# nschejtman/deepLoopCloser

Measured on AMD Instinct MI355X. Metric: query-frames/sec vs N-keyframe DB + top-k recall@1, higher is better.
Workload: dtype bf16; 1 GPU; 1000000 x 4096 bf16 keyframe DB, Q=256, top-20 cosine match, 1 GPU(s); db_rows=1000000, dim=4096, k=20, rows_per_gpu=1000000, pipelined=False, crowded=False

## Files before the change

deeploopcloser_amd/_lib.py:

```python
import ctypes as C
import os

_HERE = os.path.dirname(os.path.abspath(__file__))
LIB_PATH = os.path.join(_HERE, "libdlc_hip.so")

DLC_OK = 0
DLC_ERR_BAD_ARG, DLC_ERR_BAD_SHAPE, DLC_ERR_UNSUPPORTED, DLC_ERR_HIP, DLC_ERR_WORKSPACE = -1, -2, -3, -4, -5
DLC_BF16, DLC_F16, DLC_F32, DLC_F64, DLC_I8, DLC_U8, DLC_I64 = 0, 1, 2, 3, 4, 5, 6
DLC_ACT_NONE, DLC_ACT_SIGMOID, DLC_ACT_RELU = 0, 1, 2
DLC_B_KN, DLC_B_NK = 0, 1
DLC_MAX_K = 128
DLC_ABI_VERSION = 17
DLC_SELECT_COOP = 1
DLC_SIM_FORCE_F64, DLC_SIM_NO_HOST_SYNC = 1, 2

_vp, _i64, _int, _sz, _dbl, _flt = C.c_void_p, C.c_int64, C.c_int, C.c_size_t, C.c_double, C.c_float

SIGNATURES = {
    "dlc_abi_version": (_int, []),
    "dlc_create": (_int, [_int, C.POINTER(_vp)]),
    "dlc_destroy": (_int, [_vp]),
    "dlc_last_error": (C.c_char_p, [_vp]),
    "dlc_status_string": (C.c_char_p, [_int]),
    "dlc_gemm_bias_act": (_int, [_vp, _int, _int, _int, _i64, _i64, _i64, _vp, _i64, _vp, _i64, _vp, _vp, _i64, _vp]),
    "dlc_bias_act": (_int, [_vp, _int, _int, _i64, _i64, _vp, _i64, _vp, _vp, _i64, _vp]),
    "dlc_sdav_encode_workspace_bytes": (_sz, [_i64, C.POINTER(_i64), _int, _int]),
    "dlc_sdav_encode": (_int, [_vp, _int, _i64, _int, C.POINTER(_i64), _vp, C.POINTER(_vp), C.POINTER(_vp), _vp, _vp,
                               _sz, _vp]),
    "dlc_sdav_split_panels_bytes": (_sz, [_int, C.POINTER(_i64)]),
    "dlc_sdav_split_prepare": (_int, [_vp, _int, C.POINTER(_i64), C.POINTER(_vp), _vp, _sz, _vp]),
    "dlc_sdav_encode_split_workspace_bytes": (_sz, [_i64, C.POINTER(_i64), _int]),
    "dlc_cnnvtl_split_panels_bytes": (_sz, [_int, C.POINTER(C.c_int32)]),
    "dlc_cnnvtl_split_prepare": (_int, [_vp, _int, C.POINTER(C.c_int32), C.POINTER(_vp), _vp, _sz, _vp]),
    "dlc_cnnvtl_encode_split_workspace_bytes": (_sz, [_i64, _int, _int, _int, _int, C.POINTER(C.c_int32)]),
    "dlc_cnnvtl_encode_split": (_int, [_vp, _int, _vp, _i64, _int, _int, _int, _int, _int, C.POINTER(C.c_int32), _vp, C.POINTER(_vp),
                                       _vp, _i64, _vp, C.POINTER(_vp), _vp, _vp, _sz, _vp]),
    "dlc_cnnvtl_layers_split": (_int, [_vp, _vp, _i64, _int, _int, _int, _int, C.POINTER(C.c_int32), _int, _int, _vp, C.POINTER(_vp),
                                       C.POINTER(_vp), _vp, _vp, _sz, _vp]),
    "dlc_sdav_encode_split": (_int, [_vp, _i64, _int, C.POINTER(_i64), _vp, _vp, C.POINTER(_vp), _vp, _vp, _sz, _vp]),
    "dlc_sdav_train_workspace_bytes": (_sz, [_i64, _i64, C.POINTER(_i64), _int, _int]),
    "dlc_sdav_train_step": (_int, [_vp, _int, _i64, _i64, _int, C.POINTER(_i64), _vp, C.POINTER(_vp), C.POINTER(_vp),
                                  C.POINTER(_vp), _vp, _dbl, _dbl, _dbl, _dbl, _vp, _vp, _sz, _vp]),
    "dlc_random_mask_f64": (_int, [_vp, _vp, _i64, _i64, C.c_uint64, C.c_uint64, _vp]),
    "dlc_salt_pepper_mask_f64": (_int, [_vp, _vp, _vp, _i64, _i64, C.c_uint64, C.c_uint64, _vp]),
    "dlc_da_corrupt_f64": (_int, [_vp, _vp, _vp, _vp, _i64, _i64, _vp, _i64, _vp]),
    "dlc_da_train_workspace_bytes": (_sz, [_i64, _i64, _i64, _i64]),
    "dlc_da_train_step": (_int, [_vp, _i64, _i64, _i64, _i64, _vp, _vp, _vp, _vp, _vp, _dbl, _dbl, _dbl, _dbl, _vp, _vp, _sz,
                                _vp]),
    "dlc_rgb_to_gray_u8": (_int, [_vp, _vp, _i64, _vp, _vp]),
    "dlc_harris_keypoints_workspace_bytes": (_sz, [_i64, _int, _int]),
    "dlc_harris_keypoints_u8": (_int, [_vp, _vp, _i64, _int, _int, _int, _vp, _vp, _vp, _vp, _sz, _vp]),
    "dlc_extract_patches": (_int, [_vp, _vp, _i64, _int, _int, _vp, _int, _int, _int, _vp, _vp]),
    "dlc_im2col_nhwc_f64": (_int, [_vp, _vp, _i64, _int, _int, _int, _int, _int, _int, _int, _int, _int, _int, _vp, _vp]),
    "dlc_conv2d_nhwc_f64": (_int, [_vp, _vp, _i64, _int, _int, _int, _vp, _vp, _int, _int, _int, _int, _int, _int, _int,
                                  _int, _int, _vp, _vp]),
    "dlc_space_to_depth_nhwc_f64": (_int, [_vp, _vp, _i64, _int, _int, _int, _int, _vp, _vp]),
    "dlc_maxpool3x3s2_nhwc_f64": (_int, [_vp, _vp, _i64, _int, _int, _int, _vp, _vp]),
    "dlc_minmax_quant_gather_i8": (_int, [_vp, C.POINTER(_vp), C.POINTER(_i64), _int, _i64, _vp, _i64, _vp, _vp, _vp]),
    "dlc_cnnvtl_frame_minmax_init": (_int, [_vp, _vp, _i64, _vp]),
    "dlc_conv2d_nhwc_f64_stats": (_int, [_vp, _vp, _i64, _int, _int, _int, _vp, _vp, _int, _int, _int, _int, _int, _int, _int,
                                         _int, _int, _vp, _vp, _vp]),
    "dlc_quant_gather_i8": (_int, [_vp, C.POINTER(_vp), C.POINTER(_i64), _int, _i64, _vp, _i64, _vp, _vp, _vp, _vp]),
    "dlc_sdav_range_words": (_sz, [_i64]),
    "dlc_sdav_distinctive_score": (_int, [_vp, _vp, _i64, _i64, _dbl, _dbl, _vp, _vp, _vp]),
    "dlc_sdav_similarity_workspace_bytes": (_sz, [_i64, _i64, _i64, _int, _i64]),
    "dlc_sdav_similarity_matrix": (_int, [_vp, _vp, _i64, _i64, _i64, _vp, _dbl, _dbl, _vp, _vp, _int, _i64, _vp, _vp, _vp,
                                         _vp, _sz, _vp]),
    "dlc_topk_rows_f64": (_int, [_vp, _vp, _i64, _i64, _i64, _i64, _int, _vp, _vp, _vp, _vp]),
    "dlc_sdav_stream_state_bytes": (_sz, [_i64, _i64, _i64]),
    "dlc_sdav_stream_init": (_int, [_vp, _vp, _sz, _i64, _i64, _i64, _dbl, _dbl, _vp, _vp]),
    "dlc_sdav_stream_append": (_int, [_vp, _vp, _sz, _i64, _i64, _i64, _vp, _i64, _i64, _vp, _vp]),
    "dlc_sdav_stream_query": (_int, [_vp, _vp, _sz, _i64, _i64, _i64, _vp, _i64, _vp, _dbl, _dbl, _vp, _vp, _vp]),
    "dlc_sdav_stream_query_batch_workspace_bytes": (_sz, [_i64, _i64, _i64]),
    "dlc_sdav_stream_query_batch": (_int, [_vp, _vp, _sz, _i64, _i64, _i64, _vp, _i64, _i64, _vp, _dbl, _dbl, _vp, _i64, _vp,
                                           _vp, _sz, _vp]),
    "dlc_sdav_stream_query_batch_staged": (_int, [_vp, _vp, _sz, _i64, _i64, _i64, _vp, _i64, _i64, _vp, _dbl, _dbl, _vp, _i64,
                                                  _vp, _vp, _sz, _int, _vp]),
    "dlc_cnnvtl_distance_matrix": (_int, [_vp, _vp, _i64, _i64, _i64, _vp, _vp]),
    "dlc_cnnvtl_distance_topk_workspace_bytes": (_sz, [_i64, _i64, _i64, _int]),
    "dlc_cnnvtl_distance_topk": (_int, [_vp, _vp, _i64, _i64, _vp, _i64, _i64, _i64, _i64, _i64, _int, _vp, _vp, _vp, _sz,
                                        _vp]),
    "dlc_cnnvtl_distance_rows": (_int, [_vp, _vp, _i64, _i64, _vp, _i64, _i64, _i64, _i64, _i64, _vp, _i64, _vp]),
    "dlc_sequence_topk_workspace_bytes": (_sz, [_i64, _i64, _int, _int, _int]),
    "dlc_sequence_topk": (_int, [_vp, _int, _vp, _i64, _i64, _i64, _i64, _i64, _i64, _int, _int, C.POINTER(C.c_int32), _int, _int,
                                 _vp, _vp, _vp, _vp, _i64, _vp, _vp, _sz, _vp]),
    "dlc_contrast_rows": (_int, [_vp, _int, _vp, _i64, _i64, _i64, _i64, _i64, _int, _vp, _i64, _vp]),
    "dlc_peak_topk_rows_workspace_bytes": (_sz, [_i64, _i64, _int]),
    "dlc_peak_topk_rows": (_int, [_vp, _int, _vp, _i64, _i64, _i64, _i64, _i64, _int, _i64, _int, _i64, _int, _vp, _vp, _vp,
                                  _vp, _sz, _vp]),
    "dlc_l2_normalize_rows": (_int, [_vp, _int, _vp, _i64, _i64, _i64, _int, _int, _vp, _i64, _vp]),
    "dlc_cosine_topk_workspace_bytes": (_sz, [_i64, _i64, _i64, _int]),
    "dlc_cosine_topk": (_int, [_vp, _int, _vp, _i64, _i64, _vp, _i64, _i64, _i64, _int, _i64, _vp, _vp, _vp, _vp, _vp, _vp, _sz,
                              _vp]),
    "dlc_max_row_norm": (_int, [_vp, _int, _vp, _i64, _i64, _i64, _vp, _vp]),
    "dlc_cosine_tau_scale": (_int, [_vp, _int, _vp, _i64, _i64, _i64, _vp, _vp, _vp]),
    "dlc_cosine_topk_older": (_int, [_vp, _int, _vp, _i64, _i64, _vp, _i64, _i64, _i64, _int, _i64, _i64, _vp, _vp, _vp, _vp, _vp,
                                    _vp, _sz, _vp]),
    "dlc_cosine_score_error_bound": (_dbl, [_i64, _i64, _i64, _int]),
    "dlc_cosine_score_error_bound_any_plan": (_dbl, [_i64]),
    "dlc_cosine_score_groups": (_int, [_vp, _int, _vp, _i64, _i64, _vp, _i64, _i64, _i64, _int, _vp, _sz, _vp]),
    "dlc_cosine_select_topk": (_int, [_vp, _int, _vp, _i64, _i64, _vp, _i64, _i64, _i64, _int, _i64, _vp, _vp, _vp, _vp, _vp, _vp,
                                     _sz, _int, _vp]),
    "dlc_cosine_groups_per_query": (_int, [_int]),
    "dlc_cosine_select_groups": (_int, [_vp, _int, _vp, _i64, _i64, _vp, _i64, _i64, _i64, _int, _vp, _sz, _vp, _vp, _int,
                                       _vp]),
    "dlc_cosine_rescore_topk": (_int, [_vp, _int, _vp, _i64, _i64, _vp, _i64, _i64, _i64, _int, _i64, _vp, _vp, _vp, _int,
                                      _vp, _vp, _vp, _vp, _int, _vp]),
    "dlc_cosine_exhaustive_topk": (_int, [_vp, _int, _vp, _i64, _i64, _vp, _i64, _i64, _i64, _int, _i64, _vp, _i64, _dbl,
                                         _vp, _vp, _vp, _vp, _vp, _vp, _sz, _vp]),
    "dlc_topk_merge_strided": (_int, [_vp, _vp, _i64, _vp, _i64, _int, _i64, _int, _vp, _dbl, _vp, _vp, _vp, _vp, _vp, _vp]),
    "dlc_topk_merge": (_int, [_vp, _vp, _vp, _int, _i64, _int, _vp, _vp, _vp, _vp]),
    "dlc_topk_keep_older": (_int, [_vp, _vp, _vp, _i64, _int, _i64, _int, _vp, _vp, _vp]),
    "dlc_cosine_scores_workspace_bytes": (_sz, [_i64, _i64, _i64]),
    "dlc_cosine_scores": (_int, [_vp, _int, _vp, _i64, _i64, _vp, _i64, _i64, _i64, _vp, _i64, _vp, _sz, _vp]),
    "dlc_cosine_score_rows": (_int, [_vp, _int, _vp, _i64, _i64, _vp, _i64, _i64, _i64, _i64, _i64, _vp, _vp, _i64, _vp]),
    "dlc_host_to_device": (_int, [_vp, _vp, _vp, _sz, _vp]),
    "dlc_device_to_host": (_int, [_vp, _vp, _vp, _sz, _vp]),
    "dlc_set_host_threads": (_int, [_vp, _int]),
    "dlc_set_scratch": (_int, [_vp, _vp, _sz]),
    "dlc_set_profiling": (_int, [_vp, _int]),
    "dlc_profile_gemm_ms": (_int, [_vp, C.POINTER(_flt), _int]),
}

_lib = None


class DlcError(RuntimeError):
    """A HIP-side failure (DLC_ERR_HIP / DLC_ERR_WORKSPACE) reported by the C ABI."""


def load():
    global _lib
    if _lib is not None:
        return _lib
    if not os.path.exists(LIB_PATH):
        raise ImportError(
            "deeploopcloser_amd: %s is missing -- build it with `python -c 'import __graft_entry__ as g; g.build()'` "
            "or `make -C deeploopcloser_amd/csrc`.  There is no CPU fallback." % LIB_PATH)
    lib = C.CDLL(LIB_PATH)
    for name, (res, args) in SIGNATURES.items():
        fn = getattr(lib, name)
        fn.restype = res
        fn.argtypes = args
    if lib.dlc_abi_version() != DLC_ABI_VERSION:
        raise ImportError("deeploopcloser_amd: %s has ABI %d, these bindings are for ABI %d -- rebuild it"
                          % (LIB_PATH, lib.dlc_abi_version(), DLC_ABI_VERSION))
    _lib = lib
    return lib


def raise_for_status(lib, ctx, rc):
    if rc == DLC_OK:
        return
    msg = lib.dlc_last_error(ctx).decode() if ctx else ""
    text = "%s: %s" % (lib.dlc_status_string(rc).decode(), msg)
    if rc in (DLC_ERR_BAD_ARG, DLC_ERR_BAD_SHAPE, DLC_ERR_UNSUPPORTED):
        raise ValueError(text)
    raise DlcError(text)
```

deeploopcloser_amd/csrc/cosine_topk.hip:

```cpp
#include "dlc_internal.h"
#include "lds_dma.h"

#include <algorithm>

namespace {

constexpr int BM = 256;
constexpr int BNQ = 256;
constexpr int BK = 64;
constexpr int NTHREADS = 512;
constexpr int TILE_BYTES = 256 * BK * 2;
constexpr int A_TILE = TILE_BYTES;
constexpr int B_TILE = TILE_BYTES;
#ifndef DLC_A_STAGES
#define DLC_A_STAGES 2
#endif
constexpr int A_STAGES = DLC_A_STAGES;
constexpr int B_RING = A_STAGES * A_TILE;
constexpr int LDS_BYTES = A_STAGES * A_TILE + 2 * B_TILE;
#ifndef DLC_STAGGER_SLEEP
#define DLC_STAGGER_SLEEP 15
#endif
#ifndef DLC_STAGGER_PHASES
#define DLC_STAGGER_PHASES 32
// ... 241 lines not shown
#pragma unroll
                for (int r = 0; r < 4; ++r)
                    if (row0 + r < p.n) p.S[(long long)qidx * p.lds + row0 + r] = acc[t][c][r];
            }
        }
    } else {
#pragma unroll
        for (int c = 0; c < 4; ++c) {
            const int qidx = qblk * BNQ + wc * 64 + c * 16 + i;
            float hm[2];
#pragma unroll
            for (int th = 0; th < 2; ++th) {
                float m0 = acc[th * 4][c][0], m1 = acc[th * 4 + 2][c][0];
#pragma unroll
                for (int tt = 0; tt < 2; ++tt)
#pragma unroll
                    for (int r = 0; r < 4; ++r) {
                        m0 = fmaxf(m0, acc[th * 4 + tt][c][r]);
                        m1 = fmaxf(m1, acc[th * 4 + 2 + tt][c][r]);
                    }
                hm[th] = fmaxf(m0, m1);
                const long long g = tile * (BM / GROUP) + wr * 16 + th * 8 + lg * 2;
                if (qidx < p.q) {
                    float* dst = p.gmax + (long long)qidx * p.ldg + g;
                    if (g + 1 < p.ng) *(float2*)dst = make_float2(m0, m1);
                    else if (g < p.ng) dst[0] = m0;
                }
            }
            float h = fmaxf(hm[0], hm[1]);
            h = fmaxf(h, __shfl_xor(h, 16));
            h = fmaxf(h, __shfl_xor(h, 32));
            const long long ht = tile * 2 + wr;
            if (lg == 0 && qidx < p.q && ht < p.nh) p.tmax[(long long)qidx * p.ldt + ht] = h;
        }
    }
}

template <typename Tag> struct Dot2;
template <> struct Dot2<dlc_bf16_tag> {
    typedef __attribute__((ext_vector_type(2))) __bf16 v2_t;
    static __device__ __forceinline__ float run(unsigned a, unsigned b, float c) {
        return __builtin_amdgcn_fdot2_f32_bf16(__builtin_bit_cast(v2_t, a), __builtin_bit_cast(v2_t, b), c, false);
    }
};
template <> struct Dot2<dlc_f16_tag> {
    typedef __attribute__((ext_vector_type(2))) _Float16 v2_t;
    static __device__ __forceinline__ float run(unsigned a, unsigned b, float c) {
        return __builtin_amdgcn_fdot2(__builtin_bit_cast(v2_t, a), __builtin_bit_cast(v2_t, b), c, false);
    }
};

constexpr int GEMV_MAX_Q = 4;
constexpr int GEMV_MAX_LDS = 64 * 1024;

template <typename Tag, int QB>
__global__ __launch_bounds__(256) void score_gemv_kernel(GemmArgs p) {
    extern __shared__ __attribute__((aligned(16))) char smem[];
    __shared__ float wmax[4][QB];
    const int tid = threadIdx.x, lane = tid & 63, w = tid >> 6;
    const long long half = blockIdx.x;
    const int d_bytes = p.nk * 128;
    for (int off = tid * 16; off < QB * d_bytes; off += 256 * 16) {
        const int qi = off / d_bytes, within = off - qi * d_bytes;
        uint4 v = make_uint4(0, 0, 0, 0);
        if (qi < p.q) v = *(const uint4*)(p.Q + (long long)qi * p.ldq_b + within);
        *(uint4*)(smem + off) = v;
    }
    __syncthreads();
    float hmax[QB];
#pragma unroll
    for (int qq = 0; qq < QB; ++qq) hmax[qq] = -INFINITY;
    for (int gi = 0; gi < 4; ++gi) {
        const long long g = half * GROUPS_PER_HALF + w * 4 + gi;
        const char* rows[GROUP];
#pragma unroll
        for (int r = 0; r < GROUP; ++r) {
            long long rr = g * GROUP + r;
            if (rr > p.n - 1) rr = p.n - 1;
            rows[r] = p.DB + rr * p.lddb_b;
        }
        float acc[QB][GROUP];
#pragma unroll
        for (int qq = 0; qq < QB; ++qq)
#pragma unroll
            for (int r = 0; r < GROUP; ++r) acc[qq][r] = 0.f;
        for (int c = lane * 16; c < d_bytes; c += 1024) {
            uint4 rv[GROUP];
#pragma unroll
            for (int r = 0; r < GROUP; ++r) rv[r] = *(const uint4*)(rows[r] + c);
#pragma unroll
            for (int qq = 0; qq < QB; ++qq) {
                const uint4 qv = *(const uint4*)(smem + qq * d_bytes + c);
#pragma unroll
                for (int r = 0; r < GROUP; ++r) {
                    float a = acc[qq][r];
                    a = Dot2<Tag>::run(rv[r].x, qv.x, a);
                    a = Dot2<Tag>::run(rv[r].y, qv.y, a);
                    a = Dot2<Tag>::run(rv[r].z, qv.z, a);
                    a = Dot2<Tag>::run(rv[r].w, qv.w, a);
                    acc[qq][r] = a;
                }
            }
        }
#pragma unroll
        for (int qq = 0; qq < QB; ++qq) {
            float m = -INFINITY;
#pragma unroll
            for (int r = 0; r < GROUP; ++r) {
                float v = acc[qq][r];
#pragma unroll
                for (int o = 32; o > 0; o >>= 1) v += __shfl_xor(v, o);
                m = fmaxf(m, v);
            }
            hmax[qq] = fmaxf(hmax[qq], m);
            if (lane == 0 && qq < p.q && g < p.ng) p.gmax[(long long)qq * p.ldg + g] = m;
        }
    }
    if (lane == 0) {
#pragma unroll
        for (int qq = 0; qq < QB; ++qq) wmax[w][qq] = hmax[qq];
    }
    __syncthreads();
    if (tid < QB && tid < p.q && half < p.nh)
        p.tmax[(long long)tid * p.ldt + half] = fmaxf(fmaxf(wmax[0][tid], wmax[1][tid]), fmaxf(wmax[2][tid], wmax[3][tid]));
}

__device__ __forceinline__ unsigned f32_key(float x) {
    unsigned u = __float_as_uint(x);
    return (u & 0x80000000u) ? ~u : (u | 0x80000000u);
}
__device__ __forceinline__ float key_f32(unsigned k) {
    return __uint_as_float((k & 0x80000000u) ? (k ^ 0x80000000u) : ~k);
}
__device__ __forceinline__ unsigned long long pack_key(float score, unsigned id) {
    return ((unsigned long long)f32_key(score) << 32) | (unsigned long long)(~id);
}
__device__ __forceinline__ unsigned key_id(unsigned long long key) { return ~(unsigned)key; }


__device__ __forceinline__ unsigned wave_max_u32(unsigned v) {
#define DLC_DPP_MAX(ctrl, rmask) \
    v = max(v, (unsigned)__builtin_amdgcn_update_dpp((int)v, (int)v, ctrl, rmask, 0xf, false))
    DLC_DPP_MAX(0x111, 0xf);
    DLC_DPP_MAX(0x112, 0xf);
    DLC_DPP_MAX(0x114, 0xf);
    DLC_DPP_MAX(0x118, 0xf);
    DLC_DPP_MAX(0x142, 0xa);
    DLC_DPP_MAX(0x143, 0xc);
#undef DLC_DPP_MAX
    return (unsigned)__builtin_amdgcn_readlane((int)v, 63);
}

constexpr int FIN_THREADS = 512;
__host__ __device__ inline size_t fin_lds_fixed(int kg) {
    return (size_t)kg * (GROUPS_PER_HALF * 8 + GROUP * (8 + 8 + 4)) + (size_t)(kg + 1) * 8 + 64;
}

__device__ __forceinline__ void rank_select(const unsigned long long* keys, int m, int k, int* out, bool plus_one = false) {
    const int lim = plus_one ? k + 1 : k;
    for (int e = threadIdx.x; e < m; e += blockDim.x) {
        const unsigned long long ke = keys[e];
        if (ke == 0ull) continue;
        int rank = 0;
#pragma unroll 8
        for (int j = 0; j < m; ++j) rank += keys[j] > ke ? 1 : 0;
        if (rank < lim) out[rank] = e;
    }
}
template <typename Id>
__device__ __forceinline__ void rank_select64(const long long* keys, const Id* ids, int m, int k, int* out) {
    for (int e = threadIdx.x; e < m; e += blockDim.x) {
        const long long ke = keys[e];
        if (ke == KEY64_EMPTY) continue;
        const Id ie = ids[e];
        int rank = 0;
#pragma unroll 4
        for (int j = 0; j < m; ++j) {
            const long long kj = keys[j];
            rank += (kj > ke || (kj == ke && kj != KEY64_EMPTY && ids[j] < ie)) ? 1 : 0;
        }
        if (rank < k) out[rank] = e;
    }
}

template <typename Tag, int RS_UNROLL>
__device__ __forceinline__ void rescore8_f64(const char* qrow, const char* const (&rows)[GROUP], int d, int lane,
                                             double (&acc)[GROUP]) {
#pragma unroll
    for (int r = 0; r < GROUP; ++r) acc[r] = 0.0;
    for (int d0 = lane * 8; d0 < d; d0 += 512 * RS_UNROLL) {
        uint4 qv[RS_UNROLL], rv[RS_UNROLL][GROUP];
#pragma unroll
        for (int u = 0; u < RS_UNROLL; ++u) {
            const int dd = d0 + u * 512;
            const bool ok = dd < d;
            qv[u] = ok ? *(const uint4*)(qrow + (long long)dd * 2) : make_uint4(0, 0, 0, 0);
#pragma unroll
            for (int r = 0; r < GROUP; ++r)
                rv[u][r] = ok ? *(const uint4*)(rows[r] + (long long)dd * 2) : make_uint4(0, 0, 0, 0);
        }
#pragma unroll
        for (int u = 0; u < RS_UNROLL; ++u) {
            const unsigned qw[4] = {qv[u].x, qv[u].y, qv[u].z, qv[u].w};
            double qd[8];
#pragma unroll
            for (int e = 0; e < 4; ++e) {
                qd[2 * e] = (double)Mfma16<Tag>::to_f32((unsigned short)(qw[e] & 0xffffu));
                qd[2 * e + 1] = (double)Mfma16<Tag>::to_f32((unsigned short)(qw[e] >> 16));
            }
#pragma unroll
            for (int r = 0; r < GROUP; ++r) {
                const unsigned w4[4] = {rv[u][r].x, rv[u][r].y, rv[u][r].z, rv[u][r].w};
#pragma unroll
                for (int e = 0; e < 4; ++e) {
                    acc[r] = fma(qd[2 * e], (double)Mfma16<Tag>::to_f32((unsigned short)(w4[e] & 0xffffu)), acc[r]);
                    acc[r] = fma(qd[2 * e + 1], (double)Mfma16<Tag>::to_f32((unsigned short)(w4[e] >> 16)), acc[r]);
                }
            }
        }
    }
#pragma unroll
    for (int r = 0; r < GROUP; ++r) {
        double v = acc[r];
#pragma unroll
        for (int o = 32; o > 0; o >>= 1) v += __shfl_xor(v, o);
        acc[r] = v;
    }
}

template <typename Tag, int R, int U>
__device__ __forceinline__ void rescore_rows_f64(const char* qrow, const char* const (&rows)[R], int d, int lane,
                                                 double (&acc)[R]) {
#pragma unroll
    for (int r = 0; r < R; ++r) acc[r] = 0.0;
    for (int d0 = lane * 8; d0 < d; d0 += 512 * U) {
        uint4 qv[U], rv[U][R];
#pragma unroll
        for (int u = 0; u < U; ++u) {
            const int dd = d0 + u * 512;
            const bool ok = dd < d;
            qv[u] = ok ? *(const uint4*)(qrow + (long long)dd * 2) : make_uint4(0, 0, 0, 0);
#pragma unroll
            for (int r = 0; r < R; ++r) rv[u][r] = ok ? *(const uint4*)(rows[r] + (long long)dd * 2) : make_uint4(0, 0, 0, 0);
        }
#pragma unroll
        for (int u = 0; u < U; ++u) {
            const unsigned qw[4] = {qv[u].x, qv[u].y, qv[u].z, qv[u].w};
            double qd[8];
#pragma unroll
            for (int e = 0; e < 4; ++e) {
                qd[2 * e] = (double)Mfma16<Tag>::to_f32((unsigned short)(qw[e] & 0xffffu));
                qd[2 * e + 1] = (double)Mfma16<Tag>::to_f32((unsigned short)(qw[e] >> 16));
            }
#pragma unroll
            for (int r = 0; r < R; ++r) {
                const unsigned w4[4] = {rv[u][r].x, rv[u][r].y, rv[u][r].z, rv[u][r].w};
#pragma unroll
                for (int e = 0; e < 4; ++e) {
                    acc[r] = fma(qd[2 * e], (double)Mfma16<Tag>::to_f32((unsigned short)(w4[e] & 0xffffu)), acc[r]);
                    acc[r] = fma(qd[2 * e + 1], (double)Mfma16<Tag>::to_f32((unsigned short)(w4[e] >> 16)), acc[r]);
                }
            }
        }
    }
#pragma unroll
    for (int r = 0; r < R; ++r) {
        double v = acc[r];
#pragma unroll
        for (int o = 32; o > 0; o >>= 1) v += __shfl_xor(v, o);
        acc[r] = v;
    }
}
template <typename Tag>
__device__ __forceinline__ double rescore1_f64(const char* qrow, const char* row, int d, int lane) {
    const char* const rows[1] = {row};
    double acc[1];
    rescore_rows_f64<Tag, 1, 4>(qrow, rows, d, lane, acc);
    return acc[0];
}

__device__ __forceinline__ double scaled_tau(double tau, const float* __restrict__ tau_scale, int qi) {
    return tau_scale ? tau * (double)tau_scale[qi] : tau;
}

enum { FIN_FUSED = 0, FIN_GROUPS = 1, FIN_RESCORE = 2 };
struct FinishArgs {
    float* tmax; long long ldt; int nh; int tv_in_lds;
    const float* gmax; long long ldg; long long ng;
    int kg;
    const char* Q; long long ldq_b; const char* DB; long long lddb_b;
    long long n; int d; int k; long long row_offset;
    float* out_s;
    double* out_s64;
    long long* out_i;
    int* status;
    double tau;
    const float* tau_scale;
    int* grp_ids;
    float* grp_max;
    const float* all_max;
    int parts;
    long long nq;
    int gparts;
    float* bound_out;
    const float* dense_S;
    long long ld_s;
    int rslack;
    int limited;
    long long limit0;
};
__device__ __forceinline__ long long visible_rows(long long n, int limited, long long limit0, int qi) {
    if (!limited) return n;
    const long long lim = limit0 + qi;
    return lim < 0 ? 0 : (lim < n ? lim : n);
}

template <typename Tag, int THREADS, int RS_UNROLL, int MODE>
__device__ __forceinline__ void finish_topk_body(const FinishArgs& a) {
    extern __shared__ __attribute__((aligned(16))) char dsm[];
    constexpr int FIN_WAVES = THREADS / 64;
    constexpr int FIN_THREADS = THREADS;
    constexpr int GPH = GROUPS_PER_HALF;
    const int kg = a.kg, k = a.k;
    const double tau = scaled_tau(a.tau, a.tau_scale, (int)blockIdx.x);
    const long long n = visible_rows(a.n, a.limited, a.limit0, (int)blockIdx.x);
    const long long ng = a.limited ? (n + GROUP - 1) / GROUP : a.ng;
    if (n <= 0) {
        if constexpr (MODE == FIN_GROUPS) {
            for (int e = threadIdx.x; e <= kg; e += THREADS) {
                if (e < kg) a.grp_ids[(long long)blockIdx.x * kg + e] = -1;
                a.grp_max[(long long)blockIdx.x * (kg + 1) + e] = -INFINITY;
            }
        } else {
            const long long oq = (long long)blockIdx.y * a.nq + blockIdx.x;
            for (int e = threadIdx.x; e < k; e += THREADS) {
                if (a.out_s) a.out_s[oq * k + e] = -INFINITY;
                a.out_s64[oq * k + e] = -INFINITY;
                a.out_i[oq * k + e] = -1;
            }
            if (MODE == FIN_FUSED && threadIdx.x == 0) a.status[blockIdx.x] = 0;
            if (MODE == FIN_RESCORE && a.bound_out && blockIdx.y == 0 && threadIdx.x == 0) a.bound_out[blockIdx.x] = -INFINITY;
        }
        return;
    }
    unsigned long long* ckey = (unsigned long long*)dsm;
    long long* ck64 = (long long*)(dsm + (size_t)kg * GPH * 8);
    double* cs64 = (double*)(dsm + (size_t)kg * (GPH * 8 + GROUP * 8));
    int* crow = (int*)(dsm + (size_t)kg * (GPH * 8 + GROUP * 16));
    int* sel = (int*)(dsm + (size_t)kg * (GPH * 8 + GROUP * 20));
    int* sel2 = sel + kg + 1;
    unsigned* misc = (unsigned*)(sel2 + kg + 1);
    const int qi = blockIdx.x, tid = threadIdx.x, lane = tid & 63, w = tid >> 6;
    float* tv = a.tv_in_lds ? (float*)(dsm + fin_lds_fixed(kg)) : a.tmax + (long long)qi * a.ldt;
    if (a.tv_in_lds)
        for (int e = tid; e < a.nh; e += FIN_THREADS) tv[e] = a.tmax[(long long)qi * a.ldt + e];
    for (int e = tid; e <= kg; e += FIN_THREADS) { sel[e] = -1; sel2[e] = -1; }
    if (tid < 16) misc[tid] = 0u;
    __syncthreads();
    int kg2;
    unsigned bkey = 0u;
    if constexpr (MODE != FIN_RESCORE) {
    const int nh = a.limited ? (int)((n + HALF - 1) / HALF) : a.nh;
    const int kt = min(kg, nh);
    {
        const int chunk = (nh + FIN_WAVES - 1) / FIN_WAVES;
        const int lo_e = w * chunk, hi_e = min(nh, lo_e + chunk);
        unsigned bh = 0, bl = 0;
        constexpr int LV = 16;
        if ((THREADS == 512 || MODE == FIN_GROUPS) && chunk <= 64 * LV) {
            unsigned vk[LV];
#pragma unroll
            for (int j = 0; j < LV; ++j) {
                const int e = lo_e + lane + 64 * j;
                const float v = e < hi_e ? tv[e] : -INFINITY;
                vk[j] = v == -INFINITY ? 0u : f32_key(v);
            }
            auto rescan_regs = [&]() {
                bh = 0; bl = 0;
#pragma unroll
                for (int j = 0; j < LV; ++j) {
                    const unsigned l = ~(unsigned)(lo_e + lane + 64 * j);
                    if (vk[j] > bh) { bh = vk[j]; bl = l; }
                }
            };
            rescan_regs();
            for (int it = 0; it < kt; ++it) {
                const unsigned mh = wave_max_u32(bh);
                const unsigned ml = wave_max_u32(bh == mh ? bl : 0u);
                if (lane == 0) ckey[w * kt + it] = mh == 0u ? 0ull : (((unsigned long long)mh << 32) | ml);
                if (mh != 0u && bh == mh && bl == ml) {
                    const int jr = (int)((~ml) - (unsigned)(lo_e + lane)) >> 6;
#pragma unroll
                    for (int j = 0; j < LV; ++j)
                        if (j == jr) vk[j] = 0u;
                    rescan_regs();
                }
            }
        } else {
        auto rescan = [&]() {
            bh = 0; bl = 0;
            for (int e = lo_e + lane; e < hi_e; e += 64) {
                const float v = tv[e];
                if (v == -INFINITY) continue;
                const unsigned h = f32_key(v), l = ~(unsigned)e;
                if (h > bh || (h == bh && l > bl)) { bh = h; bl = l; }
            }
        };
        rescan();
        for (int it = 0; it < kt; ++it) {
            const unsigned mh = wave_max_u32(bh);
            const unsigned ml = wave_max_u32(bh == mh ? bl : 0u);
            if (lane == 0) ckey[w * kt + it] = mh == 0u ? 0ull : (((unsigned long long)mh << 32) | ml);
            if (mh != 0u && bh == mh && bl == ml) {
                tv[~ml] = -INFINITY;
                rescan();
            }
        }
        }
        const unsigned rest = wave_max_u32(bh);
        if (lane == 0) misc[w] = rest;
    }
    __syncthreads();
    rank_select(ckey, FIN_WAVES * kt, kt, sel, true);
    __syncthreads();
#pragma unroll
    for (int ww = 0; ww < FIN_WAVES; ++ww) bkey = max(bkey, misc[ww]);
    if (sel[kt] >= 0) bkey = max(bkey, (unsigned)(ckey[sel[kt]] >> 32));
    if (tid < kt) { const int c = sel[tid]; sel[tid] = c < 0 ? -1 : (int)key_id(ckey[c]); }
    __syncthreads();

    const int m2 = kt * GPH;
    for (int e = tid; e < m2; e += FIN_THREADS) {
        const int ht = sel[e / GPH];
        const long long g = (long long)ht * GPH + (e % GPH);
        float gm = (ht >= 0 && g < ng) ? a.gmax[(long long)qi * a.ldg + g] : 0.0f;
        if (a.limited && a.dense_S && ht >= 0 && g == ng - 1 && (n & (GROUP - 1))) {
            gm = -INFINITY;
            for (long long row = g * GROUP; row < n; ++row) gm = fmaxf(gm, a.dense_S[(long long)qi * a.ld_s + row]);
        }
        ckey[e] = (ht >= 0 && g < ng) ? pack_key(gm, (unsigned)g) : 0ull;
    }
    __syncthreads();
    kg2 = min(kg, m2);
    rank_select(ckey, m2, kg2, sel2, true);
    __syncthreads();
    if (sel2[kg2] >= 0) bkey = max(bkey, (unsigned)(ckey[sel2[kg2]] >> 32));
    if constexpr (MODE == FIN_GROUPS) {
        const long long W = kg + 1;
        for (int e = tid; e < kg; e += FIN_THREADS) {
            const int c = e < kg2 ? sel2[e] : -1;
            a.grp_ids[(long long)qi * kg + e] = c < 0 ? -1 : (int)key_id(ckey[c]);
            a.grp_max[(long long)qi * W + e] = c < 0 ? -INFINITY : a.gmax[(long long)qi * a.ldg + key_id(ckey[c])];
        }
        if (tid == 0) a.grp_max[(long long)qi * W + kg] = bkey ? key_f32(bkey) : -INFINITY;
        return;
    }
    if (tid < kg2) {
        const int c = sel2[tid];
        int g = c < 0 ? -1 : (int)key_id(ckey[c]);
        if (tid >= k && g >= 0 && sel2[k - 1] >= 0 && !(a.limited && !a.dense_S)) {
            const double uk = (double)key_f32((unsigned)(ckey[sel2[k - 1]] >> 32));
            if ((double)key_f32((unsigned)(ckey[c] >> 32)) < uk - 2.0 * tau) g = -2;
        }
        misc[9] = 0u;
        crow[tid] = g;
    }
    __syncthreads();
    if (tid < kg2) {
        const int g = crow[tid];
        if (g == -2) atomicMax(&misc[9], (unsigned)(ckey[sel2[tid]] >> 32));
    }
    __syncthreads();
    if (tid < kg2) sel2[tid] = crow[tid] < 0 ? -1 : crow[tid];
    bkey = max(bkey, misc[9]);
    __syncthreads();
    } else {
        kg2 = kg;
        const long long W = kg + 1;
        if (a.parts > 0) {
            unsigned bk = 0u;
            for (int e = tid; e < a.parts * (int)W; e += FIN_THREADS) {
                const int pp = e / (int)W, j = e % (int)W;
                const float v = a.all_max[((long long)pp * a.nq + qi) * W + j];
                if (v == -INFINITY) continue;
                if (j == kg) { bk = max(bk, f32_key(v)); continue; }
                int greater = 0;
                for (int p2 = 0; p2 < a.parts; ++p2) {
                    const float* av = a.all_max + ((long long)p2 * a.nq + qi) * W;
                    for (int j2 = 0; j2 < kg; ++j2) greater += av[j2] > v ? 1 : 0;
                }
                if (greater >= kg) bk = max(bk, f32_key(v));
            }
            if (bk) atomicMax(&misc[8], bk);
        }
        for (int e = tid; e < kg; e += FIN_THREADS) {
            int g = a.grp_ids[(long long)qi * kg + e];
            if (g >= 0 && a.parts > 0) {
                const float v = a.grp_max[(long long)qi * W + e];
                int greater = 0;
                for (int pp = 0; pp < a.parts; ++pp) {
                    const float* av = a.all_max + ((long long)pp * a.nq + qi) * W;
                    for (int j = 0; j < kg; ++j) greater += av[j] > v ? 1 : 0;
                }
                if (greater >= kg) g = -1;
            }
            if (a.gparts > 1 && e % a.gparts != (int)blockIdx.y) g = -1;
            sel2[e] = g;
        }
        __syncthreads();
        if (a.parts > 0) bkey = misc[8];
        else {
            const float v = a.grp_max[(long long)qi * W + kg];
            bkey = v == -INFINITY ? 0u : f32_key(v);
        }
        if (a.bound_out && blockIdx.y == 0 && tid == 0) a.bound_out[qi] = bkey ? key_f32(bkey) : -INFINITY;
    }

    int m3;
    if (a.dense_S) {
        const int m = kg2 * GROUP;
        for (int e = tid; e < m; e += FIN_THREADS) {
            const int g = sel2[e / GROUP];
            const long long row = (long long)g * GROUP + (e % GROUP);
            ckey[e] = (g >= 0 && row < n) ? pack_key(a.dense_S[(long long)qi * a.ld_s + row], (unsigned)row) : 0ull;
        }
        m3 = min(k + a.rslack, m);
        for (int e = tid; e <= m3 && e < kg * GROUP; e += FIN_THREADS) crow[e] = -1;
        __syncthreads();
        if (m3 < m) rank_select(ckey, m, m3, crow, true);
        else rank_select(ckey, m, m3, crow, false);
        __syncthreads();
        if (m3 < m && crow[m3] >= 0) bkey = max(bkey, (unsigned)(ckey[crow[m3]] >> 32));
        __syncthreads();
        for (int e = tid; e < m3; e += FIN_THREADS) { const int c = crow[e]; crow[e] = c < 0 ? -1 : (int)key_id(ckey[c]); }
    } else {
        m3 = kg2 * GROUP;
        for (int e = tid; e < m3; e += FIN_THREADS) {
            const int g = sel2[e / GROUP];
            const long long row = (long long)g * GROUP + (e % GROUP);
            crow[e] = (g >= 0 && row < n) ? (int)row : -1;
        }
    }
    __syncthreads();

    const char* qrow = a.Q + (long long)qi * a.ldq_b;
    if (MODE == FIN_FUSED && a.dense_S != nullptr) {
        for (int ci = w; ci < m3; ci += FIN_WAVES) {
            const int id = __builtin_amdgcn_readfirstlane(crow[ci]);
            const double sc = id < 0 ? 0.0 : rescore1_f64<Tag>(qrow, a.DB + (long long)id * a.lddb_b, a.d, lane);
            if (lane == 0) {
                cs64[ci] = id < 0 ? -INFINITY : sc;
                ck64[ci] = id < 0 ? KEY64_EMPTY : f64_key(sc);
            }
        }
    } else
    for (int s = w; s * GROUP < m3; s += FIN_WAVES) {
        int ids[GROUP];
        bool any = false;
        const char* rows[GROUP];
#pragma unroll
        for (int r = 0; r < GROUP; ++r) {
            ids[r] = __builtin_amdgcn_readfirstlane(s * GROUP + r < m3 ? crow[s * GROUP + r] : -1);
            any |= ids[r] >= 0;
            rows[r] = a.DB + (long long)(ids[r] < 0 ? 0 : ids[r]) * a.lddb_b;
        }
        double acc[GROUP] = {0.0, 0.0, 0.0, 0.0, 0.0, 0.0, 0.0, 0.0};
        if (any) rescore8_f64<Tag, RS_UNROLL>(qrow, rows, a.d, lane, acc);
#pragma unroll
        for (int r = 0; r < GROUP; ++r)
            if (lane == r && s * GROUP + r < m3) {
                cs64[s * GROUP + r] = ids[r] < 0 ? -INFINITY : acc[r];
                ck64[s * GROUP + r] = ids[r] < 0 ? KEY64_EMPTY : f64_key(acc[r]);
            }
    }
    const long long oq = (long long)blockIdx.y * a.nq + qi;
    for (int e = tid; e < k; e += FIN_THREADS) {
        if (a.out_s) a.out_s[oq * k + e] = -INFINITY;
        a.out_s64[oq * k + e] = -INFINITY;
        a.out_i[oq * k + e] = -1;
    }
    for (int e = tid; e <= kg; e += FIN_THREADS) sel[e] = -1;
    __syncthreads();

    rank_select64(ck64, crow, m3, k, sel);
    __syncthreads();
    for (int e = tid; e < k; e += FIN_THREADS) {
        const int c = sel[e];
        if (c >= 0) {
            if (a.out_s) a.out_s[oq * k + e] = (float)cs64[c];
            a.out_s64[oq * k + e] = cs64[c];
            a.out_i[oq * k + e] = (long long)crow[c] + a.row_offset;
        }
    }
    if constexpr (MODE == FIN_FUSED) {
        if (tid == 0) {
            const int c = sel[k - 1];
            const bool cert = bkey == 0u || (c >= 0 && cs64[c] > (double)key_f32(bkey) + tau);
            a.status[qi] = cert ? 0 : 1;
        }
    }
}

template <typename Tag, int THREADS, int RS_UNROLL, int MODE>
__global__ __launch_bounds__(THREADS) void finish_topk_kernel(FinishArgs a) {
    finish_topk_body<Tag, THREADS, RS_UNROLL, MODE>(a);
}
template <typename Tag, int RS_UNROLL, int MODE>
__global__ __launch_bounds__(256) __attribute__((amdgpu_waves_per_eu(5))) void finish_topk_coop_kernel(FinishArgs a) {
    finish_topk_body<Tag, 256, RS_UNROLL, MODE>(a);
}

struct ExhaustiveArgs {
    const float* gmax; long long ldg; long long ng;
    const char* Q; long long ldq_b; const char* DB; long long lddb_b;
    long long n; int d; int k; long long row_offset;
    const double* lower; long long lower_stride;
    float* out_s; double* out_s64; long long* out_i;
    int* status;
    double tau;
    const float* tau_scale;
    int limited; long long limit0;
};
constexpr int EXH_BATCH = 64;
constexpr int EXH_POOL = EXH_BATCH * GROUP + DLC_MAX_K;

template <typename Tag, int RS_UNROLL = 4>
__device__ __forceinline__ void exhaustive_topk_body(const ExhaustiveArgs& a, double lower) {
    const int qi = blockIdx.x;
    __shared__ long long pk[EXH_POOL];
    __shared__ double ps[EXH_POOL];
    __shared__ int pid[EXH_POOL];
    __shared__ int qlist[FIN_THREADS];
    __shared__ int wcnt[FIN_THREADS / 64];
    __shared__ int sel[DLC_MAX_K];
    const int tid = threadIdx.x, lane = tid & 63, w = tid >> 6, k = a.k;
    const long long n_vis = visible_rows(a.n, a.limited, a.limit0, qi);
    const long long ng_vis = a.limited ? (n_vis + GROUP - 1) / GROUP : a.ng;
    const double tau = scaled_tau(a.tau, a.tau_scale, qi);
    double theta = lower - tau;
    int cnt = 0;
    const char* qrow = a.Q + (long long)qi * a.ldq_b;
    for (long long c0 = 0; c0 < ng_vis; c0 += FIN_THREADS) {
        const long long g = c0 + tid;
        const bool qual = g < ng_vis && (double)a.gmax[(long long)qi * a.ldg + g] >= theta;
        const unsigned long long bal = __ballot(qual);
        if (lane == 0) wcnt[w] = __popcll(bal);
        __syncthreads();
        int base = 0, nqual = 0;
#pragma unroll
        for (int ww = 0; ww < FIN_THREADS / 64; ++ww) {
            base += ww < w ? wcnt[ww] : 0;
            nqual += wcnt[ww];
        }
        if (qual) qlist[base + __popcll(bal & ((1ull << lane) - 1ull))] = (int)g;
        __syncthreads();
        for (int b0 = 0; b0 < nqual; b0 += EXH_BATCH) {
            const int nb = min(EXH_BATCH, nqual - b0);
            for (int s = w; s < nb; s += FIN_THREADS / 64) {
                const long long row0 = (long long)qlist[b0 + s] * GROUP;
                const char* rows[GROUP];
#pragma unroll
                for (int r = 0; r < GROUP; ++r) rows[r] = a.DB + (row0 + r < a.n ? row0 + r : a.n - 1) * a.lddb_b;
                double acc[GROUP];
                rescore8_f64<Tag, RS_UNROLL>(qrow, rows, a.d, lane, acc);
#pragma unroll
                for (int r = 0; r < GROUP; ++r)
                    if (lane == r) {
                        const bool ok = row0 + r < n_vis;
                        ps[cnt + s * GROUP + r] = ok ? acc[r] : -INFINITY;
                        pk[cnt + s * GROUP + r] = ok ? f64_key(acc[r]) : KEY64_EMPTY;
                        pid[cnt + s * GROUP + r] = (int)(row0 + r);
                    }
            }
            for (int e = tid; e < k; e += FIN_THREADS) sel[e] = -1;
            __syncthreads();
            const int m = cnt + nb * GROUP;
            rank_select64(pk, pid, m, k, sel);
            __syncthreads();
            long long tk = KEY64_EMPTY; double ts = -INFINITY; int ti = -1;
            if (tid < k && sel[tid] >= 0) { const int c = sel[tid]; tk = pk[c]; ts = ps[c]; ti = pid[c]; }
            const unsigned long long have = __ballot(tid < k && sel[tid] >= 0);
            if (lane == 0) wcnt[w] = __popcll(have);
            __syncthreads();
            if (tid < k) { pk[tid] = tk; ps[tid] = ts; pid[tid] = ti; }
            cnt = 0;
#pragma unroll
            for (int ww = 0; ww < FIN_THREADS / 64; ++ww) cnt += wcnt[ww];
            __syncthreads();
            if (cnt == k && ps[k - 1] - tau > theta) theta = ps[k - 1] - tau;
        }
        __syncthreads();
    }
    for (int e = tid; e < k; e += FIN_THREADS) {
        const bool ok = e < cnt;
        if (a.out_s) a.out_s[(long long)qi * k + e] = ok ? (float)ps[e] : -INFINITY;
        if (a.out_s64) a.out_s64[(long long)qi * k + e] = ok ? ps[e] : -INFINITY;
        a.out_i[(long long)qi * k + e] = ok ? (long long)pid[e] + a.row_offset : -1;
    }
    if (tid == 0) a.status[qi] = 2;
}

template <typename Tag>
__global__ __launch_bounds__(FIN_THREADS) void exhaustive_topk_kernel(ExhaustiveArgs a) {
    const int qi = blockIdx.x;
    if (a.status[qi] != 1) return;
    exhaustive_topk_body<Tag>(a, a.lower[(long long)qi * a.lower_stride]);
}

struct SmallArgs {
    const float* P; long long ldp; long long qstride; int nsplit;
    float* gmax; long long ldg;
    const char* Q; long long ldq_b; const char* DB; long long lddb_b;
    long long n; int d; int k; int m3max; long long row_offset;
    float* out_s; double* out_s64; long long* out_i; int* status; double tau;
    const float* tau_scale;
    int limited; long long limit0;
};
constexpr int SMALL_KT_MAX = 40;
constexpr int SMALL_GPT = 4;

template <typename Tag, bool LONG>
__device__ __forceinline__ void small_topk_body(const SmallArgs& a) {
    __shared__ unsigned long long ckey[(FIN_THREADS / 64) * SMALL_KT_MAX];
    __shared__ long long ck64[SMALL_KT_MAX];
    __shared__ double cs64[SMALL_KT_MAX];
    __shared__ int crow[SMALL_KT_MAX];
    __shared__ int sel[SMALL_KT_MAX + 1];
    const int qi = blockIdx.x, tid = threadIdx.x, lane = tid & 63, w = tid >> 6, k = a.k;
    const long long n = visible_rows(a.n, a.limited, a.limit0, qi);
    for (int e = tid; e < k; e += FIN_THREADS) {
        if (a.out_s) a.out_s[(long long)qi * k + e] = -INFINITY;
        a.out_s64[(long long)qi * k + e] = -INFINITY;
        a.out_i[(long long)qi * k + e] = -1;
    }
    for (int e = tid; e <= SMALL_KT_MAX; e += FIN_THREADS) sel[e] = -1;
    if (n <= 0) {
        if (tid == 0) a.status[qi] = 0;
        return;
    }
    const long long ng_all = (a.n + GROUP - 1) / GROUP;
    unsigned vk[SMALL_GPT][GROUP];
#pragma unroll
    for (int j = 0; j < SMALL_GPT; ++j) {
        const long long g = tid + (long long)FIN_THREADS * j;
#pragma unroll
        for (int r = 0; r < GROUP; ++r) vk[j][r] = 0u;
        if (g < ng_all) {
            f64x4_t a64 = {0., 0., 0., 0.}, b64 = {0., 0., 0., 0.};
            const float* src = a.P + (long long)qi * a.ldp + g * GROUP;
            constexpr int PU = LONG ? 4 : 16;
            for (int c0 = 0; c0 < a.nsplit; c0 += PU) {
                f32x4_t pa[PU], pb[PU];
#pragma unroll
                for (int u = 0; u < PU; ++u) {
                    const float* sp = src + (long long)(c0 + u < a.nsplit ? c0 + u : c0) * a.qstride;
                    pa[u] = *(const f32x4_t*)(sp);
                    pb[u] = *(const f32x4_t*)(sp + 4);
                }
#pragma unroll
                for (int u = 0; u < PU; ++u)
                    if (c0 + u < a.nsplit) {
                        a64 += __builtin_convertvector(pa[u], f64x4_t);
                        b64 += __builtin_convertvector(pb[u], f64x4_t);
                    }
            }
            const f32x4_t lo = __builtin_convertvector(a64, f32x4_t), hi = __builtin_convertvector(b64, f32x4_t);
            a.gmax[(long long)qi * a.ldg + g] =
                fmaxf(fmaxf(fmaxf(lo[0], lo[1]), fmaxf(lo[2], lo[3])), fmaxf(fmaxf(hi[0], hi[1]), fmaxf(hi[2], hi[3])));
#pragma unroll
            for (int r = 0; r < 4; ++r) {
                vk[j][r] = g * GROUP + r < n ? f32_key(lo[r]) : 0u;
                vk[j][r + 4] = g * GROUP + r + 4 < n ? f32_key(hi[r]) : 0u;
            }
        }
    }
    const int m3 = (int)(n < (long long)a.m3max ? n : (long long)a.m3max);
    const int kt = (int)(n < (long long)(m3 + 1) ? n : (long long)(m3 + 1));
    unsigned bh = 0u, bl = 0u;
    unsigned gh[SMALL_GPT], gl[SMALL_GPT];
    auto rescan_group = [&](int j) {
        gh[j] = 0u; gl[j] = 0u;
#pragma unroll
        for (int r = 0; r < GROUP; ++r)
            if (vk[j][r] > gh[j]) { gh[j] = vk[j][r]; gl[j] = ~(unsigned)((tid + FIN_THREADS * j) * GROUP + r); }
    };
    auto combine = [&]() {
        bh = 0u; bl = 0u;
#pragma unroll
        for (int j = 0; j < SMALL_GPT; ++j)
            if (gh[j] > bh) { bh = gh[j]; bl = gl[j]; }
    };
#pragma unroll
    for (int j = 0; j < SMALL_GPT; ++j) rescan_group(j);
    combine();
    for (int it = 0; it < kt; ++it) {
        const unsigned mh = wave_max_u32(bh);
        const unsigned ml = wave_max_u32(bh == mh ? bl : 0u);
        if (lane == 0) ckey[w * kt + it] = mh == 0u ? 0ull : (((unsigned long long)mh << 32) | ml);
        if (mh != 0u && bh == mh && bl == ml) {
            const unsigned row = ~ml;
#pragma unroll
            for (int j = 0; j < SMALL_GPT; ++j)
                if ((row >> 3) == (unsigned)(tid + FIN_THREADS * j)) {
#pragma unroll
                    for (int r = 0; r < GROUP; ++r)
                        if ((row & 7u) == (unsigned)r) vk[j][r] = 0u;
                    rescan_group(j);
                }
            combine();
        }
    }
    __syncthreads();
    rank_select(ckey, (FIN_THREADS / 64) * kt, kt, sel);
    __syncthreads();
    const unsigned bkey = (kt > m3 && sel[m3] >= 0) ? (unsigned)(ckey[sel[m3]] >> 32) : 0u;
    if (tid < m3) crow[tid] = sel[tid] < 0 ? -1 : (int)key_id(ckey[sel[tid]]);
    __syncthreads();
    const char* qrow = a.Q + (long long)qi * a.ldq_b;
    constexpr int NW = FIN_THREADS / 64;
    if constexpr (LONG) {
        for (int s3 = w; s3 * 3 < m3; s3 += NW) {
            int ids[3];
            const char* rows[3];
#pragma unroll
            for (int r = 0; r < 3; ++r) {
                ids[r] = __builtin_amdgcn_readfirstlane(s3 * 3 + r < m3 ? crow[s3 * 3 + r] : -1);
                rows[r] = a.DB + (long long)(ids[r] < 0 ? 0 : ids[r]) * a.lddb_b;
            }
            double acc[3];
            rescore_rows_f64<Tag, 3, 4>(qrow, rows, a.d, lane, acc);
#pragma unroll
            for (int r = 0; r < 3; ++r)
                if (lane == r && s3 * 3 + r < m3) {
                    cs64[s3 * 3 + r] = ids[r] < 0 ? -INFINITY : acc[r];
                    ck64[s3 * 3 + r] = ids[r] < 0 ? KEY64_EMPTY : f64_key(acc[r]);
                }
        }
    } else {
    int ci = w;
    for (; ci + NW < m3; ci += 2 * NW) {
        const int id0 = __builtin_amdgcn_readfirstlane(crow[ci]), id1 = __builtin_amdgcn_readfirstlane(crow[ci + NW]);
        const char* const rows[2] = {a.DB + (long long)(id0 < 0 ? 0 : id0) * a.lddb_b,
                                     a.DB + (long long)(id1 < 0 ? 0 : id1) * a.lddb_b};
        double sc[2];
        rescore_rows_f64<Tag, 2, 8>(qrow, rows, a.d, lane, sc);
        if (lane == 0) {
            cs64[ci] = id0 < 0 ? -INFINITY : sc[0];
            ck64[ci] = id0 < 0 ? KEY64_EMPTY : f64_key(sc[0]);
            cs64[ci + NW] = id1 < 0 ? -INFINITY : sc[1];
            ck64[ci + NW] = id1 < 0 ? KEY64_EMPTY : f64_key(sc[1]);
        }
    }
// ... 172 lines not shown
    }
}

template <typename Src, typename Tag, int TPR, int NVEC>
__global__ __launch_bounds__(256) void l2_normalize_regs_kernel(const Src* __restrict__ src, long long lds, long long n,
                                                                int d, int center, unsigned short* __restrict__ dst,
                                                                long long ldd) {
    constexpr int VW = 16 / (int)sizeof(Src);
    typedef Src vec_t __attribute__((ext_vector_type(VW)));
    __shared__ double red[2][4];
    const int tid = threadIdx.x, lane = tid & 63;
    const int t = TPR == 64 ? lane : tid;
    const long long row = TPR == 64 ? (long long)blockIdx.x * 4 + (tid >> 6) : (long long)blockIdx.x;
    if (row >= n) return;
    const Src* x = src + row * lds;
    vec_t v[NVEC];
#pragma unroll
    for (int j = 0; j < NVEC; ++j) {
        const int e0 = (j * TPR + t) * VW;
        if (e0 + VW <= d) {
            v[j] = *(const vec_t*)(x + e0);
        } else {
#pragma unroll
            for (int i = 0; i < VW; ++i) v[j][i] = e0 + i < d ? x[e0 + i] : (Src)0;
        }
    }
    auto row_sum = [&](double s, int slot) -> double {
        for (int o = 32; o > 0; o >>= 1) s += __shfl_xor(s, o);
        if constexpr (TPR == 64) return s;
        if (lane == 0) red[slot][tid >> 6] = s;
        __syncthreads();
        return red[slot][0] + red[slot][1] + red[slot][2] + red[slot][3];
    };
    double mean = 0.0;
    if (center) {
        double s = 0.0;
#pragma unroll
        for (int j = 0; j < NVEC; ++j)
#pragma unroll
            for (int i = 0; i < VW; ++i) s += (double)v[j][i];
        mean = row_sum(s, 0) / (double)d;
    }
    double ss = 0.0;
#pragma unroll
    for (int j = 0; j < NVEC; ++j)
#pragma unroll
        for (int i = 0; i < VW; ++i) {
            const double c = (double)v[j][i] - mean;
            ss += ((j * TPR + t) * VW + i < d) ? c * c : 0.0;
        }
    const double nrm = sqrt(row_sum(ss, 1));
    const double inv = nrm > 0.0 ? 1.0 / nrm : 1.0;
    unsigned short* o = dst + row * ldd;
#pragma unroll
    for (int j = 0; j < NVEC; ++j) {
        const int e0 = (j * TPR + t) * VW;
        if (e0 >= ldd) continue;
        unsigned short bits[VW];
#pragma unroll
        for (int i = 0; i < VW; ++i) {
            bits[i] = 0;
            if (e0 + i < d) {
                const float f = f64_to_f32_once(((double)v[j][i] - mean) * inv);
                if constexpr (__is_same(Tag, dlc_bf16_tag)) bits[i] = __builtin_bit_cast(unsigned short, (__bf16)f);
                else bits[i] = __builtin_bit_cast(unsigned short, (_Float16)f);
            }
        }
        if constexpr (VW == 4) {
            *(uint2*)(o + e0) = make_uint2((unsigned)bits[0] | ((unsigned)bits[1] << 16),
                                           (unsigned)bits[2] | ((unsigned)bits[3] << 16));
        } else {
            *(unsigned*)(o + e0) = (unsigned)bits[0] | ((unsigned)bits[1] << 16);
        }
    }
}

__global__ __launch_bounds__(256) void splitk_groups_kernel(float* __restrict__ P, long long ldp, int q, int nsplit,
                                                            float* __restrict__ gmax, long long ldg, long long ng,
                                                            float* __restrict__ tmax, long long ldt, long long nh,
                                                            int keep_sum) {
    const int qi = blockIdx.x;
    const long long g = (long long)blockIdx.y * 256 + threadIdx.x;
    float m = -INFINITY;
    if (g < ng) {
        f64x4_t a64 = {0., 0., 0., 0.}, b64 = {0., 0., 0., 0.};
        float* dst0 = P + (long long)qi * ldp + g * GROUP;
        const float* src = dst0;
        for (int c = 0; c < nsplit; ++c) {
            a64 += __builtin_convertvector(*(const f32x4_t*)(src), f64x4_t);
            b64 += __builtin_convertvector(*(const f32x4_t*)(src + 4), f64x4_t);
            src += (long long)q * ldp;
        }
        const f32x4_t a = __builtin_convertvector(a64, f32x4_t), b = __builtin_convertvector(b64, f32x4_t);
        if (keep_sum && nsplit > 1) {
            *(f32x4_t*)dst0 = a;
            *(f32x4_t*)(dst0 + 4) = b;
        }
        m = fmaxf(fmaxf(fmaxf(a[0], a[1]), fmaxf(a[2], a[3])), fmaxf(fmaxf(b[0], b[1]), fmaxf(b[2], b[3])));
        gmax[(long long)qi * ldg + g] = m;
    }
    m = fmaxf(m, __shfl_xor(m, 1));
    m = fmaxf(m, __shfl_xor(m, 2));
    m = fmaxf(m, __shfl_xor(m, 4));
    m = fmaxf(m, __shfl_xor(m, 8));
    const long long ht = g / GROUPS_PER_HALF;
    if ((threadIdx.x & 15) == 0 && ht < nh) tmax[(long long)qi * ldt + ht] = m;
}

__global__ __launch_bounds__(256) void splitk_dense_kernel(const float* __restrict__ P, long long ldp, int q, int nsplit,
                                                           float* __restrict__ S, long long lds, long long n) {
    const int qi = blockIdx.x;
    const long long r0 = ((long long)blockIdx.y * 256 + threadIdx.x) * 4;
    if (r0 >= n) return;
    f64x4_t a64 = {0., 0., 0., 0.};
    const float* src = P + (long long)qi * ldp + r0;
    for (int c = 0; c < nsplit; ++c) {
        a64 += __builtin_convertvector(*(const f32x4_t*)src, f64x4_t);
        src += (long long)q * ldp;
    }
    const f32x4_t a = __builtin_convertvector(a64, f32x4_t);
#pragma unroll
    for (int r = 0; r < 4; ++r)
        if (r0 + r < n) S[(long long)qi * lds + r0 + r] = a[r];
}

struct SplitPlan {
    int nsplit, kchunk;
};
SplitPlan split_plan(int64_t q, int64_t n, int64_t d) {
    const int64_t ntiles = dlc::cdiv(n, BM);
    const int64_t base = dlc::cdiv(ntiles, (int64_t)8) * 8 * dlc::cdiv(q, BNQ);
    const int64_t nk = d / BK;
    SplitPlan best{1, (int)nk};
    if (base >= 256 || nk < 8) return best;
    const double t_k = 1.6, t_fix = 8.0, t_launch = 5.0, bytes_per_us = 3.0e6;
    const double part_bytes = (double)q * (double)ntiles * BM * 4.0;
    const int64_t work = ntiles * dlc::cdiv(q, BNQ);
    double best_t = (double)dlc::cdiv(work, (int64_t)256) * ((double)nk * t_k + t_fix);
    for (int64_t ns = 2; ns <= nk / 4 && ns <= 256; ++ns) {
        const int64_t kc = dlc::cdiv(nk, ns), ns_eff = dlc::cdiv(nk, kc);
        if (ns_eff != ns) continue;
        if ((double)ns_eff * part_bytes > (double)(1ll << 30)) break;
        const double t = (double)dlc::cdiv(work * ns_eff, (int64_t)256) * ((double)kc * t_k + t_fix) +
                         2.0 * (double)ns_eff * part_bytes / bytes_per_us + t_launch;
        if (t < best_t * 0.9) {
            best_t = t;
            best = SplitPlan{(int)ns_eff, (int)kc};
        }
    }
    return best;
}

struct WsLayout {
    size_t gmax, tmax, part, status, s64, rs_ids, rs_max, rs_scores, rs_idx, rs_bound, total;
    long long ldg, ldt, ldp;
    int kg;
    SplitPlan sp;
    int rparts;
    bool dense;
    double tau;
};

inline bool gemv_shape(int64_t q, int64_t nk) {
    const int qb = q <= 1 ? 1 : (q <= 2 ? 2 : 4);
    return q <= GEMV_MAX_Q && (long long)qb * nk * 128 <= GEMV_MAX_LDS;
}

constexpr int64_t DENSE_MAX_ROWS = 16384;
constexpr int DENSE_ROW_SLACK = 4;
constexpr int64_t DENSE_GEMV_BYTES = 32ll << 20;
inline bool dense_plan(int64_t q, int64_t n, int64_t d) {
    return n <= DENSE_MAX_ROWS && (!gemv_shape(q, d / BK) || n * d * 2 <= DENSE_GEMV_BYTES);
}

int rescore_parts(int64_t q, int64_t d, int kg, int k) {
    if (q > 32 || (int64_t)kg * GROUP * d * 2 < (2 << 20)) return 1;
    return std::min(kg, 2048 / k);
}

constexpr double SCORE_STEP_EPS = 1.1920928955078125e-07;
double score_error_bound(int64_t q, int64_t nk, const SplitPlan& sp, bool dense) {
    double steps;
    if (!dense && gemv_shape(q, nk)) steps = (double)nk * 0.5 + 8.0;
    else steps = 2.0 * (double)sp.kchunk + 2.0;
    return SCORE_STEP_EPS * 1.01 * steps + 3.7e-12;
}

WsLayout ws_layout(int64_t q, int64_t n, int64_t d, int k) {
    WsLayout w;
    const int64_t ntiles = dlc::cdiv(n, BM);
    w.ldg = ntiles * (BM / GROUP);
    w.ldt = ntiles * 2;
    w.kg = k + SLACK;
    size_t o = 0;
    w.gmax = o; o += dlc::align_up((size_t)q * w.ldg * 4, 256);
    w.tmax = o; o += dlc::align_up((size_t)q * w.ldt * 4, 256);
    w.sp = split_plan(q, n, d);
    w.dense = dense_plan(q, n, d);
    w.tau = score_error_bound(q, d / BK, w.sp, w.dense);
    w.ldp = ntiles * BM;
    w.part = o;
    if (w.sp.nsplit > 1 || w.dense) o += dlc::align_up((size_t)w.sp.nsplit * q * w.ldp * 4, 256);
    w.status = o; o += dlc::align_up((size_t)q * 4, 256);
    w.s64 = o; o += dlc::align_up((size_t)q * k * 8, 256);
    w.rparts = w.dense ? 1 : rescore_parts(q, d, w.kg, k);
    w.rs_ids = w.rs_max = w.rs_scores = w.rs_idx = w.rs_bound = o;
    if (w.rparts > 1) {
        w.rs_ids = o; o += dlc::align_up((size_t)q * w.kg * 4, 256);
        w.rs_max = o; o += dlc::align_up((size_t)q * (w.kg + 1) * 4, 256);
        w.rs_scores = o; o += dlc::align_up((size_t)w.rparts * q * k * 8, 256);
        w.rs_idx = o; o += dlc::align_up((size_t)w.rparts * q * k * 8, 256);
        w.rs_bound = o; o += dlc::align_up((size_t)q * 4, 256);
    }
    w.total = o;
    return w;
}

int check_operands(dlc_ctx* ctx, int dtype, const void* Q, int64_t q, int64_t ldq, const void* DB, int64_t n,
                   int64_t lddb, int64_t d) {
    if (!ctx) return DLC_ERR_BAD_ARG;
    if (dtype != DLC_BF16 && dtype != DLC_F16)
        return dlc::fail(ctx, DLC_ERR_UNSUPPORTED, "cosine match: dtype %d (need DLC_BF16 or DLC_F16)", dtype);
    if (!Q || !DB || q < 1 || n < 1 || d < 1) return dlc::fail(ctx, DLC_ERR_BAD_ARG, "cosine match: null/empty operand");
    if (d % BK != 0) return dlc::fail(ctx, DLC_ERR_BAD_SHAPE, "cosine match: d=%lld must be a multiple of %d", (long long)d, BK);
    if (ldq < d || lddb < d || (ldq % 8) || (lddb % 8))
        return dlc::fail(ctx, DLC_ERR_BAD_SHAPE, "cosine match: row strides must be >= d and multiples of 8 elements");
    if (((uintptr_t)Q & 15) || ((uintptr_t)DB & 15))
        return dlc::fail(ctx, DLC_ERR_BAD_ARG, "cosine match: operands must be 16-byte aligned");
    if (ldq * 2 * 255 + 128 > 0xffffffffll || lddb * 2 * 255 + 128 > 0xffffffffll)
        return dlc::fail(ctx, DLC_ERR_BAD_SHAPE, "cosine match: row stride %lld elements too large (255 rows must span < 4 GiB)",
                         (long long)(ldq > lddb ? ldq : lddb));
    if (q > 0x7fffff00ll) return dlc::fail(ctx, DLC_ERR_BAD_SHAPE, "cosine match: q too large");
    if (n > 0x7ffffff0ll) return dlc::fail(ctx, DLC_ERR_BAD_SHAPE, "cosine match: more than 2^31 rows in one shard");
    return DLC_OK;
}

template <typename Tag, int MODE, bool MASKQ>
int launch_gemm_masked(dlc_ctx* ctx, const GemmArgs& a, hipStream_t st);

template <typename Tag, int MODE>
int launch_gemm(dlc_ctx* ctx, const GemmArgs& a, hipStream_t st) {
    const int tail = a.q % BNQ;
    return (tail > 0 && tail <= 192) ? launch_gemm_masked<Tag, MODE, true>(ctx, a, st)
                                     : launch_gemm_masked<Tag, MODE, false>(ctx, a, st);
}

template <typename Tag> constexpr int tag_id() { return __is_same(Tag, dlc_bf16_tag) ? 0 : 1; }

template <typename K>
int raise_lds_limit(dlc_ctx* ctx, K kern, int bit, int bytes) {
    const unsigned long long m = 1ull << bit;
    if (!(ctx->func_attr_set & m)) {
        DLC_HIP_CHECK(ctx, hipFuncSetAttribute((const void*)kern, hipFuncAttributeMaxDynamicSharedMemorySize, bytes));
        ctx->func_attr_set |= m;
    }
    return DLC_OK;
}

template <typename Tag, int MODE, bool MASKQ>
int launch_gemm_masked(dlc_ctx* ctx, const GemmArgs& a, hipStream_t st) {
    auto kern = score_gemm_kernel<Tag, MODE, MASKQ>;
    int rc_attr = raise_lds_limit(ctx, kern, DLC_ATTR_GEMM_BASE + tag_id<Tag>() * 8 + MODE * 2 + (MASKQ ? 1 : 0), LDS_BYTES);
    if (rc_attr != DLC_OK) return rc_attr;
    GemmArgs b = a;
    b.ntiles = dlc::cdiv(a.n, BM);
    b.nqb = (int)dlc::cdiv(a.q, BNQ);
    if (MODE != GEMM_PARTIAL) { b.nsplit = 1; b.kchunk = a.nk; }
    const long long nwg = dlc::cdiv(b.ntiles, 8) * 8 * b.nqb * b.nsplit;
    if (nwg > 0x7fffffffll) return dlc::fail(ctx, DLC_ERR_BAD_SHAPE, "cosine match: %lld workgroups exceed the grid limit", nwg);
    dim3 grid((unsigned)nwg);
    b.stagger_mult = (nwg >= 3 * 256) ? 4 : 2;
    b.stagger_phases = (nwg >= 3 * 256) ? DLC_STAGGER_PHASES : 16;
    hipLaunchKernelGGL(kern, grid, dim3(NTHREADS), LDS_BYTES, st, b);
    DLC_LAUNCH_CHECK(ctx, "score_gemm_kernel");
    return DLC_OK;
}

inline bool use_gemv(const GemmArgs& a) { return gemv_shape(a.q, a.nk); }

template <typename Tag, int QB>
int launch_gemv_qb(dlc_ctx* ctx, const GemmArgs& a, hipStream_t st) {
    auto kern = score_gemv_kernel<Tag, QB>;
    const int lds = QB * a.nk * 128;
    int rc_attr = raise_lds_limit(ctx, kern, DLC_ATTR_GEMV_BASE + tag_id<Tag>() * 3 + (QB == 1 ? 0 : (QB == 2 ? 1 : 2)), GEMV_MAX_LDS);
    if (rc_attr != DLC_OK) return rc_attr;
    hipLaunchKernelGGL(kern, dim3((unsigned)a.nh), dim3(256), lds, st, a);
    DLC_LAUNCH_CHECK(ctx, "score_gemv_kernel");
    return DLC_OK;
}

template <typename Tag>
int launch_gemv(dlc_ctx* ctx, const GemmArgs& a, hipStream_t st) {
    if (a.q <= 1) return launch_gemv_qb<Tag, 1>(ctx, a, st);
    if (a.q <= 2) return launch_gemv_qb<Tag, 2>(ctx, a, st);
    return launch_gemv_qb<Tag, 4>(ctx, a, st);
}

template <typename Tag>
int launch_scores(dlc_ctx* ctx, const GemmArgs& a, bool dense, hipStream_t st, bool keep = false, bool partials_only = false) {
    if (!dense && !keep && use_gemv(a)) return launch_gemv<Tag>(ctx, a, st);
    if (a.nsplit <= 1 && !keep)
        return dense ? launch_gemm<Tag, GEMM_DENSE>(ctx, a, st) : launch_gemm<Tag, GEMM_GROUPS>(ctx, a, st);
    int rc = launch_gemm<Tag, GEMM_PARTIAL>(ctx, a, st);
    if (rc != DLC_OK) return rc;
    if (partials_only) return DLC_OK;
    if (dense) {
        dim3 grid((unsigned)a.q, (unsigned)dlc::cdiv(a.n, (int64_t)1024));
        hipLaunchKernelGGL(splitk_dense_kernel, grid, dim3(256), 0, st, a.P, a.ldp, a.q, a.nsplit, a.S, a.lds, a.n);
        DLC_LAUNCH_CHECK(ctx, "splitk_dense_kernel");
    } else {
        const long long groups = dlc::cdiv(a.n, BM) * (BM / GROUP);
        dim3 grid((unsigned)a.q, (unsigned)dlc::cdiv(groups, (long long)256));
        hipLaunchKernelGGL(splitk_groups_kernel, grid, dim3(256), 0, st, a.P, a.ldp, a.q, a.nsplit, a.gmax, a.ldg, a.ng,
                           a.tmax, a.ldt, a.nh, keep ? 1 : 0);
        DLC_LAUNCH_CHECK(ctx, "splitk_groups_kernel");
    }
    return DLC_OK;
}

}

extern "C" size_t dlc_cosine_topk_workspace_bytes(int64_t q, int64_t n, int64_t d, int k) {
    if (q < 1 || n < 1 || d < BK || k < 1 || k > DLC_MAX_K) return 0;
    return ws_layout(q, n, d, k).total;
}

namespace {

struct MatchCall {
    GemmArgs a;
    WsLayout w;
};

int prepare_match(dlc_ctx* ctx, const char* what, int dtype, const void* Q, int64_t q, int64_t ldq, const void* DB,
                  int64_t n, int64_t lddb, int64_t d, int k, void* workspace, size_t workspace_bytes, MatchCall* mc) {
    int rc = check_operands(ctx, dtype, Q, q, ldq, DB, n, lddb, d);
    if (rc != DLC_OK) return rc;
    if (k < 1 || k > DLC_MAX_K) return dlc::fail(ctx, DLC_ERR_BAD_ARG, "%s: k=%d outside 1..%d", what, k, DLC_MAX_K);
    mc->w = ws_layout(q, n, d, k);
    if (!workspace || workspace_bytes < mc->w.total)
        return dlc::fail(ctx, DLC_ERR_WORKSPACE, "%s: workspace %zu < %zu bytes", what, workspace_bytes, mc->w.total);
    if (((uintptr_t)workspace & 255)) return dlc::fail(ctx, DLC_ERR_BAD_ARG, "%s: workspace must be 256-byte aligned", what);
    char* ws = (char*)workspace;
    GemmArgs& a = mc->a;
    a.Q = (const char*)Q; a.DB = (const char*)DB;
    a.ldq_b = ldq * 2; a.lddb_b = lddb * 2;
    a.q = (int)q; a.n = n; a.nk = (int)(d / BK);
    a.gmax = (float*)(ws + mc->w.gmax); a.ldg = mc->w.ldg;
    a.tmax = (float*)(ws + mc->w.tmax); a.ldt = mc->w.ldt;
    a.ng = dlc::cdiv(n, GROUP); a.nh = dlc::cdiv(n, HALF);
    a.S = nullptr; a.lds = 0;
    a.nsplit = mc->w.sp.nsplit; a.kchunk = mc->w.sp.kchunk;
    a.P = (float*)(ws + mc->w.part); a.ldp = mc->w.ldp;
    return DLC_OK;
}

inline bool small_direct(const MatchCall& mc, int k) {
    return mc.w.dense && mc.a.n <= (int64_t)FIN_THREADS * SMALL_GPT * GROUP && k + DENSE_ROW_SLACK + 1 <= SMALL_KT_MAX;
}

int run_score(dlc_ctx* ctx, int dtype, MatchCall& mc, hipStream_t st, bool partials_only = false) {
    return dlc::profiled(ctx, st, [&]() -> int {
        return (dtype == DLC_BF16) ? launch_scores<dlc_bf16_tag>(ctx, mc.a, false, st, mc.w.dense, partials_only)
                                   : launch_scores<dlc_f16_tag>(ctx, mc.a, false, st, mc.w.dense, partials_only);
    });
}

FinishArgs finish_args(const MatchCall& mc, int k, int64_t n, int64_t d, int64_t q, int64_t row_offset) {
    const GemmArgs& g = mc.a;
    FinishArgs f{};
    f.tmax = g.tmax; f.ldt = g.ldt; f.nh = (int)g.nh;
    f.gmax = g.gmax; f.ldg = g.ldg; f.ng = g.ng;
    f.kg = mc.w.kg;
    f.Q = g.Q; f.ldq_b = g.ldq_b; f.DB = g.DB; f.lddb_b = g.lddb_b;
    f.n = n; f.d = (int)d; f.k = k; f.row_offset = row_offset;
    f.tau = mc.w.tau;
    f.nq = q;
    return f;
}

template <typename Tag, int THREADS, int RS_UNROLL, int MODE>
int launch_finish(dlc_ctx* ctx, FinishArgs f, int64_t q, bool small_lds, hipStream_t st) {
    size_t dsm = fin_lds_fixed(f.kg);
    f.tv_in_lds = MODE != FIN_RESCORE && !small_lds && (size_t)f.nh * 4 <= 96 * 1024;
    if (f.tv_in_lds) dsm += (size_t)f.nh * 4;
    dsm = dlc::align_up(dsm, 16);
    void (*fk)(FinishArgs);
    if constexpr (THREADS == 256) fk = finish_topk_coop_kernel<Tag, RS_UNROLL, MODE>;
    else fk = finish_topk_kernel<Tag, THREADS, RS_UNROLL, MODE>;
    if (dsm > 48 * 1024)
        DLC_HIP_CHECK(ctx, hipFuncSetAttribute((const void*)fk, hipFuncAttributeMaxDynamicSharedMemorySize, (int)dsm));
    hipLaunchKernelGGL(fk, dim3((unsigned)q, (unsigned)(MODE == FIN_RESCORE && f.gparts > 1 ? f.gparts : 1)), dim3(THREADS),
                       dsm, st, f);
    DLC_LAUNCH_CHECK(ctx, "finish_topk_kernel");
    return DLC_OK;
}

template <int MODE>
int run_select(dlc_ctx* ctx, int dtype, const FinishArgs& f, int64_t q, int flags, hipStream_t st) {
    const bool coop = (flags & DLC_SELECT_COOP) != 0;
    if (dtype == DLC_BF16)
        return coop ? launch_finish<dlc_bf16_tag, 256, 1, MODE>(ctx, f, q, true, st)
                    : launch_finish<dlc_bf16_tag, 512, 4, MODE>(ctx, f, q, false, st);
    return coop ? launch_finish<dlc_f16_tag, 256, 1, MODE>(ctx, f, q, true, st)
                : launch_finish<dlc_f16_tag, 512, 4, MODE>(ctx, f, q, false, st);
}

int run_exhaustive(dlc_ctx* ctx, int dtype, const FinishArgs& f, int64_t q, const double* lower, int64_t lower_stride,
                   float* out_s, double* out_s64, int64_t* out_i, int* status, hipStream_t st) {
    ExhaustiveArgs e{};
    e.gmax = f.gmax; e.ldg = f.ldg; e.ng = f.ng;
    e.Q = f.Q; e.ldq_b = f.ldq_b; e.DB = f.DB; e.lddb_b = f.lddb_b;
    e.n = f.n; e.d = f.d; e.k = f.k; e.row_offset = f.row_offset;
    e.lower = lower; e.lower_stride = lower_stride;
    e.out_s = out_s; e.out_s64 = out_s64; e.out_i = (long long*)out_i;
    e.status = status; e.tau = f.tau; e.tau_scale = f.tau_scale;
    e.limited = f.limited; e.limit0 = f.limit0;
    if (dtype == DLC_BF16)
        hipLaunchKernelGGL(exhaustive_topk_kernel<dlc_bf16_tag>, dim3((unsigned)q), dim3(FIN_THREADS), 0, st, e);
    else
        hipLaunchKernelGGL(exhaustive_topk_kernel<dlc_f16_tag>, dim3((unsigned)q), dim3(FIN_THREADS), 0, st, e);
    DLC_LAUNCH_CHECK(ctx, "exhaustive_topk_kernel");
    return DLC_OK;
}

int launch_merge(dlc_ctx* ctx, const double* scores, int64_t score_part_stride, const int64_t* idx, int64_t idx_part_stride,
                 int parts, int64_t q, int k, const float* bound, double tau, const float* tau_scale, float* out_scores,
                 double* out_scores_f64, int64_t* out_idx, int* status, hipStream_t st) {
    const size_t m = (size_t)parts * k;
    const size_t dsm = m * 24;
    if (dsm > 48 * 1024) return dlc::fail(ctx, DLC_ERR_BAD_SHAPE, "topk_merge: parts*k=%zu too large (max 2048)", m);
    hipLaunchKernelGGL(merge_topk_kernel, dim3((unsigned)q), dim3(FIN_THREADS), dsm, st, scores, (long long)score_part_stride,
                       (const long long*)idx, (long long)idx_part_stride, parts, (long long)q, k, bound, tau, tau_scale,
                       out_scores, out_scores_f64, (long long*)out_idx, status);
    DLC_LAUNCH_CHECK(ctx, "merge_topk_kernel");
    return DLC_OK;
}

int run_finish(dlc_ctx* ctx, int dtype, const MatchCall& mc, int k, int64_t n, int64_t d, int64_t q, int64_t row_offset,
               float* out_scores, double* out_scores_f64, int64_t* out_idx, int32_t* out_status, void* workspace, int flags,
               const float* tau_scale, hipStream_t st, int limited = 0, int64_t limit0 = 0, bool direct = false) {
    char* ws = (char*)workspace;
    FinishArgs f = finish_args(mc, k, n, d, q, row_offset);
    f.limited = limited; f.limit0 = limit0; f.tau_scale = tau_scale;
    int* status = out_status ? out_status : (int*)(ws + mc.w.status);
    double* s64 = out_scores_f64 ? out_scores_f64 : (double*)(ws + mc.w.s64);
    int rc;
    if (direct) {
        SmallArgs sa{};
        sa.P = mc.a.P; sa.ldp = mc.a.ldp; sa.qstride = (long long)q * mc.a.ldp; sa.nsplit = mc.a.nsplit;
        sa.gmax = mc.a.gmax; sa.ldg = mc.a.ldg;
        sa.Q = f.Q; sa.ldq_b = f.ldq_b; sa.DB = f.DB; sa.lddb_b = f.lddb_b;
        sa.n = n; sa.d = (int)d; sa.k = k; sa.m3max = k + DENSE_ROW_SLACK; sa.row_offset = row_offset;
        sa.out_s = out_scores; sa.out_s64 = s64; sa.out_i = (long long*)out_idx; sa.status = status; sa.tau = mc.w.tau;
        sa.tau_scale = tau_scale; sa.limited = limited; sa.limit0 = limit0;
        const bool long_rows = d >= 16384;
        if (dtype == DLC_BF16) {
            if (long_rows) hipLaunchKernelGGL(small_topk_long_kernel<dlc_bf16_tag>, dim3((unsigned)q), dim3(FIN_THREADS), 0, st, sa);
            else hipLaunchKernelGGL(small_topk_kernel<dlc_bf16_tag>, dim3((unsigned)q), dim3(FIN_THREADS), 0, st, sa);
        } else {
            if (long_rows) hipLaunchKernelGGL(small_topk_long_kernel<dlc_f16_tag>, dim3((unsigned)q), dim3(FIN_THREADS), 0, st, sa);
            else hipLaunchKernelGGL(small_topk_kernel<dlc_f16_tag>, dim3((unsigned)q), dim3(FIN_THREADS), 0, st, sa);
        }
        DLC_LAUNCH_CHECK(ctx, "small_topk_kernel");
    } else if (mc.w.rparts <= 1) {
        f.out_s = out_scores; f.out_s64 = s64; f.out_i = (long long*)out_idx; f.status = status;
        if (mc.w.dense) { f.dense_S = mc.a.P; f.ld_s = mc.a.ldp; f.rslack = DENSE_ROW_SLACK; }
        rc = run_select<FIN_FUSED>(ctx, dtype, f, q, flags, st);
        if (rc != DLC_OK) return rc;
    } else {
        f.grp_ids = (int*)(ws + mc.w.rs_ids); f.grp_max = (float*)(ws + mc.w.rs_max);
        rc = run_select<FIN_GROUPS>(ctx, dtype, f, q, 0, st);
        if (rc != DLC_OK) return rc;
        double* ps = (double*)(ws + mc.w.rs_scores);
        int64_t* pi = (int64_t*)(ws + mc.w.rs_idx);
        float* pb = (float*)(ws + mc.w.rs_bound);
        f.gparts = mc.w.rparts; f.out_s = nullptr; f.out_s64 = ps; f.out_i = (long long*)pi; f.bound_out = pb;
        rc = run_select<FIN_RESCORE>(ctx, dtype, f, q, DLC_SELECT_COOP, st);
        if (rc != DLC_OK) return rc;
        rc = launch_merge(ctx, ps, q * k, pi, q * k, mc.w.rparts, q, k, pb, mc.w.tau, tau_scale, out_scores, s64, out_idx, status, st);
        if (rc != DLC_OK) return rc;
    }
    if (direct) return DLC_OK;
    return run_exhaustive(ctx, dtype, f, q, s64 + (k - 1), k, out_scores, s64, out_idx, status, st);
}

}

extern "C" double dlc_cosine_score_error_bound(int64_t q, int64_t n, int64_t d, int k) {
    if (q < 1 || n < 1 || d < BK || k < 1 || k > DLC_MAX_K) return 0.0;
    return ws_layout(q, n, d, k).tau;
}

extern "C" int dlc_cosine_topk(dlc_ctx* ctx, int dtype, const void* Q, int64_t q, int64_t ldq, const void* DB,
                               int64_t n, int64_t lddb, int64_t d, int k, int64_t row_offset, float* out_scores,
                               double* out_scores_f64, int64_t* out_idx, int32_t* out_status, const float* tau_scale,
                               void* workspace, size_t workspace_bytes, void* stream) {
    if (!ctx) return DLC_ERR_BAD_ARG;
    if (!out_scores || !out_idx) return dlc::fail(ctx, DLC_ERR_BAD_ARG, "cosine_topk: null output");
    MatchCall mc;
    int rc = prepare_match(ctx, "cosine_topk", dtype, Q, q, ldq, DB, n, lddb, d, k, workspace, workspace_bytes, &mc);
    if (rc != DLC_OK) return rc;
    dlc::DeviceGuard guard(ctx->device);
    if (!guard.ok) return dlc::fail(ctx, DLC_ERR_HIP, "hipSetDevice(%d) failed", ctx->device);
    const bool direct = small_direct(mc, k);
    rc = run_score(ctx, dtype, mc, (hipStream_t)stream, direct);
    if (rc != DLC_OK) return rc;
    return run_finish(ctx, dtype, mc, k, n, d, q, row_offset, out_scores, out_scores_f64, out_idx, out_status, workspace, 0,
                      tau_scale, (hipStream_t)stream, 0, 0, direct);
}

extern "C" int dlc_cosine_topk_older(dlc_ctx* ctx, int dtype, const void* Q, int64_t q, int64_t ldq, const void* DB,
                                     int64_t n, int64_t lddb, int64_t d, int k, int64_t row_offset, int64_t limit0,
                                     float* out_scores, double* out_scores_f64, int64_t* out_idx, int32_t* out_status,
                                     const float* tau_scale, void* workspace, size_t workspace_bytes, void* stream) {
    if (!ctx) return DLC_ERR_BAD_ARG;
    if (!out_scores || !out_idx) return dlc::fail(ctx, DLC_ERR_BAD_ARG, "cosine_topk_older: null output");
    MatchCall mc;
    int rc = prepare_match(ctx, "cosine_topk_older", dtype, Q, q, ldq, DB, n, lddb, d, k, workspace, workspace_bytes, &mc);
    if (rc != DLC_OK) return rc;
    dlc::DeviceGuard guard(ctx->device);
    if (!guard.ok) return dlc::fail(ctx, DLC_ERR_HIP, "hipSetDevice(%d) failed", ctx->device);
    const bool direct = small_direct(mc, k);
    rc = run_score(ctx, dtype, mc, (hipStream_t)stream, direct);
    if (rc != DLC_OK) return rc;
    return run_finish(ctx, dtype, mc, k, n, d, q, row_offset, out_scores, out_scores_f64, out_idx, out_status, workspace, 0,
                      tau_scale, (hipStream_t)stream, 1, limit0, direct);
}

extern "C" int dlc_cosine_score_groups(dlc_ctx* ctx, int dtype, const void* Q, int64_t q, int64_t ldq, const void* DB,
                                       int64_t n, int64_t lddb, int64_t d, int k, void* workspace,
                                       size_t workspace_bytes, void* stream) {
    if (!ctx) return DLC_ERR_BAD_ARG;
    MatchCall mc;
    int rc = prepare_match(ctx, "cosine_score_groups", dtype, Q, q, ldq, DB, n, lddb, d, k, workspace, workspace_bytes, &mc);
    if (rc != DLC_OK) return rc;
    dlc::DeviceGuard guard(ctx->device);
    if (!guard.ok) return dlc::fail(ctx, DLC_ERR_HIP, "hipSetDevice(%d) failed", ctx->device);
    return run_score(ctx, dtype, mc, (hipStream_t)stream);
}

extern "C" int dlc_cosine_select_topk(dlc_ctx* ctx, int dtype, const void* Q, int64_t q, int64_t ldq, const void* DB,
                                      int64_t n, int64_t lddb, int64_t d, int k, int64_t row_offset, float* out_scores,
                                      double* out_scores_f64, int64_t* out_idx, int32_t* out_status,
                                      const float* tau_scale, void* workspace, size_t workspace_bytes, int flags,
                                      void* stream) {
    if (!ctx) return DLC_ERR_BAD_ARG;
    if (!out_scores || !out_idx) return dlc::fail(ctx, DLC_ERR_BAD_ARG, "cosine_select_topk: null output");
    MatchCall mc;
    int rc = prepare_match(ctx, "cosine_select_topk", dtype, Q, q, ldq, DB, n, lddb, d, k, workspace, workspace_bytes, &mc);
    if (rc != DLC_OK) return rc;
    dlc::DeviceGuard guard(ctx->device);
    if (!guard.ok) return dlc::fail(ctx, DLC_ERR_HIP, "hipSetDevice(%d) failed", ctx->device);
    return run_finish(ctx, dtype, mc, k, n, d, q, row_offset, out_scores, out_scores_f64, out_idx, out_status, workspace, flags,
                      tau_scale, (hipStream_t)stream);
}

extern "C" int dlc_cosine_groups_per_query(int k) { return (k < 1 || k > DLC_MAX_K) ? 0 : k + SLACK; }

extern "C" int dlc_cosine_select_groups(dlc_ctx* ctx, int dtype, const void* Q, int64_t q, int64_t ldq, const void* DB,
                                        int64_t n, int64_t lddb, int64_t d, int k, void* workspace,
                                        size_t workspace_bytes, int32_t* group_ids, float* group_max, int flags,
                                        void* stream) {
    if (!ctx) return DLC_ERR_BAD_ARG;
    if (!group_ids || !group_max) return dlc::fail(ctx, DLC_ERR_BAD_ARG, "cosine_select_groups: null output");
    MatchCall mc;
    int rc = prepare_match(ctx, "cosine_select_groups", dtype, Q, q, ldq, DB, n, lddb, d, k, workspace, workspace_bytes, &mc);
    if (rc != DLC_OK) return rc;
    dlc::DeviceGuard guard(ctx->device);
    if (!guard.ok) return dlc::fail(ctx, DLC_ERR_HIP, "hipSetDevice(%d) failed", ctx->device);
    FinishArgs f = finish_args(mc, k, n, d, q, 0);
    f.grp_ids = group_ids; f.grp_max = group_max;
    return run_select<FIN_GROUPS>(ctx, dtype, f, q, flags, (hipStream_t)stream);
}

namespace {
int operands_only(dlc_ctx* ctx, const char* what, int dtype, const void* Q, int64_t q, int64_t ldq, const void* DB, int64_t n,
                  int64_t lddb, int64_t d, int k, MatchCall* mc) {
    int rc = check_operands(ctx, dtype, Q, q, ldq, DB, n, lddb, d);
    if (rc != DLC_OK) return rc;
    if (k < 1 || k > DLC_MAX_K) return dlc::fail(ctx, DLC_ERR_BAD_ARG, "%s: k=%d outside 1..%d", what, k, DLC_MAX_K);
    mc->w = ws_layout(q, n, d, k);
    mc->a = GemmArgs{};
    mc->a.Q = (const char*)Q; mc->a.DB = (const char*)DB;
    mc->a.ldq_b = ldq * 2; mc->a.lddb_b = lddb * 2;
    mc->a.q = (int)q; mc->a.n = n; mc->a.nk = (int)(d / BK);
    mc->a.ng = dlc::cdiv(n, GROUP); mc->a.nh = dlc::cdiv(n, HALF);
    return DLC_OK;
}
}

extern "C" int dlc_cosine_rescore_topk(dlc_ctx* ctx, int dtype, const void* Q, int64_t q, int64_t ldq, const void* DB,
                                       int64_t n, int64_t lddb, int64_t d, int k, int64_t row_offset,
                                       const int32_t* group_ids, const float* group_max, const float* all_group_max,
                                       int parts, double* out_scores_f64, int64_t* out_idx, float* out_bound,
                                       const float* tau_scale, int flags, void* stream) {
    if (!ctx) return DLC_ERR_BAD_ARG;
    if (!out_scores_f64 || !out_idx || !group_ids || !group_max || parts < 0 || (parts > 0 && !all_group_max))
        return dlc::fail(ctx, DLC_ERR_BAD_ARG, "cosine_rescore_topk: bad argument");
    MatchCall mc;
    int rc = operands_only(ctx, "cosine_rescore_topk", dtype, Q, q, ldq, DB, n, lddb, d, k, &mc);
    if (rc != DLC_OK) return rc;
    dlc::DeviceGuard guard(ctx->device);
    if (!guard.ok) return dlc::fail(ctx, DLC_ERR_HIP, "hipSetDevice(%d) failed", ctx->device);
    FinishArgs f = finish_args(mc, k, n, d, q, row_offset);
    f.grp_ids = const_cast<int32_t*>(group_ids); f.grp_max = const_cast<float*>(group_max);
    f.all_max = all_group_max; f.parts = parts;
    f.out_s = nullptr; f.out_s64 = out_scores_f64; f.out_i = (long long*)out_idx; f.bound_out = out_bound;
    f.tau_scale = tau_scale;
    return run_select<FIN_RESCORE>(ctx, dtype, f, q, flags, (hipStream_t)stream);
}

extern "C" int dlc_cosine_exhaustive_topk(dlc_ctx* ctx, int dtype, const void* Q, int64_t q, int64_t ldq, const void* DB,
                                          int64_t n, int64_t lddb, int64_t d, int k, int64_t row_offset,
                                          const double* lower, int64_t lower_stride, double tau,
                                          const float* tau_scale, int32_t* status, float* out_scores, double* out_scores_f64, int64_t* out_idx, void* workspace,
                                          size_t workspace_bytes, void* stream) {
    if (!ctx) return DLC_ERR_BAD_ARG;
    if (!lower || lower_stride < 0 || !status || !out_idx || !(tau >= 0.0))
        return dlc::fail(ctx, DLC_ERR_BAD_ARG, "cosine_exhaustive_topk: bad argument");
    MatchCall mc;
    int rc = prepare_match(ctx, "cosine_exhaustive_topk", dtype, Q, q, ldq, DB, n, lddb, d, k, workspace, workspace_bytes, &mc);
    if (rc != DLC_OK) return rc;
    dlc::DeviceGuard guard(ctx->device);
    if (!guard.ok) return dlc::fail(ctx, DLC_ERR_HIP, "hipSetDevice(%d) failed", ctx->device);
    FinishArgs f = finish_args(mc, k, n, d, q, row_offset);
    f.tau = tau; f.tau_scale = tau_scale;
    return run_exhaustive(ctx, dtype, f, q, lower, lower_stride, out_scores, out_scores_f64, out_idx, status, (hipStream_t)stream);
}

namespace {
__global__ __launch_bounds__(256) void keep_older_kernel(const float* __restrict__ scores, const long long* __restrict__ idx,
                                                         long long rows, int kk, long long limit0, int k,
                                                         float* __restrict__ out_s, long long* __restrict__ out_i) {
    const int lane = threadIdx.x & 63;
    const long long b = (long long)blockIdx.x * 4 + (threadIdx.x >> 6);
    if (b >= rows) return;
    int kept = 0;
    for (int c0 = 0; c0 < kk && kept < k; c0 += 64) {
        const int c = c0 + lane;
        const long long id = c < kk ? idx[b * kk + c] : -1;
        const bool ok = id >= 0 && id < limit0 + b;
        const unsigned long long m = __ballot(ok);
        const int pos = kept + __popcll(m & ((1ull << lane) - 1ull));
        if (ok && pos < k) {
            out_s[b * k + pos] = scores[b * kk + c];
            out_i[b * k + pos] = id;
        }
        kept += __popcll(m);
    }
    for (int e = (kept < k ? kept : k) + lane; e < k; e += 64) {
        out_s[b * k + e] = -INFINITY;
        out_i[b * k + e] = -1;
    }
}
}

extern "C" int dlc_topk_keep_older(dlc_ctx* ctx, const float* scores, const int64_t* idx, int64_t rows, int kk,
                                   int64_t limit0, int k, float* out_scores, int64_t* out_idx, void* stream) {
    if (!ctx) return DLC_ERR_BAD_ARG;
    if (!scores || !idx || !out_scores || !out_idx || rows < 1 || kk < 1 || kk > DLC_MAX_K || k < 1 || k > DLC_MAX_K)
        return dlc::fail(ctx, DLC_ERR_BAD_ARG, "topk_keep_older: bad argument (1 <= kk, k <= %d)", DLC_MAX_K);
    dlc::DeviceGuard guard(ctx->device);
    if (!guard.ok) return dlc::fail(ctx, DLC_ERR_HIP, "hipSetDevice(%d) failed", ctx->device);
    hipLaunchKernelGGL(keep_older_kernel, dim3((unsigned)dlc::cdiv(rows, (int64_t)4)), dim3(256), 0, (hipStream_t)stream, scores,
                       (const long long*)idx, (long long)rows, kk, (long long)limit0, k, out_scores, (long long*)out_idx);
    DLC_LAUNCH_CHECK(ctx, "keep_older_kernel");
    return DLC_OK;
}

extern "C" int dlc_topk_merge_strided(dlc_ctx* ctx, const double* scores_f64, int64_t score_part_stride, const int64_t* idx,
                                      int64_t idx_part_stride, int parts, int64_t q, int k, const float* bound, double tau,
                                      const float* tau_scale, float* out_scores, double* out_scores_f64, int64_t* out_idx,
                                      int32_t* out_status, void* stream) {
    if (!ctx) return DLC_ERR_BAD_ARG;
    if (!scores_f64 || !idx || !out_idx || parts < 1 || q < 1 || k < 1 || k > DLC_MAX_K ||
        score_part_stride < q * k || idx_part_stride < q * k || !(tau >= 0.0))
        return dlc::fail(ctx, DLC_ERR_BAD_ARG, "topk_merge: bad argument");
    dlc::DeviceGuard guard(ctx->device);
    if (!guard.ok) return dlc::fail(ctx, DLC_ERR_HIP, "hipSetDevice(%d) failed", ctx->device);
    return launch_merge(ctx, scores_f64, score_part_stride, idx, idx_part_stride, parts, q, k, bound, tau, tau_scale,
                        out_scores, out_scores_f64, out_idx, out_status, (hipStream_t)stream);
}

extern "C" int dlc_topk_merge(dlc_ctx* ctx, const double* scores_f64, const int64_t* idx, int parts, int64_t q, int k,
                              float* out_scores, double* out_scores_f64, int64_t* out_idx, void* stream) {
    return dlc_topk_merge_strided(ctx, scores_f64, q * k, idx, q * k, parts, q, k, nullptr, 0.0, nullptr, out_scores,
                                  out_scores_f64, out_idx, nullptr, stream);
}

extern "C" size_t dlc_cosine_scores_workspace_bytes(int64_t q, int64_t n, int64_t d) {
    if (q < 1 || n < 1 || d < BK) return 0;
    const SplitPlan sp = split_plan(q, n, d);
    return sp.nsplit > 1 ? dlc::align_up((size_t)sp.nsplit * q * dlc::cdiv(n, BM) * BM * 4, 256) : 0;
}

extern "C" int dlc_cosine_scores(dlc_ctx* ctx, int dtype, const void* Q, int64_t q, int64_t ldq, const void* DB,
                                 int64_t n, int64_t lddb, int64_t d, float* S, int64_t lds, void* workspace,
                                 size_t workspace_bytes, void* stream) {
    int rc = check_operands(ctx, dtype, Q, q, ldq, DB, n, lddb, d);
    if (rc != DLC_OK) return rc;
    if (!S || lds < n) return dlc::fail(ctx, DLC_ERR_BAD_ARG, "cosine_scores: bad output");
    const SplitPlan sp = split_plan(q, n, d);
    const size_t need = dlc_cosine_scores_workspace_bytes(q, n, d);
    if (need && (!workspace || workspace_bytes < need))
        return dlc::fail(ctx, DLC_ERR_WORKSPACE, "cosine_scores: workspace %zu < %zu bytes", workspace_bytes, need);
    if (need && ((uintptr_t)workspace & 255)) return dlc::fail(ctx, DLC_ERR_BAD_ARG, "cosine_scores: workspace must be 256-byte aligned");
    dlc::DeviceGuard guard(ctx->device);
    if (!guard.ok) return dlc::fail(ctx, DLC_ERR_HIP, "hipSetDevice(%d) failed", ctx->device);
    GemmArgs a{};
    a.Q = (const char*)Q; a.DB = (const char*)DB;
    a.ldq_b = ldq * 2; a.lddb_b = lddb * 2;
    a.q = (int)q; a.n = n; a.nk = (int)(d / BK);
    a.S = S; a.lds = lds;
    a.nsplit = sp.nsplit; a.kchunk = sp.kchunk;
    a.P = (float*)workspace; a.ldp = dlc::cdiv(n, BM) * BM;
    return (dtype == DLC_BF16) ? launch_scores<dlc_bf16_tag>(ctx, a, true, (hipStream_t)stream)
                               : launch_scores<dlc_f16_tag>(ctx, a, true, (hipStream_t)stream);
}

extern "C" int dlc_l2_normalize_rows(dlc_ctx* ctx, int src_dtype, const void* src, int64_t n, int64_t d, int64_t lds,
                                     int center, int dst_dtype, void* dst, int64_t ldd, void* stream) {
    if (!ctx) return DLC_ERR_BAD_ARG;
    if (!src || !dst || n < 1 || d < 1 || lds < d || ldd < d)
        return dlc::fail(ctx, DLC_ERR_BAD_ARG, "l2_normalize_rows: bad argument");
    if (ldd % BK) return dlc::fail(ctx, DLC_ERR_BAD_SHAPE, "l2_normalize_rows: ldd=%lld must be a multiple of %d", (long long)ldd, BK);
    if (ldd > 0x7fffffff) return dlc::fail(ctx, DLC_ERR_BAD_SHAPE, "l2_normalize_rows: ldd too large");
    if ((uintptr_t)dst & 3) return dlc::fail(ctx, DLC_ERR_BAD_SHAPE, "l2_normalize_rows: dst must be 4-byte aligned");
    dlc::DeviceGuard guard(ctx->device);
    if (!guard.ok) return dlc::fail(ctx, DLC_ERR_HIP, "hipSetDevice(%d) failed", ctx->device);
    hipStream_t st = (hipStream_t)stream;
    if (src_dtype != DLC_F32 && src_dtype != DLC_F64)
        return dlc::fail(ctx, DLC_ERR_UNSUPPORTED, "l2_normalize_rows: dtype pair %d -> %d", src_dtype, dst_dtype);
    if (dst_dtype != DLC_BF16 && dst_dtype != DLC_F16)
        return dlc::fail(ctx, DLC_ERR_UNSUPPORTED, "l2_normalize_rows: dtype pair %d -> %d", src_dtype, dst_dtype);
    unsigned short* o = (unsigned short*)dst;
    const int vw = src_dtype == DLC_F32 ? 4 : 2;
    const bool aligned = ((uintptr_t)src & 15) == 0 && (lds % vw) == 0 && ((uintptr_t)dst & 7) == 0;
    const int64_t cap_wave = 64 * 4 * vw, cap_block = 256 * 16 * vw;
#define DLC_NORM_REGS(SRC, TAG, TPR)                                                                              \
    hipLaunchKernelGGL((l2_normalize_regs_kernel<SRC, TAG, TPR, 16>), dim3((unsigned)(TPR == 64 ? dlc::cdiv(n, 4) : n)), \
                       dim3(256), 0, st, (const SRC*)src, (long long)lds, (long long)n, (int)d, center, o, (long long)ldd)
#define DLC_NORM(SRC, TAG) \
    hipLaunchKernelGGL((l2_normalize_kernel<SRC, TAG>), dim3((unsigned)n), dim3(256), 0, st, (const SRC*)src, (long long)lds, (int)d, center, o, (long long)ldd)
#define DLC_NORM_PICK(SRC, TAG)                                                   \
    do {                                                                          \
        if (aligned && ldd <= cap_wave) DLC_NORM_REGS(SRC, TAG, 64);              \
        else if (aligned && ldd <= cap_block) DLC_NORM_REGS(SRC, TAG, 256);       \
        else DLC_NORM(SRC, TAG);                                                  \
    } while (0)
    if (src_dtype == DLC_F32 && dst_dtype == DLC_BF16) DLC_NORM_PICK(float, dlc_bf16_tag);
    else if (src_dtype == DLC_F32 && dst_dtype == DLC_F16) DLC_NORM_PICK(float, dlc_f16_tag);
    else if (src_dtype == DLC_F64 && dst_dtype == DLC_BF16) DLC_NORM_PICK(double, dlc_bf16_tag);
    else DLC_NORM_PICK(double, dlc_f16_tag);
#undef DLC_NORM_PICK
#undef DLC_NORM_REGS
#undef DLC_NORM
    DLC_LAUNCH_CHECK(ctx, "l2_normalize_kernel");
    return DLC_OK;
}

namespace {
template <typename Tag>
__device__ __forceinline__ float row_norm_up(const char* __restrict__ row, int d, int lane) {
    float acc = 0.f;
    for (int c = lane * 8; c < d; c += 512) {
        const u32x4_t v = *(const u32x4_t*)(row + (long long)c * 2);
#pragma unroll
        for (int j = 0; j < 4; ++j) {
            float lo, hi;
            if constexpr (__is_same(Tag, dlc_bf16_tag)) {
                lo = __uint_as_float(v[j] << 16);
                hi = __uint_as_float(v[j] & 0xffff0000u);
            } else {
                lo = dlc_f16_bits_to_f32((unsigned short)(v[j] & 0xffffu));
                hi = dlc_f16_bits_to_f32((unsigned short)(v[j] >> 16));
            }
            acc = fmaf(lo, lo, acc);
            acc = fmaf(hi, hi, acc);
        }
    }
#pragma unroll
    for (int m = 32; m >= 1; m >>= 1) acc += __shfl_xor(acc, m, 64);
    const float nrm = sqrtf(acc) * 1.001f;
    return (nrm <= 3.0e38f) ? nrm : INFINITY;
}

template <typename Tag>
__global__ __launch_bounds__(256) void max_row_norm_kernel(const char* __restrict__ rows, long long ld_b, long long n, int d,
                                                           float* __restrict__ out) {
    const int lane = threadIdx.x & 63;
    float best = 0.f;
    for (long long r = (long long)blockIdx.x * 4 + (threadIdx.x >> 6); r < n; r += (long long)gridDim.x * 4)
        best = fmaxf(best, row_norm_up<Tag>(rows + r * ld_b, d, lane));
    if (lane == 0) atomicMax((unsigned*)out, __float_as_uint(best));
}

template <typename Tag>
__global__ __launch_bounds__(256) void tau_scale_kernel(const char* __restrict__ Q, long long ldq_b, long long q, int d,
                                                        const float* __restrict__ db_max_norm, float* __restrict__ out) {
    const int lane = threadIdx.x & 63;
    const long long qi = (long long)blockIdx.x * 4 + (threadIdx.x >> 6);
    if (qi >= q) return;
    const float nq = row_norm_up<Tag>(Q + qi * ldq_b, d, lane);
    const float R = db_max_norm ? *db_max_norm : 1.005f;
    const float prod = nq * R * (1.0f / 1.01f) * 1.000001f;
    const float s = (prod <= 3.0e38f) ? fmaxf(prod, 1.0f) : INFINITY;
    if (lane == 0) out[qi] = s;
}

int check_rows(dlc_ctx* ctx, const char* what, int dtype, const void* rows, int64_t n, int64_t ld, int64_t d) {
    if (!ctx) return DLC_ERR_BAD_ARG;
    if (dtype != DLC_BF16 && dtype != DLC_F16)
        return dlc::fail(ctx, DLC_ERR_UNSUPPORTED, "%s: dtype %d (need DLC_BF16 or DLC_F16)", what, dtype);
    if (!rows || n < 1 || d < 1) return dlc::fail(ctx, DLC_ERR_BAD_ARG, "%s: null/empty operand", what);
    if (d % 8 != 0 || ld < d || (ld % 8) || ((uintptr_t)rows & 15))
        return dlc::fail(ctx, DLC_ERR_BAD_SHAPE, "%s: rows must be 16-byte aligned, d and the stride multiples of 8 elements", what);
    if (d > 0x7ffffff0ll) return dlc::fail(ctx, DLC_ERR_BAD_SHAPE, "%s: d too large", what);
    return DLC_OK;
}
}

extern "C" int dlc_max_row_norm(dlc_ctx* ctx, int dtype, const void* rows, int64_t n, int64_t ld, int64_t d,
                                float* max_norm, void* stream) {
    int rc = check_rows(ctx, "max_row_norm", dtype, rows, n, ld, d);
    if (rc != DLC_OK) return rc;
    if (!max_norm) return dlc::fail(ctx, DLC_ERR_BAD_ARG, "max_row_norm: null output");
    dlc::DeviceGuard guard(ctx->device);
    if (!guard.ok) return dlc::fail(ctx, DLC_ERR_HIP, "hipSetDevice(%d) failed", ctx->device);
    const unsigned grid = (unsigned)std::min<int64_t>(dlc::cdiv(n, 4), 256 * 16);
    if (dtype == DLC_BF16)
        hipLaunchKernelGGL(max_row_norm_kernel<dlc_bf16_tag>, dim3(grid), dim3(256), 0, (hipStream_t)stream, (const char*)rows,
                           (long long)ld * 2, (long long)n, (int)d, max_norm);
    else
        hipLaunchKernelGGL(max_row_norm_kernel<dlc_f16_tag>, dim3(grid), dim3(256), 0, (hipStream_t)stream, (const char*)rows,
                           (long long)ld * 2, (long long)n, (int)d, max_norm);
    DLC_LAUNCH_CHECK(ctx, "max_row_norm_kernel");
    return DLC_OK;
}

extern "C" int dlc_cosine_tau_scale(dlc_ctx* ctx, int dtype, const void* Q, int64_t q, int64_t ldq, int64_t d,
                                    const float* db_max_norm, float* tau_scale, void* stream) {
    int rc = check_rows(ctx, "cosine_tau_scale", dtype, Q, q, ldq, d);
    if (rc != DLC_OK) return rc;
    if (!tau_scale) return dlc::fail(ctx, DLC_ERR_BAD_ARG, "cosine_tau_scale: null output");
    dlc::DeviceGuard guard(ctx->device);
    if (!guard.ok) return dlc::fail(ctx, DLC_ERR_HIP, "hipSetDevice(%d) failed", ctx->device);
    const unsigned grid = (unsigned)dlc::cdiv(q, 4);
    if (dtype == DLC_BF16)
        hipLaunchKernelGGL(tau_scale_kernel<dlc_bf16_tag>, dim3(grid), dim3(256), 0, (hipStream_t)stream, (const char*)Q,
                           (long long)ldq * 2, (long long)q, (int)d, db_max_norm, tau_scale);
    else
        hipLaunchKernelGGL(tau_scale_kernel<dlc_f16_tag>, dim3(grid), dim3(256), 0, (hipStream_t)stream, (const char*)Q,
                           (long long)ldq * 2, (long long)q, (int)d, db_max_norm, tau_scale);
    DLC_LAUNCH_CHECK(ctx, "tau_scale_kernel");
    return DLC_OK;
}

extern "C" double dlc_cosine_score_error_bound_any_plan(int64_t d) {
    if (d < BK) return 0.0;
    const double nk = (double)(d / BK);
    const double steps = std::max(2.0 * nk + 2.0, nk * 0.5 + 8.0);
    return SCORE_STEP_EPS * 1.01 * steps + 3.7e-12;
}
```

deeploopcloser_amd/engine.py:

```python
import collections
import contextlib
import ctypes as C
import weakref

import numpy as np
import torch

from . import _lib as L

_TORCH_TO_DLC = {torch.bfloat16: L.DLC_BF16, torch.float16: L.DLC_F16, torch.float32: L.DLC_F32,
                 torch.float64: L.DLC_F64, torch.int8: L.DLC_I8}
_NAME_TO_TORCH = {"bf16": torch.bfloat16, "bfloat16": torch.bfloat16, "f16": torch.float16, "fp16": torch.float16,
                  "float16": torch.float16, "f32": torch.float32, "float32": torch.float32, "f64": torch.float64,
                  "float64": torch.float64}

SCRATCH_BYTES = 256 << 20
K_STEP = 64


TopK = collections.namedtuple("TopK", "scores idx scores_f64 status")


_RAW_STREAM = getattr(torch._C, "_cuda_getCurrentRawStream", None)

# ... 804 lines not shown
    _SEQ_DTYPES = {torch.float64: L.DLC_F64, torch.float32: L.DLC_F32, torch.int64: L.DLC_I64}

    def _score_matrix(self, who, scores, n, nothing):
        if not isinstance(scores, torch.Tensor) or scores.dim() != 2 or scores.dtype not in self._SEQ_DTYPES:
            raise ValueError("%s: scores must be a 2-D float64, float32 or int64 tensor" % who)
        if scores.device != self.device:
            raise ValueError("%s: scores must be on %s" % (who, self.device))
        rows = scores.shape[0]
        n = scores.shape[1] if n is None else int(n)
        if rows < 1 or n < 1 or n > scores.shape[1]:
            raise ValueError("%s: scores [%d, %d] with n=%d: nothing to %s" % (who, rows, scores.shape[1], n, nothing))
        if scores.stride(1) != 1 or (rows > 1 and scores.stride(0) < n):
            scores = scores.contiguous()
        return scores, rows, n, scores.stride(0) if rows > 1 else max(n, scores.stride(0))

    def sequence_topk(self, scores, length, offsets, k=None, row0=0, n=None, limit0=None, limit_step=0, lower_is_better=False,
                      dense=False, poison=None):
        scores, rows, n, ld = self._score_matrix("sequence_topk", scores, n, "search")
        off = np.ascontiguousarray(np.asarray(offsets), dtype=np.int32)
        if off.ndim != 2 or off.shape[1] != int(length) or not np.array_equal(off, np.asarray(offsets)):
            raise ValueError("sequence_topk: offsets must be an integer table [n_slopes, L=%d]" % int(length))
        if not 0 <= int(row0) < rows:
            raise ValueError("sequence_topk: row0=%d outside 0..%d" % (row0, rows - 1))
        if k is None and not dense:
            raise ValueError("sequence_topk: neither lists (k) nor the dense scores were asked for")
        if k is not None and not 1 <= k <= L.DLC_MAX_K:
            raise ValueError("sequence_topk: k=%d outside 1..%d" % (k, L.DLC_MAX_K))
        if poison is not None:
            self._check_out("poison", poison, (1,), torch.int64)
        out_dtype = torch.int64 if scores.dtype == torch.int64 else torch.float64
        ro = rows - int(row0)
        o_s = o_i = o_v = seq = ws = None
        if k is not None:
            o_s = torch.empty((ro, k), dtype=out_dtype, device=self.device)
            o_i = torch.empty((ro, k), dtype=torch.int64, device=self.device)
            o_v = torch.empty((ro, k), dtype=torch.int32, device=self.device)
            need = self.lib.dlc_sequence_topk_workspace_bytes(rows, n, int(length), off.shape[0], int(k))
            if need == 0:
                raise ValueError("sequence_topk: L=%d, %d slopes, k=%d, n=%d outside the supported sizes" % (length, off.shape[0], k, n))
            ws = self.workspace("sequence_topk", need)
        if dense:
            seq = torch.empty((ro, n), dtype=out_dtype, device=self.device)
        self._check(self.lib.dlc_sequence_topk(
            self.ctx, self._SEQ_DTYPES[scores.dtype], _ptr(scores), rows, int(row0), n, ld, n if limit0 is None else int(limit0),
            int(limit_step), int(length), off.shape[0], off.ctypes.data_as(C.POINTER(C.c_int32)), int(bool(lower_is_better)),
            1 if k is None else int(k), _ptr(o_s), _ptr(o_i), _ptr(o_v), _ptr(seq), n, _ptr(poison), _ptr(ws),
            ws.numel() if ws is not None else 0, self._stream()))
        return o_s, o_i, o_v, seq

    def contrast_rows(self, scores, radius, n=None, limit0=None, limit_step=0, out=None):
        scores, rows, n, ld = self._score_matrix("contrast_rows", scores, n, "normalise")
        if not 1 <= int(radius) <= 32:
            raise ValueError("contrast_rows: radius=%d outside 1..32" % int(radius))
        out = self._rows_out("contrast_rows: out", out, rows, n, torch.float64, "a float64",
                             float("nan") if limit0 is not None or limit_step != 0 else None, wider=True)
        ld_out = out.stride(0) if rows > 1 else n
        self._check(self.lib.dlc_contrast_rows(self.ctx, self._SEQ_DTYPES[scores.dtype], _ptr(scores), rows, n, ld,
                                                n if limit0 is None else int(limit0), int(limit_step), int(radius), _ptr(out),
                                                ld_out, self._stream()))
        self._wrote(out)
        return out[:, :n]

    def peak_topk_rows(self, scores, k, suppress, n=None, limit0=None, limit_step=0, lower_is_better=False, absent=None,
                       poison=None):
        scores, rows, n, ld = self._score_matrix("peak_topk_rows", scores, n, "pick from")
        k, suppress = int(k), int(suppress)
        if not 1 <= k <= L.DLC_MAX_K:
            raise ValueError("peak_topk_rows: k=%d outside 1..%d" % (k, L.DLC_MAX_K))
        if not 0 <= suppress < 1 << 63:
            raise ValueError("peak_topk_rows: suppress=%d outside 0..2^63-1" % suppress)
        is_int = scores.dtype == torch.int64
        if absent is not None and not is_int:
            raise ValueError("peak_topk_rows: absent is for int64 rows (a float row marks absence with NaN)")
        if poison is not None:
            if is_int:
                raise ValueError("peak_topk_rows: the poison word marks fp64 outputs; int64 rows have none")
            self._check_out("poison", poison, (1,), torch.int64)
        o_s = torch.empty((rows, k), dtype=torch.int64 if is_int else torch.float64, device=self.device)
        o_i = torch.empty((rows, k), dtype=torch.int64, device=self.device)
        need = self.lib.dlc_peak_topk_rows_workspace_bytes(rows, n, k)
        if need == 0:
            raise ValueError("peak_topk_rows: rows=%d, n=%d outside the supported sizes" % (rows, n))
        ws = self.workspace("peak_topk_rows", need)
        self._check(self.lib.dlc_peak_topk_rows(
            self.ctx, self._SEQ_DTYPES[scores.dtype], _ptr(scores), rows, n, ld, n if limit0 is None else int(limit0),
            int(limit_step), int(bool(lower_is_better)), suppress, int(absent is not None), 0 if absent is None else int(absent),
            k, _ptr(o_s), _ptr(o_i), _ptr(poison), _ptr(ws), ws.numel(), self._stream()))
        return o_s, o_i

    @staticmethod
    def stored_width(d):
        return (d + K_STEP - 1) // K_STEP * K_STEP

    def normalize(self, x, dtype="bf16", center=False, out=None):
        dt = torch_dtype(dtype)
        if dt not in (torch.bfloat16, torch.float16):
            raise ValueError("stored descriptor dtype must be bf16 or fp16")
        if x.dtype not in (torch.float32, torch.float64):
            raise ValueError("normalize: float32 or float64 input")
        x = x.contiguous()
        n, d = x.shape
        ldd = self.stored_width(d)
        if out is None:
            out = torch.empty((n, ldd), dtype=dt, device=self.device)
        elif out.shape != (n, ldd) or out.dtype != dt or not out.is_contiguous() or out.device != self.device:
            raise ValueError("normalize: out must be a contiguous [%d, %d] %s tensor on %s" % (n, ldd, dt, self.device))
        if n > 0:
            self._check(self.lib.dlc_l2_normalize_rows(self.ctx, _TORCH_TO_DLC[x.dtype], _ptr(x), n, d, x.stride(0),
                                                        1 if center else 0, _TORCH_TO_DLC[dt], _ptr(out), ldd,
                                                        self._stream()))
        self._wrote(out)
        out._dlc_unit_rows = out._version
        return out

    @staticmethod
    def unit_rows(t):
        return getattr(t, "_dlc_unit_rows", None) == t._version

    def max_row_norm(self, rows, out=None):
        if rows.dim() != 2 or rows.dtype not in (torch.bfloat16, torch.float16) or rows.stride(1) != 1:
            raise ValueError("max_row_norm: stored rows [n, d] (bf16 / fp16, contiguous rows)")
        if out is None:
            out = torch.zeros((1,), dtype=torch.float32, device=self.device)
        else:
            self._check_out("out", out, (1,), torch.float32)
        if rows.shape[0] > 0:
            self._check(self.lib.dlc_max_row_norm(self.ctx, _TORCH_TO_DLC[rows.dtype], _ptr(rows), rows.shape[0],
                                                   rows.stride(0), rows.shape[1], _ptr(out), self._stream()))
        return out

    def cosine_tau_scale(self, q, db_max_norm=None, out=None, stream=None):
        if q.dim() != 2 or q.dtype not in (torch.bfloat16, torch.float16) or q.stride(1) != 1:
            raise ValueError("cosine_tau_scale: stored queries [Q, d] (bf16 / fp16, contiguous rows)")
        if out is None:
            out = torch.empty((q.shape[0],), dtype=torch.float32, device=self.device)
        else:
            self._check_out("out", out, (q.shape[0],), torch.float32)
        if db_max_norm is not None:
            self._check_out("db_max_norm", db_max_norm, (1,), torch.float32)
        st = C.c_void_p(stream.cuda_stream) if stream is not None else self._stream()
        if q.shape[0] > 0:
            self._check(self.lib.dlc_cosine_tau_scale(self.ctx, _TORCH_TO_DLC[q.dtype], _ptr(q), q.shape[0], q.stride(0),
                                                       q.shape[1], _ptr(db_max_norm), _ptr(out), st))
        return out

    def _check_stored(self, q, db):
        if q.dim() != 2 or db.dim() != 2 or q.shape[1] != db.shape[1]:
            raise ValueError("stored descriptors must be 2-D with one width")
        if q.dtype != db.dtype or q.dtype not in (torch.bfloat16, torch.float16):
            raise ValueError("stored descriptors must both be bf16 or both fp16")
        if q.stride(1) != 1 or db.stride(1) != 1:
            raise ValueError("stored descriptor rows must be contiguous")

    def match_topk(self, q, db, k, row_offset=0, out=None, details=False, older_than=None, tau_scale=None):
        self._check_stored(q, db)
        nq, d = q.shape
        if tau_scale is not None:
            self._check_out("tau_scale", tau_scale, (nq,), torch.float32)
        n = db.shape[0]
        need = self.lib.dlc_cosine_topk_workspace_bytes(nq, n, d, k)
        if need == 0:
            raise ValueError("match_topk: k=%d outside 1..%d (or empty operand)" % (k, L.DLC_MAX_K))
        ws = self.workspace("topk", need)
        if out is None:
            scores = torch.empty((nq, k), dtype=torch.float32, device=self.device)
            idx = torch.empty((nq, k), dtype=torch.int64, device=self.device)
        else:
            scores = self._check_out("out[0] (scores)", out[0], (nq, k), torch.float32)
            idx = self._check_out("out[1] (idx)", out[1], (nq, k), torch.int64)
        s64 = torch.empty((nq, k), dtype=torch.float64, device=self.device) if details else None
        status = torch.empty((nq,), dtype=torch.int32, device=self.device) if details else None
        if older_than is None:
            self._check(self.lib.dlc_cosine_topk(self.ctx, _TORCH_TO_DLC[q.dtype], _ptr(q), nq, q.stride(0), _ptr(db), n,
                                                  db.stride(0), d, k, row_offset, _ptr(scores), _ptr(s64), _ptr(idx),
                                                  _ptr(status), _ptr(tau_scale), _ptr(ws), ws.numel(), self._stream()))
        else:
            self._check(self.lib.dlc_cosine_topk_older(self.ctx, _TORCH_TO_DLC[q.dtype], _ptr(q), nq, q.stride(0), _ptr(db), n,
                                                        db.stride(0), d, k, row_offset, int(older_than), _ptr(scores),
                                                        _ptr(s64), _ptr(idx), _ptr(status), _ptr(tau_scale), _ptr(ws),
                                                        ws.numel(), self._stream()))
        return TopK(scores, idx, s64, status) if details else (scores, idx)

    def topk_workspace_bytes(self, nq, n, d, k):
        need = self.lib.dlc_cosine_topk_workspace_bytes(nq, n, d, k)
        if need == 0:
            raise ValueError("k=%d outside 1..%d (or empty operand)" % (k, L.DLC_MAX_K))
        return need

    def score_error_bound(self, nq, n, d, k):
        return float(self.lib.dlc_cosine_score_error_bound(nq, n, d, k))

    def score_error_bound_any_plan(self, d):
        return float(self.lib.dlc_cosine_score_error_bound_any_plan(d))

    def score_groups(self, q, db, k, ws, stream=None):
        self._check_stored(q, db)
        self._check_ws(ws)
        st = C.c_void_p(stream.cuda_stream) if stream is not None else self._stream()
        self._check(self.lib.dlc_cosine_score_groups(self.ctx, _TORCH_TO_DLC[q.dtype], _ptr(q), q.shape[0], q.stride(0),
                                                      _ptr(db), db.shape[0], db.stride(0), q.shape[1], k, _ptr(ws),
                                                      ws.numel(), st))

    def select_topk(self, q, db, k, ws, scores, idx, row_offset=0, coop=False, stream=None, scores_f64=None, status=None,
                    tau_scale=None):
        self._check_stored(q, db)
        self._check_ws(ws)
        self._check_out("scores", scores, (q.shape[0], k), torch.float32)
        self._check_out("idx", idx, (q.shape[0], k), torch.int64)
        if scores_f64 is not None:
            self._check_out("scores_f64", scores_f64, (q.shape[0], k), torch.float64)
        if status is not None:
            self._check_out("status", status, (q.shape[0],), torch.int32)
        st = C.c_void_p(stream.cuda_stream) if stream is not None else self._stream()
        self._check(self.lib.dlc_cosine_select_topk(self.ctx, _TORCH_TO_DLC[q.dtype], _ptr(q), q.shape[0], q.stride(0),
                                                     _ptr(db), db.shape[0], db.stride(0), q.shape[1], k, row_offset,
                                                     _ptr(scores), _ptr(scores_f64), _ptr(idx), _ptr(status),
                                                     _ptr(tau_scale), _ptr(ws), ws.numel(),
                                                     L.DLC_SELECT_COOP if coop else 0, st))

    def _check_ws(self, ws):
        if not isinstance(ws, torch.Tensor) or ws.dtype != torch.uint8 or not ws.is_contiguous() or ws.device != self.device:
            raise ValueError("workspace must be a contiguous uint8 tensor on %s" % (self.device,))

    def groups_per_query(self, k):
        kg = self.lib.dlc_cosine_groups_per_query(k)
        if kg == 0:
            raise ValueError("k=%d outside 1..%d" % (k, L.DLC_MAX_K))
        return kg

    def select_groups(self, q, db, k, ws, grp_ids, grp_max, coop=False, stream=None):
        self._check_stored(q, db)
        self._check_ws(ws)
        kg = self.groups_per_query(k)
        self._check_out("grp_ids", grp_ids, (q.shape[0], kg), torch.int32)
        self._check_out("grp_max", grp_max, (q.shape[0], kg + 1), torch.float32)
        st = C.c_void_p(stream.cuda_stream) if stream is not None else self._stream()
        self._check(self.lib.dlc_cosine_select_groups(self.ctx, _TORCH_TO_DLC[q.dtype], _ptr(q), q.shape[0], q.stride(0),
                                                       _ptr(db), db.shape[0], db.stride(0), q.shape[1], k, _ptr(ws),
                                                       ws.numel(), _ptr(grp_ids), _ptr(grp_max),
                                                       L.DLC_SELECT_COOP if coop else 0, st))

    def rescore_topk(self, q, db, k, grp_ids, grp_max, scores_f64, idx, bound=None, all_max=None, row_offset=0, coop=False,
                     stream=None, tau_scale=None):
        self._check_stored(q, db)
        kg = self.groups_per_query(k)
        self._check_out("grp_ids", grp_ids, (q.shape[0], kg), torch.int32)
        self._check_out("grp_max", grp_max, (q.shape[0], kg + 1), torch.float32)
        self._check_out("scores_f64", scores_f64, (q.shape[0], k), torch.float64)
        self._check_out("idx", idx, (q.shape[0], k), torch.int64)
        if bound is not None:
            self._check_out("bound", bound, (q.shape[0],), torch.float32)
        if all_max is not None:
            self._check_out("all_max", all_max, (all_max.shape[0], q.shape[0], kg + 1), torch.float32)
        st = C.c_void_p(stream.cuda_stream) if stream is not None else self._stream()
        parts = 0 if all_max is None else all_max.shape[0]
        self._check(self.lib.dlc_cosine_rescore_topk(self.ctx, _TORCH_TO_DLC[q.dtype], _ptr(q), q.shape[0], q.stride(0),
                                                      _ptr(db), db.shape[0], db.stride(0), q.shape[1], k, row_offset,
                                                      _ptr(grp_ids), _ptr(grp_max), _ptr(all_max), parts, _ptr(scores_f64),
                                                      _ptr(idx), _ptr(bound), _ptr(tau_scale),
                                                      L.DLC_SELECT_COOP if coop else 0, st))

    def exhaustive_topk(self, q, db, k, ws, lower, tau, status, scores_f64, idx, scores=None, row_offset=0, stream=None,
                        tau_scale=None):
        self._check_stored(q, db)
        self._check_ws(ws)
        nq = q.shape[0]
        self._check_out("lower", lower, (nq,), torch.float64)
        self._check_out("status", status, (nq,), torch.int32)
        self._check_out("scores_f64", scores_f64, (nq, k), torch.float64)
        self._check_out("idx", idx, (nq, k), torch.int64)
        if scores is not None:
            self._check_out("scores", scores, (nq, k), torch.float32)
        st = C.c_void_p(stream.cuda_stream) if stream is not None else self._stream()
        self._check(self.lib.dlc_cosine_exhaustive_topk(self.ctx, _TORCH_TO_DLC[q.dtype], _ptr(q), nq, q.stride(0), _ptr(db),
                                                         db.shape[0], db.stride(0), q.shape[1], k, row_offset, _ptr(lower), 1,
                                                         float(tau), _ptr(tau_scale), _ptr(status), _ptr(scores),
                                                         _ptr(scores_f64), _ptr(idx), _ptr(ws), ws.numel(), st))

    def topk_merge_packed(self, gathered, nq, k, out, bound=None, tau=0.0, scores_f64=None, status=None, tau_scale=None):
        parts = gathered.shape[0]
        self._check_out("gathered", gathered, (parts, nq * k * 16), torch.uint8)
        base = gathered.data_ptr()
        o_s = self._check_out("out[0] (scores)", out[0], (nq, k), torch.float32)
        o_i = self._check_out("out[1] (idx)", out[1], (nq, k), torch.int64)
        if bound is not None:
            self._check_out("bound", bound, (nq,), torch.float32)
        if scores_f64 is not None:
            self._check_out("scores_f64", scores_f64, (nq, k), torch.float64)
        if status is not None:
            self._check_out("status", status, (nq,), torch.int32)
        self._check(self.lib.dlc_topk_merge_strided(self.ctx, C.c_void_p(base + nq * k * 8), nq * k * 2,
                                                     C.c_void_p(base), nq * k * 2, parts, nq, k, _ptr(bound), float(tau),
                                                     _ptr(tau_scale), _ptr(o_s), _ptr(scores_f64), _ptr(o_i), _ptr(status),
                                                     self._stream()))
        return o_s, o_i

    def topk_keep_older(self, scores, idx, limit0, k):
        scores, idx = scores.contiguous(), idx.contiguous()
        if scores.dim() != 2 or idx.shape != scores.shape or scores.dtype != torch.float32 or idx.dtype != torch.int64:
            raise ValueError("topk_keep_older: scores float32 / idx int64 of one shape [B, kk]")
        b, kk = scores.shape
        o_s = torch.empty((b, k), dtype=torch.float32, device=self.device)
        o_i = torch.empty((b, k), dtype=torch.int64, device=self.device)
        self._check(self.lib.dlc_topk_keep_older(self.ctx, _ptr(scores), _ptr(idx), b, kk, int(limit0), int(k), _ptr(o_s),
                                                  _ptr(o_i), self._stream()))
        return o_s, o_i

    def topk_merge(self, scores_f64, idx, out=None, details=False):
        scores_f64, idx = scores_f64.contiguous(), idx.contiguous()
        if scores_f64.dim() != 3 or idx.shape != scores_f64.shape or scores_f64.dtype != torch.float64 or \
                idx.dtype != torch.int64:
            raise ValueError("topk_merge: scores float64 / idx int64 of one shape [parts, Q, k]")
        parts, nq, k = scores_f64.shape
        if out is None:
            o_s = torch.empty((nq, k), dtype=torch.float32, device=self.device)
            o_i = torch.empty((nq, k), dtype=torch.int64, device=self.device)
        else:
            o_s = self._check_out("out[0] (scores)", out[0], (nq, k), torch.float32)
            o_i = self._check_out("out[1] (idx)", out[1], (nq, k), torch.int64)
        o_64 = torch.empty((nq, k), dtype=torch.float64, device=self.device) if details else None
        self._check(self.lib.dlc_topk_merge(self.ctx, _ptr(scores_f64), _ptr(idx), parts, nq, k, _ptr(o_s), _ptr(o_64),
                                             _ptr(o_i), self._stream()))
        return TopK(o_s, o_i, o_64, None) if details else (o_s, o_i)

    def cosine_scores(self, q, db):
        self._check_stored(q, db)
        nq, d = q.shape
        n = db.shape[0]
        s = torch.empty((nq, n), dtype=torch.float32, device=self.device)
        need = self.lib.dlc_cosine_scores_workspace_bytes(nq, n, d)
        ws = self.workspace("scores", need) if need else None
        self._check(self.lib.dlc_cosine_scores(self.ctx, _TORCH_TO_DLC[q.dtype], _ptr(q), nq, q.stride(0), _ptr(db), n,
                                                db.stride(0), d, _ptr(s), s.stride(0), _ptr(ws) if need else None,
# ... 66 lines not shown
```

deeploopcloser_amd/matching.py:

```python
import numpy as np
import torch

from .engine import default_engine, torch_dtype


def encode(frames, network):
    return network.transform(frames)


def flatten_frame_descriptors(h, patches=30):
    h = h if isinstance(h, torch.Tensor) else torch.from_numpy(np.asarray(h))
    return h.reshape(h.shape[0] // patches, patches * h.shape[1])


class KeyframeDatabase:

    def __init__(self, descriptors, dtype="bf16", center=False, row_offset=0, device=None, stored=False,
                 capacity=None, _norm_bound=None):
        self.engine = default_engine(device)
        self.dtype = torch_dtype(dtype)
        self.center = center
        self.row_offset = int(row_offset)
        self.norm_bound = None
        if stored:
            d = descriptors.to(self.engine.device)
            if d.dtype != self.dtype:
                raise ValueError("stored descriptors have dtype %s, expected %s" % (d.dtype, self.dtype))
            rows = d
            if _norm_bound is not None:
                self.norm_bound = _norm_bound[0]
            elif d.shape[0] > 0 and not self.engine.unit_rows(d):
                self.norm_bound = self.engine.max_row_norm(
                    d, out=torch.full((1,), 1.005, dtype=torch.float32, device=self.engine.device))
        else:
            rows = self.engine.normalize(self._as_float(descriptors), self.dtype, center)
        self._n = rows.shape[0]
        if capacity is not None and capacity > self._n:
            self._store = torch.empty((int(capacity), rows.shape[1]), dtype=self.dtype, device=self.engine.device)
            self._store[:self._n] = rows
        else:
            self._store = rows

    @classmethod
    def empty(cls, dim, capacity=4096, dtype="bf16", center=False, row_offset=0, device=None):
        if dim < 1 or capacity < 1:
            raise ValueError("KeyframeDatabase.empty: dim and capacity must be positive")
        eng = default_engine(device)
        dt = torch_dtype(dtype)
        if dt not in (torch.bfloat16, torch.float16):
            raise ValueError("stored descriptor dtype must be bf16 or fp16")
        none = torch.empty((0, eng.stored_width(dim)), dtype=dt, device=eng.device)
        return cls(none, dtype=dt, center=center, row_offset=row_offset, device=device, stored=True, capacity=capacity)

    def _as_float(self, descriptors):
        x = self.engine.to_device(descriptors)
        if x.dtype not in (torch.float32, torch.float64):
            x = x.to(torch.float32)
        return x

    @property
    def rows(self):
        return self._store[:self._n]

    @property
    def capacity(self):
        return self._store.shape[0]

    def __len__(self):
        return self._n

    def reserve(self, capacity):
        if capacity > self.capacity:
            grown = torch.empty((int(capacity), self._store.shape[1]), dtype=self.dtype, device=self.engine.device)
            grown[:self._n] = self._store[:self._n]
            self._store = grown

    def append(self, descriptors):
        x = self._as_float(descriptors)
        if x.dim() != 2 or self.engine.stored_width(x.shape[1]) != self._store.shape[1]:
            raise ValueError("append: descriptors must be [B, dim] with the database's width")
        b = x.shape[0]
        if self._n + b > self.capacity:
            self.reserve(max(2 * self.capacity, self._n + b))
        self.engine.normalize(x, self.dtype, self.center, out=self._store[self._n:self._n + b])
        first = self.row_offset + self._n
        self._n += b
        return first, first + b

    def prefix(self, n):
        if not 0 <= n <= self._n:
            raise ValueError("prefix: n=%d outside 0..%d" % (n, self._n))
        return KeyframeDatabase(self._store[:n], dtype=self.dtype, center=self.center, row_offset=self.row_offset,
                                device=self.engine.device, stored=True, _norm_bound=(self.norm_bound,))

    def save(self, path):
        np.savez(path, rows_u16=self.rows.view(torch.int16).cpu().numpy().view(np.uint16),
                 dtype=np.array(str(self.dtype).replace("torch.", "")), center=np.array(bool(self.center)),
                 row_offset=np.array(self.row_offset, dtype=np.int64), format=np.array("dlc-keyframes-v1"))

    @classmethod
    def load(cls, path, device=None, row_offset=None):
        z = np.load(path)
        if str(z["format"]) != "dlc-keyframes-v1":
            raise ValueError("%s is not a dlc-keyframes-v1 file" % path)
        dt = torch_dtype(str(z["dtype"]))
        rows = torch.from_numpy(z["rows_u16"].view(np.int16).copy()).view(dt)
        return cls(rows, dtype=dt, center=bool(z["center"]), device=device, stored=True,
                   row_offset=int(z["row_offset"]) if row_offset is None else row_offset)

    def prepare_queries(self, queries):
        x = self.engine.to_device(queries)
        if x.dtype in (torch.bfloat16, torch.float16):
            return x
        return self.engine.normalize(self._as_float(x), self.dtype, self.center)

    def tau_scale(self, q, out=None, stream=None):
        if self.norm_bound is None and self.engine.unit_rows(q):
            return None
        return self.engine.cosine_tau_scale(q, self.norm_bound, out=out, stream=stream)

    def match_topk(self, queries, k, out=None, details=False):
        q = self.prepare_queries(queries)
        return self.engine.match_topk(q, self.rows, k, self.row_offset, out=out, details=details, tau_scale=self.tau_scale(q))

    def match(self, queries):
        return self.engine.cosine_scores(self.prepare_queries(queries), self.rows)

    def scores_f64(self, queries, limit0=None, limit_step=0, out=None):
        return self.engine.cosine_score_rows(self.prepare_queries(queries), self.rows, limit0=limit0, limit_step=limit_step,
                                             out=out)

    def score_keys(self, queries, limit0=None, limit_step=0, out=None):
        return self.engine.cosine_score_rows(self.prepare_queries(queries), self.rows, limit0=limit0, limit_step=limit_step,
                                             keys=True, out_keys=out)


class MatchPipeline:

    def __init__(self, db, k, depth=2, group=None, queries_per_batch=None, force_collectives=False):
        import torch.distributed as dist
        self.db, self.k, self.depth = db, int(k), int(depth)
        self.engine = db.engine
        dev = self.engine.device
        self.s_select = self.engine.side_stream
        self.group = group
        self.world = dist.get_world_size(group) if dist.is_initialized() else 1
        if force_collectives and not dist.is_initialized():
            raise ValueError("MatchPipeline(force_collectives=True) needs an initialised torch.distributed process group")
        self._force_collectives = bool(force_collectives)
        self._slots = []
        self._count = 0
        self._nq = queries_per_batch
        self.all_gather = dist.all_gather_into_tensor
        self._norm_bound = db.norm_bound
        if self.sharded:
            r = db.norm_bound.clone() if db.norm_bound is not None else \
                torch.full((1,), 1.005, dtype=torch.float32, device=dev)
            dist.all_reduce(r, op=dist.ReduceOp.MAX, group=group)
            self._norm_bound = r
        self.resolved_batches = 0
        self.dropped_batches = 0
        self.time_collectives = False
        self._coll_events = []

    @property
    def sharded(self):
        return self.world > 1 or self._force_collectives

    def _slot(self, i, nq, d):
        while len(self._slots) <= i:
            self._slots.append(None)
        s = self._slots[i]
        if s is None or s["nq"] != nq or s["n"] != len(self.db):
            if s is not None and s["busy"]:
                s["done"].synchronize()
            dev = self.engine.device
            eng, k = self.engine, self.k
            need = eng.topk_workspace_bytes(nq, len(self.db), d, k)
            s = {"nq": nq, "n": len(self.db), "ws": torch.empty(need, dtype=torch.uint8, device=dev),
                 "scores": torch.empty((nq, k), dtype=torch.float32, device=dev),
                 "idx": torch.empty((nq, k), dtype=torch.int64, device=dev),
                 "scored": torch.cuda.Event(), "done": torch.cuda.Event(), "busy": False, "fetched": True, "q": None,
                 "rows": None, "ts_buf": torch.empty((nq,), dtype=torch.float32, device=dev), "ts": None}
            if self.sharded:
                kg = eng.groups_per_query(k)
                nb = nq * k * 16
                s["pack"] = torch.empty(nb, dtype=torch.uint8, device=dev)
                s["p_idx"] = s["pack"][:nq * k * 8].view(torch.int64).view(nq, k)
                s["p_s64"] = s["pack"][nq * k * 8:].view(torch.float64).view(nq, k)
                s["g_pack"] = torch.empty((self.world, nb), dtype=torch.uint8, device=dev)
                s["grp_ids"] = torch.empty((nq, kg), dtype=torch.int32, device=dev)
                s["grp_max"] = torch.empty((nq, kg + 1), dtype=torch.float32, device=dev)
                s["g_max"] = torch.empty((self.world, nq, kg + 1), dtype=torch.float32, device=dev)
                s["bound"] = torch.empty((nq,), dtype=torch.float32, device=dev)
                s["m_s64"] = torch.empty((nq, k), dtype=torch.float64, device=dev)
                s["status"] = torch.empty((nq,), dtype=torch.int32, device=dev)
                s["flag"] = torch.zeros((nq,), dtype=torch.int32).pin_memory()
                s["tau"] = eng.score_error_bound_any_plan(d)
            self._slots[i] = s
        return s

    def submit(self, queries):
        import torch.distributed as dist
        q = self.db.prepare_queries(queries)
        eng = self.engine
        i = self._count % self.depth
        s = self._slot(i, q.shape[0], q.shape[1])
        main = torch.cuda.current_stream(eng.device)
        if s["busy"]:
            if not s["fetched"]:
                s["done"].synchronize()
                if self.sharded and bool(s["flag"].any()):
                    raise RuntimeError("MatchPipeline.submit: batch %d was never fetched and its merge did not certify %d "
                                       "quer%s -- call result(ticket) within `depth` submissions (the exhaustive round runs "
                                       "there)" % (self._count - self.depth, int((s["flag"] != 0).sum()),
                                                   "y" if int((s["flag"] != 0).sum()) == 1 else "ies"))
                self.dropped_batches += 1
            main.wait_event(s["done"])
        s["q"] = q
        rows = s["rows"] = self.db.rows
        eng.score_groups(q, rows, self.k, s["ws"], stream=main)
        s["scored"].record(main)
        self.s_select.wait_event(s["scored"])
        with torch.cuda.stream(self.s_select):
            if not self.sharded and self._norm_bound is None and eng.unit_rows(q):
                ts = s["ts"] = None
            else:
                ts = s["ts"] = eng.cosine_tau_scale(q, self._norm_bound, out=s["ts_buf"], stream=self.s_select)
            if not self.sharded:
                eng.select_topk(q, rows, self.k, s["ws"], s["scores"], s["idx"],
                                row_offset=self.db.row_offset, coop=True, stream=self.s_select, tau_scale=ts)
            else:
                eng.select_groups(q, rows, self.k, s["ws"], s["grp_ids"], s["grp_max"], coop=True,
                                  stream=self.s_select)
                ev = [torch.cuda.Event(enable_timing=True) for _ in range(4)] if self.time_collectives else None
                if ev:
                    ev[0].record(self.s_select)
                self.all_gather(s["g_max"].view(-1, s["g_max"].shape[-1]), s["grp_max"], group=self.group)
                if ev:
                    ev[1].record(self.s_select)
                eng.rescore_topk(q, rows, self.k, s["grp_ids"], s["grp_max"], s["p_s64"], s["p_idx"], bound=s["bound"],
                                 all_max=s["g_max"], row_offset=self.db.row_offset, coop=True, stream=self.s_select,
                                 tau_scale=ts)
                if ev:
                    ev[2].record(self.s_select)
                self.all_gather(s["g_pack"].view(-1), s["pack"], group=self.group)
                if ev:
                    ev[3].record(self.s_select)
                    self._coll_events.append(ev)
                eng.topk_merge_packed(s["g_pack"], q.shape[0], self.k, out=(s["scores"], s["idx"]), bound=s["bound"],
                                      tau=s["tau"], scores_f64=s["m_s64"], status=s["status"], tau_scale=ts)
                s["flag"].copy_(s["status"], non_blocking=True)
            s["done"].record(self.s_select)
        s["busy"] = True
        s["fetched"] = False
        self._count += 1
        return self._count - 1

    def _resolve(self, s):
        import torch.distributed as dist
        eng, q, k = self.engine, s["q"], self.k
        with torch.cuda.stream(self.s_select):
            lower = s["m_s64"][:, k - 1].contiguous()
            eng.exhaustive_topk(q, s["rows"], k, s["ws"], lower, s["tau"], s["status"], s["p_s64"], s["p_idx"],
                                row_offset=self.db.row_offset, stream=self.s_select, tau_scale=s["ts"])
            self.all_gather(s["g_pack"].view(-1), s["pack"], group=self.group)
            eng.topk_merge_packed(s["g_pack"], q.shape[0], k, out=(s["scores"], s["idx"]), scores_f64=s["m_s64"])
            s["done"].record(self.s_select)
        s["done"].synchronize()
        self.resolved_batches += 1

    def result(self, ticket):
        if not self._count - self.depth <= ticket < self._count:
            raise ValueError("MatchPipeline.result: ticket %d is not in flight (last submitted: %d, depth %d)"
                             % (ticket, self._count - 1, self.depth))
        s = self._slots[ticket % self.depth]
# ... 29 lines not shown
```

include/dlc.h:

```cpp
#ifndef DLC_H_
#define DLC_H_

#include <stddef.h>
#include <stdint.h>

#ifdef __cplusplus
extern "C" {
#endif

#define DLC_ABI_VERSION 17

typedef struct dlc_ctx dlc_ctx;

typedef enum dlc_status {
    DLC_OK = 0,
    DLC_ERR_BAD_ARG = -1,
    DLC_ERR_BAD_SHAPE = -2,
    DLC_ERR_UNSUPPORTED = -3,
    DLC_ERR_HIP = -4,
    DLC_ERR_WORKSPACE = -5
} dlc_status;

typedef enum dlc_dtype {
    DLC_BF16 = 0,
    DLC_F16 = 1,
    DLC_F32 = 2,
    DLC_F64 = 3,
    DLC_I8 = 4,
    DLC_U8 = 5,
    DLC_I64 = 6
} dlc_dtype;

typedef enum dlc_act {
    DLC_ACT_NONE = 0,
    DLC_ACT_SIGMOID = 1,
    DLC_ACT_RELU = 2
} dlc_act;

typedef enum dlc_blayout {
    DLC_B_KN = 0,
    DLC_B_NK = 1
} dlc_blayout;

int dlc_abi_version(void);
int dlc_create(int device, dlc_ctx** out);
int dlc_destroy(dlc_ctx* ctx);
const char* dlc_last_error(const dlc_ctx* ctx);
const char* dlc_status_string(int status);

int dlc_gemm_bias_act(dlc_ctx* ctx, int dtype, int blayout, int act,
                      int64_t M, int64_t N, int64_t K,
                      const void* A, int64_t lda, const void* B, int64_t ldb,
                      const void* bias, void* C, int64_t ldc, void* stream);

int dlc_bias_act(dlc_ctx* ctx, int dtype, int act, int64_t M, int64_t N,
                 const void* A, int64_t lda, const void* bias, void* C, int64_t ldc, void* stream);

size_t dlc_sdav_encode_workspace_bytes(int64_t rows, const int64_t* dims, int n_layers, int dtype);
int dlc_sdav_encode(dlc_ctx* ctx, int dtype, int64_t rows, int n_layers, const int64_t* dims,
                    const void* x, const void* const* W, const void* const* b,
                    void* out, void* workspace, size_t workspace_bytes, void* stream);

size_t dlc_sdav_split_panels_bytes(int n_layers, const int64_t* dims);
int dlc_sdav_split_prepare(dlc_ctx* ctx, int n_layers, const int64_t* dims, const double* const* W, void* panels,
                           size_t panels_bytes, void* stream);
size_t dlc_sdav_encode_split_workspace_bytes(int64_t rows, const int64_t* dims, int n_layers);
int dlc_sdav_encode_split(dlc_ctx* ctx, int64_t rows, int n_layers, const int64_t* dims, const double* x,
                          const void* panels, const double* const* b, double* out, void* workspace,
                          size_t workspace_bytes, void* stream);

size_t dlc_sdav_train_workspace_bytes(int64_t batch, int64_t patches, const int64_t* dims, int n_layers, int layer);
int dlc_sdav_train_step(dlc_ctx* ctx, int layer, int64_t batch, int64_t patches, int n_layers, const int64_t* dims,
                        const double* x, const double* const* masks, double* const* W, double* const* b_enc,
                        double* b_dec, double sparse_level, double sparse_penalty, double consecutive_penalty,
                        double learning_rate, double* loss_out, void* workspace, size_t workspace_bytes,
                        void* stream);

int dlc_random_mask_f64(dlc_ctx* ctx, double* mask, int64_t n, int64_t n_zeros, uint64_t seed, uint64_t counter,
                        void* stream);

int dlc_salt_pepper_mask_f64(dlc_ctx* ctx, double* zeros, double* ones, int64_t n, int64_t n_zeros, uint64_t seed,
                             uint64_t counter, void* stream);
int dlc_da_corrupt_f64(dlc_ctx* ctx, const double* x, const double* zeros, const double* ones, int64_t rows, int64_t cols,
                       double* out, int64_t ldo, void* stream);
size_t dlc_da_train_workspace_bytes(int64_t batch, int64_t patches, int64_t in_units, int64_t hidden_units);
int dlc_da_train_step(dlc_ctx* ctx, int64_t batch, int64_t patches, int64_t in_units, int64_t hidden_units, const double* x,
                      const double* x_tilde, double* W, double* b_enc, double* b_dec, double sparse_level,
                      double sparse_penalty, double consecutive_penalty, double learning_rate, double* loss_out,
                      void* workspace, size_t workspace_bytes, void* stream);

int dlc_rgb_to_gray_u8(dlc_ctx* ctx, const uint8_t* rgb, int64_t n_pixels, uint8_t* gray, void* stream);
int dlc_extract_patches(dlc_ctx* ctx, const uint8_t* gray, int64_t frames, int H, int W,
                        const int32_t* key_points, int P, int patch_size, int out_dtype, void* out,
                        void* stream);

size_t dlc_harris_keypoints_workspace_bytes(int64_t frames, int H, int W);
int dlc_harris_keypoints_u8(dlc_ctx* ctx, const uint8_t* gray, int64_t frames, int H, int W, int n,
                            int32_t* points, int64_t* responses, int32_t* counts, void* workspace,
                            size_t workspace_bytes, void* stream);

int dlc_im2col_nhwc_f64(dlc_ctx* ctx, const double* x, int64_t n, int h, int w, int c,
                        int kh, int kw, int stride, int pad_top, int pad_left, int oh, int ow,
                        double* cols, void* stream);
int dlc_conv2d_nhwc_f64(dlc_ctx* ctx, const double* x, int64_t n, int h, int w, int c,
                        const double* kernel, const double* bias, int kh, int kw, int cout,
                        int stride, int pad_top, int pad_left, int oh, int ow, int act,
                        double* out, void* stream);
int dlc_space_to_depth_nhwc_f64(dlc_ctx* ctx, const double* x, int64_t n, int h, int w, int c, int s,
                                double* y, void* stream);
int dlc_maxpool3x3s2_nhwc_f64(dlc_ctx* ctx, const double* x, int64_t n, int h, int w, int c,
                              double* y, void* stream);
int dlc_minmax_quant_gather_i8(dlc_ctx* ctx, const double* const* segs, const int64_t* seg_sizes, int n_segs,
                               int64_t n, const int64_t* cols, int64_t n_cols, double* minmax,
                               int8_t* out, void* stream);
int dlc_cnnvtl_frame_minmax_init(dlc_ctx* ctx, uint64_t* keys, int64_t n, void* stream);
int dlc_conv2d_nhwc_f64_stats(dlc_ctx* ctx, const double* x, int64_t n, int h, int w, int c,
                              const double* kernel, const double* bias, int kh, int kw, int cout,
                              int stride, int pad_top, int pad_left, int oh, int ow, int act,
                              double* out, uint64_t* frame_keys, void* stream);
int dlc_quant_gather_i8(dlc_ctx* ctx, const double* const* segs, const int64_t* seg_sizes, int n_segs,
                        int64_t n, const int64_t* cols, int64_t n_cols, const uint64_t* keys, double* minmax,
                        int8_t* out, void* stream);

size_t dlc_cnnvtl_split_panels_bytes(int n_layers, const int32_t* geom);
int dlc_cnnvtl_split_prepare(dlc_ctx* ctx, int n_layers, const int32_t* geom, const double* const* W, void* panels,
                             size_t panels_bytes, void* stream);
size_t dlc_cnnvtl_encode_split_workspace_bytes(int64_t n, int h, int w, int c, int n_layers, const int32_t* geom);
int dlc_cnnvtl_encode_split(dlc_ctx* ctx, int dtype, const void* x, int64_t n, int h, int w, int c, int s2d, int n_layers,
                            const int32_t* geom, const void* panels, const double* const* b, const int64_t* cols,
                            int64_t n_cols, int8_t* out, float* const* feats, int32_t* status, void* workspace,
                            size_t workspace_bytes, void* stream);
int dlc_cnnvtl_layers_split(dlc_ctx* ctx, const float* x, int64_t n, int h, int w, int c, int n_layers, const int32_t* geom,
                            int layer_a, int layer_b, const void* panels, const double* const* b, float* const* feats,
                            int32_t* status, void* workspace, size_t workspace_bytes, void* stream);

size_t dlc_sdav_range_words(int64_t H);
int dlc_sdav_distinctive_score(dlc_ctx* ctx, const double* dataset, int64_t rows, int64_t H,
                               double mu, double sigma, double* score, uint64_t* range, void* stream);
#define DLC_SIM_FORCE_F64 1
#define DLC_SIM_NO_HOST_SYNC 2
size_t dlc_sdav_similarity_workspace_bytes(int64_t N, int64_t P, int64_t H, int flags, int64_t chunk_bytes);
int dlc_sdav_similarity_matrix(dlc_ctx* ctx, const double* desc, int64_t N, int64_t P, int64_t H,
                               const double* score, double a, double b,
                               double* out_f64, int64_t* out_i64, int flags, int64_t chunk_bytes,
                               const uint64_t* range, int64_t* stats, uint8_t* direct_pairs,
                               void* workspace, size_t workspace_bytes, void* stream);
size_t dlc_sdav_stream_state_bytes(int64_t capacity, int64_t P, int64_t H);
int dlc_sdav_stream_init(dlc_ctx* ctx, void* state, size_t state_bytes, int64_t capacity, int64_t P, int64_t H,
                         double lo, double hi, const double* col_centre, void* stream);
int dlc_sdav_stream_append(dlc_ctx* ctx, void* state, size_t state_bytes, int64_t capacity, int64_t P, int64_t H,
                           const double* desc, int64_t n_old, int64_t n_total, const double* score, void* stream);
int dlc_sdav_stream_query(dlc_ctx* ctx, void* state, size_t state_bytes, int64_t capacity, int64_t P, int64_t H,
                          const double* desc, int64_t f, const double* score, double a, double b, double* row_out,
                          int64_t* stats, void* stream);
size_t dlc_sdav_stream_query_batch_workspace_bytes(int64_t capacity, int64_t P, int64_t n_queries);
int dlc_sdav_stream_query_batch(dlc_ctx* ctx, void* state, size_t state_bytes, int64_t capacity, int64_t P, int64_t H,
                                const double* desc, int64_t f_first, int64_t n_queries, const double* score, double a,
                                double b, double* rows_out, int64_t ld_rows, int64_t* stats, void* workspace,
                                size_t workspace_bytes, void* stream);
int dlc_sdav_stream_query_batch_staged(dlc_ctx* ctx, void* state, size_t state_bytes, int64_t capacity, int64_t P, int64_t H,
                                       const double* desc, int64_t f_first, int64_t n_queries, const double* score, double a,
                                       double b, double* rows_out, int64_t ld_rows, int64_t* stats, void* workspace,
                                       size_t workspace_bytes, int stage, void* stream);
int dlc_topk_rows_f64(dlc_ctx* ctx, const double* scores, int64_t rows, int64_t ld, int64_t limit0, int64_t limit_step,
                      int k, double* out_scores, int64_t* out_idx, const int64_t* poison, void* stream);
int dlc_cnnvtl_distance_matrix(dlc_ctx* ctx, const int8_t* desc, int64_t N, int64_t D, int64_t ldd,
                               int64_t* out, void* stream);
size_t dlc_cnnvtl_distance_topk_workspace_bytes(int64_t Q, int64_t N, int64_t D, int k);
int dlc_cnnvtl_distance_topk(dlc_ctx* ctx, const int8_t* queries, int64_t Q, int64_t ldq,
                             const int8_t* db, int64_t N, int64_t ldd, int64_t D,
                             int64_t limit0, int64_t limit_step, int k,
                             int64_t* out_dist, int64_t* out_idx,
                             void* workspace, size_t workspace_bytes, void* stream);
int dlc_cnnvtl_distance_rows(dlc_ctx* ctx, const int8_t* queries, int64_t Q, int64_t ldq,
                             const int8_t* db, int64_t N, int64_t ldd, int64_t D,
                             int64_t limit0, int64_t limit_step,
                             int64_t* out, int64_t ld_out, void* stream);

size_t dlc_sequence_topk_workspace_bytes(int64_t rows, int64_t n, int L, int n_slopes, int k);
int dlc_sequence_topk(dlc_ctx* ctx, int dtype, const void* scores, int64_t rows, int64_t row0, int64_t n, int64_t ld,
                      int64_t limit0, int64_t limit_step, int L, int n_slopes, const int32_t* offsets,
                      int lower_is_better, int k, void* out_scores, int64_t* out_idx, int32_t* out_slope,
                      void* seq_out, int64_t ld_out, const int64_t* poison, void* workspace, size_t workspace_bytes,
                      void* stream);

int dlc_contrast_rows(dlc_ctx* ctx, int dtype, const void* scores, int64_t rows, int64_t n, int64_t ld,
                      int64_t limit0, int64_t limit_step, int radius,
                      double* out, int64_t ld_out, void* stream);

size_t dlc_peak_topk_rows_workspace_bytes(int64_t rows, int64_t n, int k);
int dlc_peak_topk_rows(dlc_ctx* ctx, int dtype , const void* scores,
                       int64_t rows, int64_t n, int64_t ld, int64_t limit0, int64_t limit_step,
                       int lower_is_better, int64_t suppress, int has_absent, int64_t absent, int k,
                       void* out_scores, int64_t* out_idx, const int64_t* poison,
                       void* workspace, size_t workspace_bytes, void* stream);

int dlc_l2_normalize_rows(dlc_ctx* ctx, int src_dtype, const void* src, int64_t n, int64_t d, int64_t lds,
                          int center, int dst_dtype, void* dst, int64_t ldd, void* stream);
#define DLC_MAX_K 128
size_t dlc_cosine_topk_workspace_bytes(int64_t q, int64_t n, int64_t d, int k);
int dlc_cosine_topk(dlc_ctx* ctx, int dtype, const void* Q, int64_t q, int64_t ldq,
                    const void* DB, int64_t n, int64_t lddb, int64_t d, int k, int64_t row_offset,
                    float* out_scores, double* out_scores_f64, int64_t* out_idx, int32_t* out_status,
                    const float* tau_scale, void* workspace, size_t workspace_bytes, void* stream);
int dlc_max_row_norm(dlc_ctx* ctx, int dtype, const void* rows, int64_t n, int64_t ld, int64_t d, float* max_norm,
                     void* stream);
int dlc_cosine_tau_scale(dlc_ctx* ctx, int dtype, const void* Q, int64_t q, int64_t ldq, int64_t d,
                         const float* db_max_norm, float* tau_scale, void* stream);
int dlc_cosine_topk_older(dlc_ctx* ctx, int dtype, const void* Q, int64_t q, int64_t ldq,
                          const void* DB, int64_t n, int64_t lddb, int64_t d, int k, int64_t row_offset, int64_t limit0,
                          float* out_scores, double* out_scores_f64, int64_t* out_idx, int32_t* out_status,
                          const float* tau_scale, void* workspace, size_t workspace_bytes, void* stream);
double dlc_cosine_score_error_bound(int64_t q, int64_t n, int64_t d, int k);
double dlc_cosine_score_error_bound_any_plan(int64_t d);
#define DLC_SELECT_COOP 1
int dlc_cosine_score_groups(dlc_ctx* ctx, int dtype, const void* Q, int64_t q, int64_t ldq,
                            const void* DB, int64_t n, int64_t lddb, int64_t d, int k,
                            void* workspace, size_t workspace_bytes, void* stream);
int dlc_cosine_select_topk(dlc_ctx* ctx, int dtype, const void* Q, int64_t q, int64_t ldq,
                           const void* DB, int64_t n, int64_t lddb, int64_t d, int k, int64_t row_offset,
                           float* out_scores, double* out_scores_f64, int64_t* out_idx, int32_t* out_status,
                           const float* tau_scale, void* workspace, size_t workspace_bytes, int flags, void* stream);
int dlc_cosine_groups_per_query(int k);
int dlc_cosine_select_groups(dlc_ctx* ctx, int dtype, const void* Q, int64_t q, int64_t ldq,
                             const void* DB, int64_t n, int64_t lddb, int64_t d, int k,
                             void* workspace, size_t workspace_bytes,
                             int32_t* group_ids, float* group_max, int flags, void* stream);
int dlc_cosine_rescore_topk(dlc_ctx* ctx, int dtype, const void* Q, int64_t q, int64_t ldq,
                            const void* DB, int64_t n, int64_t lddb, int64_t d, int k, int64_t row_offset,
                            const int32_t* group_ids, const float* group_max,
                            const float* all_group_max, int parts,
                            double* out_scores_f64, int64_t* out_idx, float* out_bound, const float* tau_scale,
                            int flags, void* stream);
int dlc_cosine_exhaustive_topk(dlc_ctx* ctx, int dtype, const void* Q, int64_t q, int64_t ldq,
                               const void* DB, int64_t n, int64_t lddb, int64_t d, int k, int64_t row_offset,
                               const double* lower, int64_t lower_stride, double tau, const float* tau_scale,
                               int32_t* status, float* out_scores, double* out_scores_f64, int64_t* out_idx,
                               void* workspace, size_t workspace_bytes, void* stream);
int dlc_topk_keep_older(dlc_ctx* ctx, const float* scores, const int64_t* idx, int64_t rows, int kk,
                        int64_t limit0, int k, float* out_scores, int64_t* out_idx, void* stream);
int dlc_topk_merge(dlc_ctx* ctx, const double* scores_f64, const int64_t* idx, int parts, int64_t q, int k,
                   float* out_scores, double* out_scores_f64, int64_t* out_idx, void* stream);
int dlc_topk_merge_strided(dlc_ctx* ctx, const double* scores_f64, int64_t score_part_stride,
                           const int64_t* idx, int64_t idx_part_stride, int parts, int64_t q, int k,
                           const float* bound, double tau, const float* tau_scale,
                           float* out_scores, double* out_scores_f64, int64_t* out_idx, int32_t* out_status,
                           void* stream);
size_t dlc_cosine_scores_workspace_bytes(int64_t q, int64_t n, int64_t d);
int dlc_cosine_scores(dlc_ctx* ctx, int dtype, const void* Q, int64_t q, int64_t ldq,
                      const void* DB, int64_t n, int64_t lddb, int64_t d,
                      float* S, int64_t lds, void* workspace, size_t workspace_bytes, void* stream);

int dlc_cosine_score_rows(dlc_ctx* ctx, int dtype ,
                          const void* Q, int64_t q, int64_t ldq,
                          const void* DB, int64_t n, int64_t lddb, int64_t d,
                          int64_t limit0, int64_t limit_step,
                          double* out_scores, int64_t* out_keys, int64_t ld_out, void* stream);

int dlc_host_to_device(dlc_ctx* ctx, void* dst_device, const void* src_host, size_t bytes, void* stream);
int dlc_device_to_host(dlc_ctx* ctx, void* dst_host, const void* src_device, size_t bytes, void* stream);
int dlc_set_host_threads(dlc_ctx* ctx, int threads);

int dlc_set_scratch(dlc_ctx* ctx, void* scratch, size_t bytes);

#define DLC_PROFILE_RING 256
int dlc_set_profiling(dlc_ctx* ctx, int enabled);
int dlc_profile_gemm_ms(dlc_ctx* ctx, float* out_ms, int capacity);

#ifdef __cplusplus
}
#endif
#endif
```

Baseline: 125,500 query-frames/s.

## Fuse tau-scale norm and exhaustive fallback into fused finish kernel

Adds bound variants of cosine top-k that compute each query's norm-based tau scale inside the fused finish kernel, using its last wave, instead of a separate tau_scale launch. Uncertified queries in the 512-thread fused path now run the exhaustive rescoring inline rather than being flagged for a later pass. A sync in the finish prologue is also dropped. matching.py skips the tau scale entirely for unit-norm queries with no norm bound. This removes extra kernel launches and host round-trips, at the cost of more kernel complexity and possible long-tail blocks.

Measured after the change: 126,100 query-frames/s, median of 6. About the same (+0.5%).

```diff
diff --git a/deeploopcloser_amd/_lib.py b/deeploopcloser_amd/_lib.py
--- a/deeploopcloser_amd/_lib.py
+++ b/deeploopcloser_amd/_lib.py
@@ -10,7 +10,7 @@
 DLC_ACT_NONE, DLC_ACT_SIGMOID, DLC_ACT_RELU = 0, 1, 2
 DLC_B_KN, DLC_B_NK = 0, 1
 DLC_MAX_K = 128
-DLC_ABI_VERSION = 17
+DLC_ABI_VERSION = 18
 DLC_SELECT_COOP = 1
 DLC_SIM_FORCE_F64, DLC_SIM_NO_HOST_SYNC = 1, 2
 
@@ -96,6 +96,10 @@
     "dlc_cosine_tau_scale": (_int, [_vp, _int, _vp, _i64, _i64, _i64, _vp, _vp, _vp]),
     "dlc_cosine_topk_older": (_int, [_vp, _int, _vp, _i64, _i64, _vp, _i64, _i64, _i64, _int, _i64, _i64, _vp, _vp, _vp, _vp, _vp,
                                     _vp, _sz, _vp]),
+    "dlc_cosine_topk_bound": (_int, [_vp, _int, _vp, _i64, _i64, _vp, _i64, _i64, _i64, _int, _i64, _vp, _vp, _vp, _vp, _vp, _vp,
+                                    _sz, _vp]),
+    "dlc_cosine_topk_bound_older": (_int, [_vp, _int, _vp, _i64, _i64, _vp, _i64, _i64, _i64, _int, _i64, _i64, _vp, _vp, _vp,
+                                          _vp, _vp, _vp, _sz, _vp]),
     "dlc_cosine_score_error_bound": (_dbl, [_i64, _i64, _i64, _int]),
     "dlc_cosine_score_error_bound_any_plan": (_dbl, [_i64]),
     "dlc_cosine_score_groups": (_int, [_vp, _int, _vp, _i64, _i64, _vp, _i64, _i64, _i64, _int, _vp, _sz, _vp]),
diff --git a/deeploopcloser_amd/csrc/cosine_topk.hip b/deeploopcloser_amd/csrc/cosine_topk.hip
--- a/deeploopcloser_amd/csrc/cosine_topk.hip
+++ b/deeploopcloser_amd/csrc/cosine_topk.hip
@@ -417,6 +417,7 @@
 }
 
 constexpr int FIN_THREADS = 512;
+constexpr int FIN_LV = 16;
 __host__ __device__ inline size_t fin_lds_fixed(int kg) {
     return (size_t)kg * (GROUPS_PER_HALF * 8 + GROUP * (8 + 8 + 4)) + (size_t)(kg + 1) * 8 + 64;
 }
@@ -542,6 +543,47 @@
     double acc[1];
     rescore_rows_f64<Tag, 1, 4>(qrow, rows, d, lane, acc);
     return acc[0];
+}
+
+template <typename Tag>
+__device__ __forceinline__ float row_norm_up(const char* __restrict__ row, int d, int lane) {
+    float acc = 0.f;
+    for (int c = lane * 8; c < d; c += 512) {
+        const u32x4_t v = *(const u32x4_t*)(row + (long long)c * 2);
+#pragma unroll
+        for (int j = 0; j < 4; ++j) {
+            float lo, hi;
+            if constexpr (__is_same(Tag, dlc_bf16_tag)) {
+                lo = __uint_as_float(v[j] << 16);
+                hi = __uint_as_float(v[j] & 0xffff0000u);
+            } else {
+                lo = dlc_f16_bits_to_f32((unsigned short)(v[j] & 0xffffu));
+                hi = dlc_f16_bits_to_f32((unsigned short)(v[j] >> 16));
+            }
+            acc = fmaf(lo, lo, acc);
+            acc = fmaf(hi, hi, acc);
+        }
+    }
+#pragma unroll
+    for (int m = 32; m >= 1; m >>= 1) acc += __shfl_xor(acc, m, 64);
+    const float nrm = sqrtf(acc) * 1.001f;
+    return (nrm <= 3.0e38f) ? nrm : INFINITY;
+}
+
+__device__ __forceinline__ float tau_scale_of(float nq, float R) {
+    const float prod = nq * R * (1.0f / 1.01f) * 1.000001f;
+    return (prod <= 3.0e38f) ? fmaxf(prod, 1.0f) : INFINITY;
+}
+
+template <typename Tag>
+__global__ __launch_bounds__(256) void tau_scale_kernel(const char* __restrict__ Q, long long ldq_b, long long q, int d,
+                                                        const float* __restrict__ db_max_norm, float* __restrict__ out) {
+    const int lane = threadIdx.x & 63;
+    const long long qi = (long long)blockIdx.x * 4 + (threadIdx.x >> 6);
+    if (qi >= q) return;
+    const float nq = row_norm_up<Tag>(Q + qi * ldq_b, d, lane);
+    const float s = tau_scale_of(nq, db_max_norm ? *db_max_norm : 1.005f);
+    if (lane == 0) out[qi] = s;
 }
 
 __device__ __forceinline__ double scaled_tau(double tau, const float* __restrict__ tau_scale, int qi) {
@@ -561,6 +603,8 @@
     int* status;
     double tau;
     const float* tau_scale;
+    int scale_here;
+    const float* db_norm_bound;
     int* grp_ids;
     float* grp_max;
     const float* all_max;
@@ -580,6 +624,97 @@
     return lim < 0 ? 0 : (lim < n ? lim : n);
 }
 
+struct ExhaustiveArgs {
+    const float* gmax; long long ldg; long long ng;
+    const char* Q; long long ldq_b; const char* DB; long long lddb_b;
+    long long n; int d; int k; long long row_offset;
+    const double* lower; long long lower_stride;
+    float* out_s; double* out_s64; long long* out_i;
+    int* status;
+    double tau;
+    const float* tau_scale;
+    int limited; long long limit0;
+};
+constexpr int EXH_BATCH = 64;
+constexpr int EXH_POOL = EXH_BATCH * GROUP + DLC_MAX_K;
+
+template <typename Tag, int RS_UNROLL = 4>
+__device__ __forceinline__ void exhaustive_topk_body(const ExhaustiveArgs& a, double lower) {
+    const int qi = blockIdx.x;
+    __shared__ long long pk[EXH_POOL];
+    __shared__ double ps[EXH_POOL];
+    __shared__ int pid[EXH_POOL];
+    __shared__ int qlist[FIN_THREADS];
+    __shared__ int wcnt[FIN_THREADS / 64];
+    __shared__ int sel[DLC_MAX_K];
+    const int tid = threadIdx.x, lane = tid & 63, w = tid >> 6, k = a.k;
+    const long long n_vis = visible_rows(a.n, a.limited, a.limit0, qi);
+    const long long ng_vis = a.limited ? (n_vis + GROUP - 1) / GROUP : a.ng;
+    const double tau = scaled_tau(a.tau, a.tau_scale, qi);
+    double theta = lower - tau;
+    if (theta != theta) theta = -INFINITY;
+    int cnt = 0;
+    const char* qrow = a.Q + (long long)qi * a.ldq_b;
+    for (long long c0 = 0; c0 < ng_vis; c0 += FIN_THREADS) {
+        const long long g = c0 + tid;
+        const bool qual = g < ng_vis && (double)a.gmax[(long long)qi * a.ldg + g] >= theta;
+        const unsigned long long bal = __ballot(qual);
+        if (lane == 0) wcnt[w] = __popcll(bal);
+        __syncthreads();
+        int base = 0, nqual = 0;
+#pragma unroll
+        for (int ww = 0; ww < FIN_THREADS / 64; ++ww) {
+            base += ww < w ? wcnt[ww] : 0;
+            nqual += wcnt[ww];
+        }
+        if (qual) qlist[base + __popcll(bal & ((1ull << lane) - 1ull))] = (int)g;
+        __syncthreads();
+        for (int b0 = 0; b0 < nqual; b0 += EXH_BATCH) {
+            const int nb = min(EXH_BATCH, nqual - b0);
+            for (int s = w; s < nb; s += FIN_THREADS / 64) {
+                const long long row0 = (long long)qlist[b0 + s] * GROUP;
+                const char* rows[GROUP];
+#pragma unroll
+                for (int r = 0; r < GROUP; ++r) rows[r] = a.DB + (row0 + r < a.n ? row0 + r : a.n - 1) * a.lddb_b;
+                double acc[GROUP];
+                rescore8_f64<Tag, RS_UNROLL>(qrow, rows, a.d, lane, acc);
+#pragma unroll
+                for (int r = 0; r < GROUP; ++r)
+                    if (lane == r) {
+                        const bool ok = row0 + r < n_vis;
+                        ps[cnt + s * GROUP + r] = ok ? acc[r] : -INFINITY;
+                        pk[cnt + s * GROUP + r] = ok ? f64_key(acc[r]) : KEY64_EMPTY;
+                        pid[cnt + s * GROUP + r] = (int)(row0 + r);
+                    }
+            }
+            for (int e = tid; e < k; e += FIN_THREADS) sel[e] = -1;
+            __syncthreads();
+            const int m = cnt + nb * GROUP;
+            rank_select64(pk, pid, m, k, sel);
+            __syncthreads();
+            long long tk = KEY64_EMPTY; double ts = -INFINITY; int ti = -1;
+            if (tid < k && sel[tid] >= 0) { const int c = sel[tid]; tk = pk[c]; ts = ps[c]; ti = pid[c]; }
+            const unsigned long long have = __ballot(tid < k && sel[tid] >= 0);
+            if (lane == 0) wcnt[w] = __popcll(have);
+            __syncthreads();
+            if (tid < k) { pk[tid] = tk; ps[tid] = ts; pid[tid] = ti; }
+            cnt = 0;
+#pragma unroll
+            for (int ww = 0; ww < FIN_THREADS / 64; ++ww) cnt += wcnt[ww];
+            __syncthreads();
+            if (cnt == k && ps[k - 1] - tau > theta) theta = ps[k - 1] - tau;
+        }
+        __syncthreads();
+    }
+    for (int e = tid; e < k; e += FIN_THREADS) {
+        const bool ok = e < cnt;
+        if (a.out_s) a.out_s[(long long)qi * k + e] = ok ? (float)ps[e] : -INFINITY;
+        if (a.out_s64) a.out_s64[(long long)qi * k + e] = ok ? ps[e] : -INFINITY;
+        a.out_i[(long long)qi * k + e] = ok ? (long long)pid[e] + a.row_offset : -1;
+    }
+    if (tid == 0) a.status[qi] = 2;
+}
+
 template <typename Tag, int THREADS, int RS_UNROLL, int MODE>
 __device__ __forceinline__ void finish_topk_body(const FinishArgs& a) {
     extern __shared__ __attribute__((aligned(16))) char dsm[];
@@ -587,7 +722,7 @@
     constexpr int FIN_THREADS = THREADS;
     constexpr int GPH = GROUPS_PER_HALF;
     const int kg = a.kg, k = a.k;
-    const double tau = scaled_tau(a.tau, a.tau_scale, (int)blockIdx.x);
+    double tau = scaled_tau(a.tau, a.tau_scale, (int)blockIdx.x);
     const long long n = visible_rows(a.n, a.limited, a.limit0, (int)blockIdx.x);
     const long long ng = a.limited ? (n + GROUP - 1) / GROUP : a.ng;
     if (n <= 0) {
@@ -617,11 +752,17 @@
     unsigned* misc = (unsigned*)(sel2 + kg + 1);
     const int qi = blockIdx.x, tid = threadIdx.x, lane = tid & 63, w = tid >> 6;
     float* tv = a.tv_in_lds ? (float*)(dsm + fin_lds_fixed(kg)) : a.tmax + (long long)qi * a.ldt;
+    const bool scale_here = MODE == FIN_FUSED && a.scale_here && !a.tau_scale;
+    if (scale_here && w == FIN_WAVES - 1) {
+        const float sc = tau_scale_of(row_norm_up<Tag>(a.Q + (long long)qi * a.ldq_b, a.d, lane),
+                                      a.db_norm_bound ? *a.db_norm_bound : 1.005f);
+        if (lane == 0) misc[10] = __float_as_uint(sc);
+    }
     if (a.tv_in_lds)
         for (int e = tid; e < a.nh; e += FIN_THREADS) tv[e] = a.tmax[(long long)qi * a.ldt + e];
     for (int e = tid; e <= kg; e += FIN_THREADS) { sel[e] = -1; sel2[e] = -1; }
-    if (tid < 16) misc[tid] = 0u;
-    __syncthreads();
+    if (tid >= 8 && tid < 16 && tid != 10) misc[tid] = 0u;
+    if (MODE == FIN_RESCORE || a.tv_in_lds) __syncthreads();
     int kg2;
     unsigned bkey = 0u;
     if constexpr (MODE != FIN_RESCORE) {
@@ -631,7 +772,7 @@
         const int chunk = (nh + FIN_WAVES - 1) / FIN_WAVES;
         const int lo_e = w * chunk, hi_e = min(nh, lo_e + chunk);
         unsigned bh = 0, bl = 0;
-        constexpr int LV = 16;
+        constexpr int LV = FIN_LV;
         if ((THREADS == 512 || MODE == FIN_GROUPS) && chunk <= 64 * LV) {
             unsigned vk[LV];
 #pragma unroll
@@ -720,6 +861,7 @@
         if (tid == 0) a.grp_max[(long long)qi * W + kg] = bkey ? key_f32(bkey) : -INFINITY;
         return;
     }
+    if (scale_here) tau = a.tau * (double)__uint_as_float(misc[10]);
     if (tid < kg2) {
         const int c = sel2[tid];
         int g = c < 0 ? -1 : (int)key_id(ckey[c]);
@@ -858,10 +1000,26 @@
         }
     }
     if constexpr (MODE == FIN_FUSED) {
-        if (tid == 0) {
-            const int c = sel[k - 1];
-            const bool cert = bkey == 0u || (c >= 0 && cs64[c] > (double)key_f32(bkey) + tau);
-            a.status[qi] = cert ? 0 : 1;
+        const int c = sel[k - 1];
+        const double kth = c >= 0 ? cs64[c] : -INFINITY;
+        const bool cert = bkey == 0u || (c >= 0 && kth > (double)key_f32(bkey) + tau);
+        if constexpr (THREADS == 512) {
+            if (cert) {
+                if (tid == 0) a.status[qi] = 0;
+                return;
+            }
+            __syncthreads();
+            ExhaustiveArgs e;
+            e.gmax = a.gmax; e.ldg = a.ldg; e.ng = a.ng;
+            e.Q = a.Q; e.ldq_b = a.ldq_b; e.DB = a.DB; e.lddb_b = a.lddb_b;
+            e.n = a.n; e.d = a.d; e.k = k; e.row_offset = a.row_offset;
+            e.lower = nullptr; e.lower_stride = 0;
+            e.out_s = a.out_s; e.out_s64 = a.out_s64; e.out_i = a.out_i;
+            e.status = a.status; e.tau = tau; e.tau_scale = nullptr;
+            e.limited = a.limited; e.limit0 = a.limit0;
+            exhaustive_topk_body<Tag, RS_UNROLL>(e, kth);
+        } else {
+            if (tid == 0) a.status[qi] = cert ? 0 : 1;
         }
     }
 }
@@ -873,96 +1031,6 @@
 template <typename Tag, int RS_UNROLL, int MODE>
 __global__ __launch_bounds__(256) __attribute__((amdgpu_waves_per_eu(5))) void finish_topk_coop_kernel(FinishArgs a) {
     finish_topk_body<Tag, 256, RS_UNROLL, MODE>(a);
-}
-
-struct ExhaustiveArgs {
-    const float* gmax; long long ldg; long long ng;
-    const char* Q; long long ldq_b; const char* DB; long long lddb_b;
-    long long n; int d; int k; long long row_offset;
-    const double* lower; long long lower_stride;
-    float* out_s; double* out_s64; long long* out_i;
-    int* status;
-    double tau;
-    const float* tau_scale;
-    int limited; long long limit0;
-};
-constexpr int EXH_BATCH = 64;
-constexpr int EXH_POOL = EXH_BATCH * GROUP + DLC_MAX_K;
-
-template <typename Tag, int RS_UNROLL = 4>
-__device__ __forceinline__ void exhaustive_topk_body(const ExhaustiveArgs& a, double lower) {
-    const int qi = blockIdx.x;
-    __shared__ long long pk[EXH_POOL];
-    __shared__ double ps[EXH_POOL];
-    __shared__ int pid[EXH_POOL];
-    __shared__ int qlist[FIN_THREADS];
-    __shared__ int wcnt[FIN_THREADS / 64];
-    __shared__ int sel[DLC_MAX_K];
-    const int tid = threadIdx.x, lane = tid & 63, w = tid >> 6, k = a.k;
-    const long long n_vis = visible_rows(a.n, a.limited, a.limit0, qi);
-    const long long ng_vis = a.limited ? (n_vis + GROUP - 1) / GROUP : a.ng;
-    const double tau = scaled_tau(a.tau, a.tau_scale, qi);
-    double theta = lower - tau;
-    int cnt = 0;
-    const char* qrow = a.Q + (long long)qi * a.ldq_b;
-    for (long long c0 = 0; c0 < ng_vis; c0 += FIN_THREADS) {
-        const long long g = c0 + tid;
-        const bool qual = g < ng_vis && (double)a.gmax[(long long)qi * a.ldg + g] >= theta;
-        const unsigned long long bal = __ballot(qual);
-        if (lane == 0) wcnt[w] = __popcll(bal);
-        __syncthreads();
-        int base = 0, nqual = 0;
-#pragma unroll
-        for (int ww = 0; ww < FIN_THREADS / 64; ++ww) {
-            base += ww < w ? wcnt[ww] : 0;
-            nqual += wcnt[ww];
-        }
-        if (qual) qlist[base + __popcll(bal & ((1ull << lane) - 1ull))] = (int)g;
-        __syncthreads();
-        for (int b0 = 0; b0 < nqual; b0 += EXH_BATCH) {
-            const int nb = min(EXH_BATCH, nqual - b0);
-            for (int s = w; s < nb; s += FIN_THREADS / 64) {
-                const long long row0 = (long long)qlist[b0 + s] * GROUP;
-                const char* rows[GROUP];
-#pragma unroll
-                for (int r = 0; r < GROUP; ++r) rows[r] = a.DB + (row0 + r < a.n ? row0 + r : a.n - 1) * a.lddb_b;
-                double acc[GROUP];
-                rescore8_f64<Tag, RS_UNROLL>(qrow, rows, a.d, lane, acc);
-#pragma unroll
-                for (int r = 0; r < GROUP; ++r)
-                    if (lane == r) {
-                        const bool ok = row0 + r < n_vis;
-                        ps[cnt + s * GROUP + r] = ok ? acc[r] : -INFINITY;
-                        pk[cnt + s * GROUP + r] = ok ? f64_key(acc[r]) : KEY64_EMPTY;
-                        pid[cnt + s * GROUP + r] = (int)(row0 + r);
-                    }
-            }
-            for (int e = tid; e < k; e += FIN_THREADS) sel[e] = -1;
-            __syncthreads();
-            const int m = cnt + nb * GROUP;
-            rank_select64(pk, pid, m, k, sel);
-            __syncthreads();
-            long long tk = KEY64_EMPTY; double ts = -INFINITY; int ti = -1;
-            if (tid < k && sel[tid] >= 0) { const int c = sel[tid]; tk = pk[c]; ts = ps[c]; ti = pid[c]; }
-            const unsigned long long have = __ballot(tid < k && sel[tid] >= 0);
-            if (lane == 0) wcnt[w] = __popcll(have);
-            __syncthreads();
-            if (tid < k) { pk[tid] = tk; ps[tid] = ts; pid[tid] = ti; }
-            cnt = 0;
-#pragma unroll
-            for (int ww = 0; ww < FIN_THREADS / 64; ++ww) cnt += wcnt[ww];
-            __syncthreads();
-            if (cnt == k && ps[k - 1] - tau > theta) theta = ps[k - 1] - tau;
-        }
-        __syncthreads();
-    }
-    for (int e = tid; e < k; e += FIN_THREADS) {
-        const bool ok = e < cnt;
-        if (a.out_s) a.out_s[(long long)qi * k + e] = ok ? (float)ps[e] : -INFINITY;
-        if (a.out_s64) a.out_s64[(long long)qi * k + e] = ok ? ps[e] : -INFINITY;
-        a.out_i[(long long)qi * k + e] = ok ? (long long)pid[e] + a.row_offset : -1;
-    }
-    if (tid == 0) a.status[qi] = 2;
 }
 
 template <typename Tag>
@@ -1441,7 +1509,7 @@
 }
 
 struct WsLayout {
-    size_t gmax, tmax, part, status, s64, rs_ids, rs_max, rs_scores, rs_idx, rs_bound, total;
+    size_t gmax, tmax, part, status, s64, tscale, rs_ids, rs_max, rs_scores, rs_idx, rs_bound, total;
     long long ldg, ldt, ldp;
     int kg;
     SplitPlan sp;
@@ -1492,6 +1560,7 @@
     if (w.sp.nsplit > 1 || w.dense) o += dlc::align_up((size_t)w.sp.nsplit * q * w.ldp * 4, 256);
     w.status = o; o += dlc::align_up((size_t)q * 4, 256);
     w.s64 = o; o += dlc::align_up((size_t)q * k * 8, 256);
+    w.tscale = o; o += dlc::align_up((size_t)q * 4, 256);
     w.rparts = w.dense ? 1 : rescore_parts(q, d, w.kg, k);
     w.rs_ids = w.rs_max = w.rs_scores = w.rs_idx = w.rs_bound = o;
     if (w.rparts > 1) {
@@ -1671,7 +1740,8 @@
 template <typename Tag, int THREADS, int RS_UNROLL, int MODE>
 int launch_finish(dlc_ctx* ctx, FinishArgs f, int64_t q, bool small_lds, hipStream_t st) {
     size_t dsm = fin_lds_fixed(f.kg);
-    f.tv_in_lds = MODE != FIN_RESCORE && !small_lds && (size_t)f.nh * 4 <= 96 * 1024;
+    const bool regs = (THREADS == 512 || MODE == FIN_GROUPS) && dlc::cdiv((int64_t)f.nh, (int64_t)(THREADS / 64)) <= 64 * FIN_LV;
+    f.tv_in_lds = MODE != FIN_RESCORE && !small_lds && !regs && (size_t)f.nh * 4 <= 96 * 1024;
     if (f.tv_in_lds) dsm += (size_t)f.nh * 4;
     dsm = dlc::align_up(dsm, 16);
     void (*fk)(FinishArgs);
@@ -1726,11 +1796,39 @@
     return DLC_OK;
 }
 
+int launch_tau_scale(dlc_ctx* ctx, int dtype, const char* Q, long long ldq_b, int64_t q, int64_t d, const float* db_max_norm,
+                     float* out, hipStream_t st) {
+    const unsigned grid = (unsigned)dlc::cdiv(q, 4);
+    if (dtype == DLC_BF16)
+        hipLaunchKernelGGL(tau_scale_kernel<dlc_bf16_tag>, dim3(grid), dim3(256), 0, st, Q, ldq_b, (long long)q, (int)d, db_max_norm, out);
+    else
+        hipLaunchKernelGGL(tau_scale_kernel<dlc_f16_tag>, dim3(grid), dim3(256), 0, st, Q, ldq_b, (long long)q, (int)d, db_max_norm, out);
+    DLC_LAUNCH_CHECK(ctx, "tau_scale_kernel");
+    return DLC_OK;
+}
+
+struct TauScale {
+    const float* array = nullptr;
+    bool derive = false;
+    const float* db_norm_bound = nullptr;
+};
+
 int run_finish(dlc_ctx* ctx, int dtype, const MatchCall& mc, int k, int64_t n, int64_t d, int64_t q, int64_t row_offset,
                float* out_scores, double* out_scores_f64, int64_t* out_idx, int32_t* out_status, void* workspace, int flags,
-               const float* tau_scale, hipStream_t st, int limited = 0, int64_t limit0 = 0, bool direct = false) {
+               TauScale ts, hipStream_t st, int limited = 0, int64_t limit0 = 0, bool direct = false) {
     char* ws = (char*)workspace;
     FinishArgs f = finish_args(mc, k, n, d, q, row_offset);
+    const bool fused512 = !direct && mc.w.rparts <= 1 && !(flags & DLC_SELECT_COOP);
+    if (ts.derive && !ts.array) {
+        if (fused512) { f.scale_here = 1; f.db_norm_bound = ts.db_norm_bound; }
+        else {
+            float* arr = (float*)(ws + mc.w.tscale);
+            int rc0 = launch_tau_scale(ctx, dtype, f.Q, f.ldq_b, q, d, ts.db_norm_bound, arr, st);
+            if (rc0 != DLC_OK) return rc0;
+            ts.array = arr;
+        }
+    }
+    const float* tau_scale = ts.array;
     f.limited = limited; f.limit0 = limit0; f.tau_scale = tau_scale;
     int* status = out_status ? out_status : (int*)(ws + mc.w.status);
     double* s64 = out_scores_f64 ? out_scores_f64 : (double*)(ws + mc.w.s64);
@@ -1770,7 +1868,7 @@
         rc = launch_merge(ctx, ps, q * k, pi, q * k, mc.w.rparts, q, k, pb, mc.w.tau, tau_scale, out_scores, s64, out_idx, status, st);
         if (rc != DLC_OK) return rc;
     }
-    if (direct) return DLC_OK;
+    if (direct || fused512) return DLC_OK;
     return run_exhaustive(ctx, dtype, f, q, s64 + (k - 1), k, out_scores, s64, out_idx, status, st);
 }
 
@@ -1781,14 +1879,15 @@
     return ws_layout(q, n, d, k).tau;
 }
 
-extern "C" int dlc_cosine_topk(dlc_ctx* ctx, int dtype, const void* Q, int64_t q, int64_t ldq, const void* DB,
-                               int64_t n, int64_t lddb, int64_t d, int k, int64_t row_offset, float* out_scores,
-                               double* out_scores_f64, int64_t* out_idx, int32_t* out_status, const float* tau_scale,
-                               void* workspace, size_t workspace_bytes, void* stream) {
+namespace {
+int topk_call(dlc_ctx* ctx, const char* what, int dtype, const void* Q, int64_t q, int64_t ldq, const void* DB, int64_t n,
+              int64_t lddb, int64_t d, int k, int64_t row_offset, int limited, int64_t limit0, float* out_scores,
+              double* out_scores_f64, int64_t* out_idx, int32_t* out_status, TauScale ts, void* workspace,
+              size_t workspace_bytes, void* stream) {
     if (!ctx) return DLC_ERR_BAD_ARG;
-    if (!out_scores || !out_idx) return dlc::fail(ctx, DLC_ERR_BAD_ARG, "cosine_topk: null output");
+    if (!out_scores || !out_idx) return dlc::fail(ctx, DLC_ERR_BAD_ARG, "%s: null output", what);
     MatchCall mc;
-    int rc = prepare_match(ctx, "cosine_topk", dtype, Q, q, ldq, DB, n, lddb, d, k, workspace, workspace_bytes, &mc);
+    int rc = prepare_match(ctx, what, dtype, Q, q, ldq, DB, n, lddb, d, k, workspace, workspace_bytes, &mc);
     if (rc != DLC_OK) return rc;
     dlc::DeviceGuard guard(ctx->device);
     if (!guard.ok) return dlc::fail(ctx, DLC_ERR_HIP, "hipSetDevice(%d) failed", ctx->device);
@@ -1796,25 +1895,43 @@
     rc = run_score(ctx, dtype, mc, (hipStream_t)stream, direct);
     if (rc != DLC_OK) return rc;
     return run_finish(ctx, dtype, mc, k, n, d, q, row_offset, out_scores, out_scores_f64, out_idx, out_status, workspace, 0,
-                      tau_scale, (hipStream_t)stream, 0, 0, direct);
+                      ts, (hipStream_t)stream, limited, limit0, direct);
+}
+}
+
+extern "C" int dlc_cosine_topk(dlc_ctx* ctx, int dtype, const void* Q, int64_t q, int64_t ldq, const void* DB,
+                               int64_t n, int64_t lddb, int64_t d, int k, int64_t row_offset, float* out_scores,
+                               double* out_scores_f64, int64_t* out_idx, int32_t* out_status, const float* tau_scale,
+                               void* workspace, size_t workspace_bytes, void* stream) {
+    return topk_call(ctx, "cosine_topk", dtype, Q, q, ldq, DB, n, lddb, d, k, row_offset, 0, 0, out_scores, out_scores_f64,
+                     out_idx, out_status, TauScale{tau_scale, false, nullptr}, workspace, workspace_bytes, stream);
 }
 
 extern "C" int dlc_cosine_topk_older(dlc_ctx* ctx, int dtype, const void* Q, int64_t q, int64_t ldq, const void* DB,
                                      int64_t n, int64_t lddb, int64_t d, int k, int64_t row_offset, int64_t limit0,
                                      float* out_scores, double* out_scores_f64, int64_t* out_idx, int32_t* out_status,
                                      const float* tau_scale, void* workspace, size_t workspace_bytes, void* stream) {
-    if (!ctx) return DLC_ERR_BAD_ARG;
-    if (!out_scores || !out_idx) return dlc::fail(ctx, DLC_ERR_BAD_ARG, "cosine_topk_older: null output");
-    MatchCall mc;
-    int rc = prepare_match(ctx, "cosine_topk_older", dtype, Q, q, ldq, DB, n, lddb, d, k, workspace, workspace_bytes, &mc);
-    if (rc != DLC_OK) return rc;
-    dlc::DeviceGuard guard(ctx->device);
-    if (!guard.ok) return dlc::fail(ctx, DLC_ERR_HIP, "hipSetDevice(%d) failed", ctx->device);
-    const bool direct = small_direct(mc, k);
-    rc = run_score(ctx, dtype, mc, (hipStream_t)stream, direct);
-    if (rc != DLC_OK) return rc;
-    return run_finish(ctx, dtype, mc, k, n, d, q, row_offset, out_scores, out_scores_f64, out_idx, out_status, workspace, 0,
-                      tau_scale, (hipStream_t)stream, 1, limit0, direct);
+    return topk_call(ctx, "cosine_topk_older", dtype, Q, q, ldq, DB, n, lddb, d, k, row_offset, 1, limit0, out_scores,
+                     out_scores_f64, out_idx, out_status, TauScale{tau_scale, false, nullptr}, workspace, workspace_bytes, stream);
+}
+
+extern "C" int dlc_cosine_topk_bound(dlc_ctx* ctx, int dtype, const void* Q, int64_t q, int64_t ldq, const void* DB,
+                                     int64_t n, int64_t lddb, int64_t d, int k, int64_t row_offset, float* out_scores,
+                                     double* out_scores_f64, int64_t* out_idx, int32_t* out_status,
+                                     const float* db_norm_bound, void* workspace, size_t workspace_bytes, void* stream) {
+    return topk_call(ctx, "cosine_topk_bound", dtype, Q, q, ldq, DB, n, lddb, d, k, row_offset, 0, 0, out_scores,
+                     out_scores_f64, out_idx, out_status, TauScale{nullptr, true, db_norm_bound}, workspace, workspace_bytes,
+                     stream);
+}
+
+extern "C" int dlc_cosine_topk_bound_older(dlc_ctx* ctx, int dtype, const void* Q, int64_t q, int64_t ldq, const void* DB,
+                                           int64_t n, int64_t lddb, int64_t d, int k, int64_t row_offset, int64_t limit0,
+                                           float* out_scores, double* out_scores_f64, int64_t* out_idx,
+                                           int32_t* out_status, const float* db_norm_bound, void* workspace,
+                                           size_t workspace_bytes, void* stream) {
+    return topk_call(ctx, "cosine_topk_bound_older", dtype, Q, q, ldq, DB, n, lddb, d, k, row_offset, 1, limit0, out_scores,
+                     out_scores_f64, out_idx, out_status, TauScale{nullptr, true, db_norm_bound}, workspace, workspace_bytes,
+                     stream);
 }
 
 extern "C" int dlc_cosine_score_groups(dlc_ctx* ctx, int dtype, const void* Q, int64_t q, int64_t ldq, const void* DB,
@@ -1842,7 +1959,7 @@
     dlc::DeviceGuard guard(ctx->device);
     if (!guard.ok) return dlc::fail(ctx, DLC_ERR_HIP, "hipSetDevice(%d) failed", ctx->device);
     return run_finish(ctx, dtype, mc, k, n, d, q, row_offset, out_scores, out_scores_f64, out_idx, out_status, workspace, flags,
-                      tau_scale, (hipStream_t)stream);
+                      TauScale{tau_scale, false, nullptr}, (hipStream_t)stream);
 }
 
 extern "C" int dlc_cosine_groups_per_query(int k) { return (k < 1 || k > DLC_MAX_K) ? 0 : k + SLACK; }
@@ -2051,31 +2168,6 @@
 
 namespace {
 template <typename Tag>
-__device__ __forceinline__ float row_norm_up(const char* __restrict__ row, int d, int lane) {
-    float acc = 0.f;
-    for (int c = lane * 8; c < d; c += 512) {
-        const u32x4_t v = *(const u32x4_t*)(row + (long long)c * 2);
-#pragma unroll
-        for (int j = 0; j < 4; ++j) {
-            float lo, hi;
-            if constexpr (__is_same(Tag, dlc_bf16_tag)) {
-                lo = __uint_as_float(v[j] << 16);
-                hi = __uint_as_float(v[j] & 0xffff0000u);
-            } else {
-                lo = dlc_f16_bits_to_f32((unsigned short)(v[j] & 0xffffu));
-                hi = dlc_f16_bits_to_f32((unsigned short)(v[j] >> 16));
-            }
-            acc = fmaf(lo, lo, acc);
-            acc = fmaf(hi, hi, acc);
-        }
-    }
-#pragma unroll
-    for (int m = 32; m >= 1; m >>= 1) acc += __shfl_xor(acc, m, 64);
-    const float nrm = sqrtf(acc) * 1.001f;
-    return (nrm <= 3.0e38f) ? nrm : INFINITY;
-}
-
-template <typename Tag>
 __global__ __launch_bounds__(256) void max_row_norm_kernel(const char* __restrict__ rows, long long ld_b, long long n, int d,
                                                            float* __restrict__ out) {
     const int lane = threadIdx.x & 63;
@@ -2083,19 +2175,6 @@
     for (long long r = (long long)blockIdx.x * 4 + (threadIdx.x >> 6); r < n; r += (long long)gridDim.x * 4)
         best = fmaxf(best, row_norm_up<Tag>(rows + r * ld_b, d, lane));
     if (lane == 0) atomicMax((unsigned*)out, __float_as_uint(best));
-}
-
-template <typename Tag>
-__global__ __launch_bounds__(256) void tau_scale_kernel(const char* __restrict__ Q, long long ldq_b, long long q, int d,
-                                                        const float* __restrict__ db_max_norm, float* __restrict__ out) {
-    const int lane = threadIdx.x & 63;
-    const long long qi = (long long)blockIdx.x * 4 + (threadIdx.x >> 6);
-    if (qi >= q) return;
-    const float nq = row_norm_up<Tag>(Q + qi * ldq_b, d, lane);
-    const float R = db_max_norm ? *db_max_norm : 1.005f;
-    const float prod = nq * R * (1.0f / 1.01f) * 1.000001f;
-    const float s = (prod <= 3.0e38f) ? fmaxf(prod, 1.0f) : INFINITY;
-    if (lane == 0) out[qi] = s;
 }
 
 int check_rows(dlc_ctx* ctx, const char* what, int dtype, const void* rows, int64_t n, int64_t ld, int64_t d) {
@@ -2135,15 +2214,7 @@
     if (!tau_scale) return dlc::fail(ctx, DLC_ERR_BAD_ARG, "cosine_tau_scale: null output");
     dlc::DeviceGuard guard(ctx->device);
     if (!guard.ok) return dlc::fail(ctx, DLC_ERR_HIP, "hipSetDevice(%d) failed", ctx->device);
-    const unsigned grid = (unsigned)dlc::cdiv(q, 4);
-    if (dtype == DLC_BF16)
-        hipLaunchKernelGGL(tau_scale_kernel<dlc_bf16_tag>, dim3(grid), dim3(256), 0, (hipStream_t)stream, (const char*)Q,
-                           (long long)ldq * 2, (long long)q, (int)d, db_max_norm, tau_scale);
-    else
-        hipLaunchKernelGGL(tau_scale_kernel<dlc_f16_tag>, dim3(grid), dim3(256), 0, (hipStream_t)stream, (const char*)Q,
-                           (long long)ldq * 2, (long long)q, (int)d, db_max_norm, tau_scale);
-    DLC_LAUNCH_CHECK(ctx, "tau_scale_kernel");
-    return DLC_OK;
+    return launch_tau_scale(ctx, dtype, (const char*)Q, (long long)ldq * 2, q, d, db_max_norm, tau_scale, (hipStream_t)stream);
 }
 
 extern "C" double dlc_cosine_score_error_bound_any_plan(int64_t d) {
diff --git a/deeploopcloser_amd/engine.py b/deeploopcloser_amd/engine.py
--- a/deeploopcloser_amd/engine.py
+++ b/deeploopcloser_amd/engine.py
@@ -980,11 +980,16 @@
         if q.stride(1) != 1 or db.stride(1) != 1:
             raise ValueError("stored descriptor rows must be contiguous")
 
-    def match_topk(self, q, db, k, row_offset=0, out=None, details=False, older_than=None, tau_scale=None):
+    def match_topk(self, q, db, k, row_offset=0, out=None, details=False, older_than=None, tau_scale=None, norm_bound=False):
         self._check_stored(q, db)
         nq, d = q.shape
+        bound = norm_bound is not False
+        if bound and tau_scale is not None:
+            raise ValueError("match_topk: tau_scale or norm_bound, not both")
         if tau_scale is not None:
             self._check_out("tau_scale", tau_scale, (nq,), torch.float32)
+        if bound and norm_bound is not None:
+            self._check_out("norm_bound", norm_bound, (1,), torch.float32)
         n = db.shape[0]
         need = self.lib.dlc_cosine_topk_workspace_bytes(nq, n, d, k)
         if need == 0:
@@ -998,15 +1003,16 @@
             idx = self._check_out("out[1] (idx)", out[1], (nq, k), torch.int64)
         s64 = torch.empty((nq, k), dtype=torch.float64, device=self.device) if details else None
         status = torch.empty((nq,), dtype=torch.int32, device=self.device) if details else None
+        lib, dt = self.lib, _TORCH_TO_DLC[q.dtype]
+        norms = _ptr(norm_bound if bound else tau_scale)
         if older_than is None:
-            self._check(self.lib.dlc_cosine_topk(self.ctx, _TORCH_TO_DLC[q.dtype], _ptr(q), nq, q.stride(0), _ptr(db), n,
-                                                  db.stride(0), d, k, row_offset, _ptr(scores), _ptr(s64), _ptr(idx),
-                                                  _ptr(status), _ptr(tau_scale), _ptr(ws), ws.numel(), self._stream()))
+            fn = lib.dlc_cosine_topk_bound if bound else lib.dlc_cosine_topk
+            self._check(fn(self.ctx, dt, _ptr(q), nq, q.stride(0), _ptr(db), n, db.stride(0), d, k, row_offset, _ptr(scores),
+                           _ptr(s64), _ptr(idx), _ptr(status), norms, _ptr(ws), ws.numel(), self._stream()))
         else:
-            self._check(self.lib.dlc_cosine_topk_older(self.ctx, _TORCH_TO_DLC[q.dtype], _ptr(q), nq, q.stride(0), _ptr(db), n,
-                                                        db.stride(0), d, k, row_offset, int(older_than), _ptr(scores),
-                                                        _ptr(s64), _ptr(idx), _ptr(status), _ptr(tau_scale), _ptr(ws),
-                                                        ws.numel(), self._stream()))
+            fn = lib.dlc_cosine_topk_bound_older if bound else lib.dlc_cosine_topk_older
+            self._check(fn(self.ctx, dt, _ptr(q), nq, q.stride(0), _ptr(db), n, db.stride(0), d, k, row_offset, int(older_than),
+                           _ptr(scores), _ptr(s64), _ptr(idx), _ptr(status), norms, _ptr(ws), ws.numel(), self._stream()))
         return TopK(scores, idx, s64, status) if details else (scores, idx)
 
     def topk_workspace_bytes(self, nq, n, d, k):
diff --git a/deeploopcloser_amd/matching.py b/deeploopcloser_amd/matching.py
--- a/deeploopcloser_amd/matching.py
+++ b/deeploopcloser_amd/matching.py
@@ -121,7 +121,9 @@
 
     def match_topk(self, queries, k, out=None, details=False):
         q = self.prepare_queries(queries)
-        return self.engine.match_topk(q, self.rows, k, self.row_offset, out=out, details=details, tau_scale=self.tau_scale(q))
+        if self.norm_bound is None and self.engine.unit_rows(q):
+            return self.engine.match_topk(q, self.rows, k, self.row_offset, out=out, details=details)
+        return self.engine.match_topk(q, self.rows, k, self.row_offset, out=out, details=details, norm_bound=self.norm_bound)
 
     def match(self, queries):
         return self.engine.cosine_scores(self.prepare_queries(queries), self.rows)
diff --git a/include/dlc.h b/include/dlc.h
--- a/include/dlc.h
+++ b/include/dlc.h
@@ -8,7 +8,7 @@
 extern "C" {
 #endif
 
-#define DLC_ABI_VERSION 17
+#define DLC_ABI_VERSION 18
 
 typedef struct dlc_ctx dlc_ctx;
 
@@ -207,10 +207,18 @@
                      void* stream);
 int dlc_cosine_tau_scale(dlc_ctx* ctx, int dtype, const void* Q, int64_t q, int64_t ldq, int64_t d,
                          const float* db_max_norm, float* tau_scale, void* stream);
+int dlc_cosine_topk_bound(dlc_ctx* ctx, int dtype, const void* Q, int64_t q, int64_t ldq,
+                          const void* DB, int64_t n, int64_t lddb, int64_t d, int k, int64_t row_offset,
+                          float* out_scores, double* out_scores_f64, int64_t* out_idx, int32_t* out_status,
+                          const float* db_norm_bound, void* workspace, size_t workspace_bytes, void* stream);
 int dlc_cosine_topk_older(dlc_ctx* ctx, int dtype, const void* Q, int64_t q, int64_t ldq,
                           const void* DB, int64_t n, int64_t lddb, int64_t d, int k, int64_t row_offset, int64_t limit0,
                           float* out_scores, double* out_scores_f64, int64_t* out_idx, int32_t* out_status,
                           const float* tau_scale, void* workspace, size_t workspace_bytes, void* stream);
+int dlc_cosine_topk_bound_older(dlc_ctx* ctx, int dtype, const void* Q, int64_t q, int64_t ldq,
+                                const void* DB, int64_t n, int64_t lddb, int64_t d, int k, int64_t row_offset, int64_t limit0,
+                                float* out_scores, double* out_scores_f64, int64_t* out_idx, int32_t* out_status,
+                                const float* db_norm_bound, void* workspace, size_t workspace_bytes, void* stream);
 double dlc_cosine_score_error_bound(int64_t q, int64_t n, int64_t d, int k);
 double dlc_cosine_score_error_bound_any_plan(int64_t d);
 #define DLC_SELECT_COOP 1
```
